# Chemical118/TREW

Hardware: NVIDIA B200
Metric: Gbases/s for trew short 5 32 at 1/2/4/8 B200; % of HBM roofline (higher is better)
Workload: dtype u64

## Files before the change

trew_b200/csrc/device_ctx.cu:

```cuda
#include <algorithm>
#include <chrono>
#include <cstdarg>
#include <cstdio>
#include <cstdlib>
#include <cstring>
#include <string>
#include <thread>
#include <vector>

#include <cuda_runtime.h>

#include "host_internal.h"
#include "scan_kernels.cuh"

using namespace trew;

namespace {

template <typename T, bool Pinned = false>
struct Buf {
    T* p = nullptr;
    size_t cap = 0;
    Buf() = default;
    Buf(Buf&& o) noexcept : p(o.p), cap(o.cap) { o.p = nullptr; o.cap = 0; }
    Buf(const Buf&) = delete;
    Buf& operator=(const Buf&) = delete;
    ~Buf() { release(); }
    cudaError_t grow(size_t n, cudaStream_t st) {
        if (n <= cap) return cudaSuccess;
        if (p) { cudaError_t e = cudaStreamSynchronize(st); if (e != cudaSuccess) return e; }
        return alloc(std::max((n + n / 4) * sizeof(T), (size_t)1 << 20) / sizeof(T));
    }
    cudaError_t alloc(size_t n) {
        cudaError_t e = release();
        if (e == cudaSuccess) e = Pinned ? cudaHostAlloc((void**)&p, n * sizeof(T), cudaHostAllocDefault) : cudaMalloc((void**)&p, n * sizeof(T));
        if (e != cudaSuccess) p = nullptr;
        else cap = n;
        return e;
    }
    cudaError_t release() {
        cudaError_t e = cudaSuccess;
        if (p) e = Pinned ? cudaFreeHost(p) : cudaFree(p);
        p = nullptr; cap = 0;
        return e;
    }
};

constexpr int kScanCounters = 8;
struct ScanBufs {
    Buf<unsigned int> survivors, counters;
    Buf<unsigned char> scratch;
    cudaError_t alloc(uint32_t n_units) {
        cudaError_t e = survivors.alloc(2 * (size_t)std::max<uint32_t>(n_units, 1));
        return e == cudaSuccess ? counters.alloc(kScanCounters) : e;
    }
};

struct SlotRes {
    Buf<unsigned char, true> h_buf;
    Buf<unsigned char> d_buf;
    Buf<unsigned char, true> h_inv;
    Buf<unsigned char> d_inv;
    size_t inv_cap = 0;
    Buf<unsigned int, true> h_keys;
    ScanBufs scan;
    size_t survivors_cap = 0;
    cudaStream_t stream = nullptr;
    cudaEvent_t ev_start = nullptr, ev_done = nullptr;
    bool in_flight = false;
};

struct RangeInfo { uint32_t r0, r1; uint64_t bases; uint32_t max_len; };

}

struct trew_resident {
    Buf<unsigned char> d_buf;
    DevBatch batch{};
    uint32_t n_reads = 0, n_units = 0, max_read_len = 0;
    uint64_t bases = 0;
    ScanBufs scan;
    cudaEvent_t ev[4] = {nullptr, nullptr, nullptr, nullptr};
    bool ev_pending = false;
};

struct trew_ctx {
    trew_config cfg{};
    int sm_count = 0;
    LaunchPlan plan{};
    cudaStream_t aux_stream = nullptr;
    cudaEvent_t ev_join = nullptr;
    int resident_streams = 1;
    uint64_t resident_seq = 0;
    DevCfg dcfg{};
    size_t n_slots = 0;
    Buf<Slot> table;
    Buf<unsigned int> d_error;
    Buf<unsigned short> d_thr;
    Buf<unsigned long long> d_total_surv;
    std::vector<SlotRes> slots;
    size_t next_slot = 0;
    size_t staging_bytes = 0;
    cudaStream_t main_stream = nullptr;
    cudaEvent_t ev_a = nullptr, ev_b = nullptr;
    Buf<trew_entry> d_entries;
    Buf<trew_entry> d_sorted;
    Buf<trew_entry> d_concat;
    bool sorted_valid = false;
    Buf<unsigned char> d_sort_tmp;
    Buf<unsigned int> d_n;
    uint64_t n_export = 0;
    bool export_valid = false;
    trew_stats stats{};
    Pool* pool = nullptr;
    bool own_pool = true;
    std::string err;
    std::vector<RangeInfo> ranges_tmp;
    unsigned int keys_seen = 0;
    bool sparse_val = true;
    unsigned int exact_flags = 0;
    std::vector<InvList> inv_tmp;
    IngestScratch ingest;
    cudaEvent_t ev_t0 = nullptr, ev_t1 = nullptr;
    double screen_ms = 0, decide_ms = 0, exact_ms = 0; uint64_t n_prof_scans = 0;
    std::vector<trew_resident*> pending_prof;
    Buf<trew_entry, true> h_export;
    unsigned int report_min = 0;
    Buf<trew_entry> d_filtered;
    Buf<UnitRecs> d_recs; Buf<trew_unit_record> d_rec_buf;
    uint64_t unit_next = 0;
    bool table_used = false;
    Buf<trew_unit_record> d_rec_out;
    Buf<trew_unit_record> d_rec_cat;
    Buf<trew_unit_record, true> h_rec;
};

namespace {

int fail(trew_ctx* c, int status, const char* fmt, ...) {
    char buf[512];
    va_list ap; va_start(ap, fmt); vsnprintf(buf, sizeof(buf), fmt, ap); va_end(ap);
    if (c) c->err = buf;
    return status;
}

#define CK(call)                                                                                         \
    do {                                                                                                 \
        cudaError_t e_ = (call);                                                                         \
        if (e_ != cudaSuccess) return fail(ctx, TREW_ERR_CUDA, "%s: %s", #call, cudaGetErrorString(e_)); \
    } while (0)

void build_thr(double B, std::vector<unsigned short>& thr) {
    thr.assign(kThrTableSize, 0xFFFF);
    for (int T = 1; T < kThrTableSize; T++) {
        int lo = 0, hi = T;
        while (lo < hi) {
            int mid = (lo + hi) / 2;
            if ((double)mid / (double)T >= B) hi = mid; else lo = mid + 1;
        }
        thr[T] = (unsigned short)lo;
    }
}

int run_cap_for(const trew_config& cfg, uint32_t max_read_len) {
    uint32_t w = max_read_len;
    if (cfg.mode == TREW_MODE_LONG) w = std::min<uint32_t>(max_read_len, 2u * (uint32_t)cfg.slice_length);
    w = std::min<uint32_t>(w, (uint32_t)kMaxWindow);
    return (int)std::max<uint32_t>((w + 2 + 7) & ~7u, 32u);
}

constexpr unsigned int kLongThreadCap = 32768;

size_t scratch_need(const trew_ctx* ctx, uint32_t max_read_len, uint32_t n_units, unsigned int* stride, size_t* long_off,
                    unsigned int* s_cap, unsigned int* max_slices) {
    unsigned int st = 16;
    if (ctx->cfg.mode == TREW_MODE_LONG) st = 2u * (max_read_len / (uint32_t)ctx->cfg.slice_length + 2u);
    st = (st + 15u) & ~15u;
    *stride = st;
    size_t bytes = ((size_t)st * (size_t)exact_warps_total(ctx->sm_count) + 255) & ~(size_t)255;
    *long_off = bytes;
    *s_cap = 0; *max_slices = 0;
    if (long_thread_path_applies(ctx->dcfg) && (ctx->exact_flags & 16u)) {
        *s_cap = std::min<unsigned int>(std::max<unsigned int>(n_units, 1u), kLongThreadCap);
        *max_slices = max_read_len / (uint32_t)ctx->cfg.slice_length + 1u;
        bytes += long_thread_scratch_bytes(*s_cap, *max_slices);
    }
    return bytes;
}

static int env_blocks_thread() {
    static const int v = [] { const char* e = getenv("TREW_GRID_THREAD"); int x = e && *e ? atoi(e) : 0; return x > 0 ? x : 0; }();
    return v;
}

int launch_scan(trew_ctx* ctx, const DevBatch& b, uint32_t n_units, uint32_t max_read_len, ScanBufs& sb, cudaStream_t st,
                cudaEvent_t* ev = nullptr) {
    unsigned int stride, s_cap, max_slices;
    size_t long_off;
    CK(sb.scratch.grow(scratch_need(ctx, max_read_len, n_units, &stride, &long_off, &s_cap, &max_slices), st));
    unsigned int* d_survivors = sb.survivors.p;
    unsigned int* d_counters = sb.counters.p;
    ctx->export_valid = false;
    ctx->table_used = true;
    DevCfg cfg = ctx->dcfg;
    cfg.unit_base = ctx->unit_next;
    ctx->unit_next += n_units;
    CK(cudaMemsetAsync(d_counters, 0, kScanCounters * sizeof(unsigned int), st));
    if (ev) CK(cudaEventRecord(ev[0], st));
    const bool thread_path = thread_path_applies(cfg, max_read_len) && !(ctx->exact_flags & 4u) && n_units < (1u << 28);
    launch_filter(cfg, b, n_units, max_read_len, d_survivors + n_units, d_counters + 2, d_survivors, d_counters, ctx->plan, st,
                  ev ? ev[1] : nullptr, thread_path ? d_survivors + n_units - 1 : nullptr, thread_path ? d_counters + 4 : nullptr,
                  d_counters + 7);
    if (ev) CK(cudaEventRecord(ev[2], st));
    ExactArgs a{};
    a.survivors = d_survivors; a.n_survivors = d_counters; a.work_counter = d_counters + 1;
    a.slice_scratch = sb.scratch.p; a.slice_scratch_stride = stride; a.run_cap = run_cap_for(ctx->cfg, max_read_len);
    a.total_survivors = ctx->d_total_surv.p;
    a.packed_probes = n_units < (1u << 28) ? 1 : 0;
    a.exp_flags = ctx->exact_flags;
    if (thread_path) {
        unsigned int* hard = d_survivors + n_units;
        launch_exact_thread(cfg, b, d_survivors, d_counters, a.packed_probes, hard, d_counters + 3, ctx->d_total_surv.p,
                            ctx->sm_count, env_blocks_thread(), d_counters + 6, st);
        ExactArgs ab = a;
        ab.survivors = d_survivors + n_units - 1; ab.reverse = 1; ab.n_survivors = d_counters + 4;
        launch_exact(cfg, b, ab, ctx->plan, st);
        a.survivors = hard; a.n_survivors = d_counters + 3; a.work_counter = d_counters + 5; a.total_survivors = nullptr;
        ctx->stats.kernel_launches += 2;
    } else if (s_cap > 0 && n_units < (1u << 28)) {
        unsigned int* hard = d_survivors + n_units;
        launch_long_thread(cfg, b, d_survivors, d_counters, a.packed_probes, s_cap, max_slices, sb.scratch.p + long_off, hard,
                           d_counters + 3, ctx->d_total_surv.p, ctx->sm_count, st);
        a.survivors = hard; a.n_survivors = d_counters + 3; a.total_survivors = nullptr;
        ctx->stats.kernel_launches += 3;
    }
    launch_exact(cfg, b, a, ctx->plan, st);
    if (ev) CK(cudaEventRecord(ev[3], st));
    CK(cudaGetLastError());
    ctx->stats.kernel_launches += 3;
    return TREW_OK;
}

int retire_slot(trew_ctx* ctx, SlotRes& s) {
    if (!s.in_flight) return TREW_OK;
    CK(cudaEventSynchronize(s.ev_done));
    float ms = 0.f;
    CK(cudaEventElapsedTime(&ms, s.ev_start, s.ev_done));
    ctx->stats.device_ms += ms;
    s.in_flight = false;
    ctx->keys_seen = std::max(ctx->keys_seen, *s.h_keys.p);
    return TREW_OK;
}

int export_entries(trew_ctx* ctx, bool need_sorted, const trew_entry** out, uint64_t* n_out);
int check_device_error(trew_ctx* ctx);

int grow_table_to(trew_ctx* ctx, size_t min_slots) {
    size_t new_slots = ctx->n_slots;
    while (new_slots < ((size_t)1 << 28) && new_slots < min_slots) new_slots <<= 1;
    if (new_slots == ctx->n_slots) return TREW_OK;
    uint64_t n = 0;
    int rc = export_entries(ctx, false, nullptr, &n);
    if (rc) return rc;
    Buf<Slot> other;
    CK(other.alloc(new_slots));
    CK(cudaMemsetAsync(other.p, 0, new_slots * sizeof(Slot), ctx->main_stream));
    CK(cudaMemsetAsync(ctx->d_error.p + 1, 0, sizeof(unsigned int), ctx->main_stream));
    std::swap(ctx->table.p, other.p); std::swap(ctx->table.cap, other.cap);
    ctx->dcfg.slots = ctx->table.p; ctx->dcfg.slot_mask = (unsigned int)(new_slots - 1); ctx->n_slots = new_slots;
    launch_merge_entries(ctx->dcfg, ctx->d_entries.p, (unsigned int)n, ctx->main_stream);
    CK(cudaGetLastError());
    CK(cudaStreamSynchronize(ctx->main_stream));
    CK(other.release());
    ctx->stats.kernel_launches += 1;
    ctx->keys_seen = (unsigned int)n;
    for (auto& sl : ctx->slots) *sl.h_keys.p = (unsigned int)n;
    return check_device_error(ctx);
}

int maybe_grow_table(trew_ctx* ctx) {
    if ((size_t)ctx->keys_seen * 16 <= ctx->n_slots) return TREW_OK;
    unsigned int keys = 0;
    CK(cudaMemcpy(&keys, ctx->d_error.p + 1, sizeof(keys), cudaMemcpyDeviceToHost));
    ctx->keys_seen = std::max(ctx->keys_seen, keys);
    if ((size_t)keys * 4 <= ctx->n_slots) return TREW_OK;
    return grow_table_to(ctx, (size_t)keys * 8);
}

DevBatch device_batch(const BatchView& v, uint32_t n, const void* host_base, const void* device_base) {
    auto at = [&](const uint32_t* p) { return (const unsigned int*)((const char*)device_base + ((const char*)p - (const char*)host_base)); };
    DevBatch b{};
    b.n_reads = n; b.bit_off = at(v.bit_off); b.hi = at(v.hi); b.lo = at(v.lo); b.val = at(v.val);
    return b;
}

void copy_batch(const trew_batch* batch, const BatchView& v, Pool* pool) {
    const uint32_t n = batch->n_reads;
    const size_t words = (size_t)((batch->bit_off[n] + 31ULL) / 32);
    memcpy(v.bit_off, batch->bit_off, (size_t)(n + 1) * 4);
    const uint32_t* src[3] = {batch->hi, batch->lo, batch->val};
    uint32_t* dst[3] = {v.hi, v.lo, v.val};
    pool->run(3, [&](int i) {
        memcpy(dst[i], src[i], words * 4);
        memset(dst[i] + words, 0, (v.plane_words - words) * 4);
    });
}

int scan_on_slot(trew_ctx* ctx, SlotRes& s, const DevBatch& b, uint32_t max_len, uint64_t bases, size_t h2d_bytes) {
    const uint32_t n = b.n_reads;
    const uint32_t n_units = ctx->cfg.mode == TREW_MODE_PAIR ? n / 2 : n;
    int rc = launch_scan(ctx, b, n_units, max_len, s.scan, s.stream);
    if (rc) return rc;
    CK(cudaMemcpyAsync(s.h_keys.p, ctx->d_error.p + 1, sizeof(unsigned int), cudaMemcpyDeviceToHost, s.stream));
    CK(cudaEventRecord(s.ev_done, s.stream));
    s.in_flight = true;
    ctx->stats.reads += n; ctx->stats.bases += bases; ctx->stats.units += n_units; ctx->stats.h2d_bytes += h2d_bytes;
    return TREW_OK;
}

int submit_ranges(trew_ctx* ctx, const ChunkView& cv, const RangeInfo* rg, int n_ranges) {
    uint64_t total_bases = 0; uint32_t max_len = 0;
    for (int i = 0; i < n_ranges; i++) { total_bases += rg[i].bases; max_len = std::max(max_len, rg[i].max_len); }
    const uint32_t n = n_ranges ? rg[n_ranges - 1].r1 - rg[0].r0 : 0u;
    if (n == 0) return TREW_OK;
    SlotRes& s = ctx->slots[ctx->next_slot];
    ctx->next_slot = (ctx->next_slot + 1) % ctx->slots.size();
    static const bool trace = getenv("TREW_SUBMIT_TRACE") != nullptr;
    auto now = [] { return std::chrono::duration<double, std::milli>(std::chrono::steady_clock::now().time_since_epoch()).count(); };
    const double t0 = trace ? now() : 0;
    int rc = retire_slot(ctx, s);
    if (rc) return rc;
    const double t1 = trace ? now() : 0;
    if ((rc = maybe_grow_table(ctx)) != TREW_OK) return rc;
    const double t2 = now();
    BatchView v;
    batch_layout(s.h_buf.p, n, total_bases, &v);
    std::vector<uint64_t> bit0((size_t)n_ranges);
    uint64_t acc = 0;
    for (int i = 0; i < n_ranges; i++) { bit0[i] = acc; acc += rg[i].bases; }
    v.bit_off[n] = (uint32_t)total_bases;
    const uint32_t first = rg[0].r0;
    std::vector<uint64_t> side_flat((size_t)3 * n_ranges);
    uint64_t (*side)[3] = (uint64_t (*)[3])side_flat.data();
    if (ctx->inv_tmp.size() < (size_t)n_ranges) ctx->inv_tmp.resize((size_t)n_ranges);
    auto pack = [&](bool list) {
        pack_prepare(bit0.data(), n_ranges, total_bases, v);
        ctx->pool->run(n_ranges, [&](int i) {
            pack_chunk_range(cv, rg[i].r0, rg[i].r1, rg[i].r0 - first, bit0[i], v, side[i], list ? &ctx->inv_tmp[(size_t)i] : nullptr, list,
                             rg[i].bases);
        });
        pack_fixup(bit0.data(), side, n_ranges, v);
    };
    size_t n_inv = 0;
    bool sparse = ctx->sparse_val;
    pack(sparse);
    const bool tail_pad = (total_bases & 31) != 0;
    if (sparse) {
        n_inv = tail_pad ? 1 : 0;
        for (int i = 0; i < n_ranges; i++) n_inv += ctx->inv_tmp[(size_t)i].size();
        if (n_inv > s.inv_cap) { sparse = false; pack(false); }
    }

    const double t3 = now();
    ctx->stats.host_pack_bytes += total_bases; ctx->stats.host_pack_ms += t3 - t2;
    CK(cudaEventRecord(s.ev_start, s.stream));
    const size_t head_bytes = (size_t)((char*)v.val - (char*)s.h_buf.p);
    unsigned int* d_val = (unsigned int*)(s.d_buf.p + head_bytes);
    size_t sent = v.bytes;
    if (sparse) {
        std::vector<size_t> at((size_t)n_ranges + 1, 0);
        for (int i = 0; i < n_ranges; i++) at[(size_t)i + 1] = at[(size_t)i] + ctx->inv_tmp[(size_t)i].bytes();
        ctx->pool->run(n_ranges, [&](int i) {
            const InvList& l = ctx->inv_tmp[(size_t)i];
            if (l.bytes()) memcpy(s.h_inv.p + at[(size_t)i], l.buf.get(), l.bytes());
        });
        if (tail_pad) inv_record(s.h_inv.p + at[(size_t)n_ranges], (uint32_t)total_bases, (1ULL << (32 - (total_bases & 31))) - 1ULL);
        const size_t ones_words = (size_t)((total_bases + 31) / 32);
        CK(cudaMemsetAsync(d_val, 0xFF, ones_words * 4, s.stream));
        CK(cudaMemsetAsync(d_val + ones_words, 0, (v.plane_words - ones_words) * 4, s.stream));
        CK(cudaMemcpyAsync(s.d_buf.p, s.h_buf.p, head_bytes, cudaMemcpyHostToDevice, s.stream));
        if (n_inv) {
            CK(cudaMemcpyAsync(s.d_inv.p, s.h_inv.p, n_inv * kInvRecBytes, cudaMemcpyHostToDevice, s.stream));
            launch_clear_invalid(d_val, (const unsigned int*)s.d_inv.p, (unsigned int)n_inv, s.stream);
            ctx->stats.kernel_launches += 1;
        }
        sent = head_bytes + n_inv * kInvRecBytes;
    } else {
        CK(cudaMemcpyAsync(s.d_buf.p, s.h_buf.p, v.bytes, cudaMemcpyHostToDevice, s.stream));
    }
    rc = scan_on_slot(ctx, s, device_batch(v, n, s.h_buf.p, s.d_buf.p), max_len, total_bases, sent);
    if (rc) return rc;
    if (trace)
        fprintf(stderr, "[submit] %u reads: wait slot %.3f ms, table check %.3f ms, pack %.3f ms, enqueue %.3f ms\n", n, t1 - t0, t2 - t1,
                t3 - t2, now() - t3);
    return TREW_OK;
}

int check_lengths(trew_ctx* ctx, int mode, uint32_t longest) {
    if (mode == TREW_MODE_SHORT && longest > 1000) return fail(ctx, TREW_ERR_TOO_LONG, "%s", trew_status_string(TREW_ERR_TOO_LONG));
    if (mode == TREW_MODE_PAIR && longest > (uint32_t)kMaxWindow) return fail(ctx, TREW_ERR_TOO_LONG, "paired read longer than %d", kMaxWindow);
    return TREW_OK;
}

size_t take_fitting(const trew_ctx* ctx, const RangeInfo* rg, size_t g, size_t n_ranges) {
    size_t h = g; uint64_t bases = 0, reads = 0;
    while (h < n_ranges) {
        const uint64_t nb = bases + rg[h].bases, nr = reads + (rg[h].r1 - rg[h].r0);
        if (batch_bytes((uint32_t)nr, nb) > ctx->staging_bytes || nr > ctx->slots[0].survivors_cap || nb >= 0xfffff000ULL) break;
        bases = nb; reads = nr; h++;
    }
    return h;
}

int submit_chunk_view(trew_ctx* ctx, const ChunkView& cv, uint32_t n) {
    if (n == 0) return TREW_OK;
    const uint32_t unit = cv.unit;
    const uint32_t n_units = n / unit;
    uint64_t span = 0;
    for (int sd = 0; sd < (int)unit; sd++) {
        const int32_t* l = cv.locs[sd];
        span += (uint64_t)std::max<int64_t>(0, (int64_t)l[2 * (size_t)(n_units - 1) + 1] - l[0] + 1);
    }
    uint64_t by_size = span / std::max<uint64_t>(1, ctx->staging_bytes / 16) + 1;
    uint32_t n_ranges = (uint32_t)std::min<uint64_t>(n_units, std::max<uint64_t>(by_size, (uint64_t)ctx->pool->size() * 4));
    auto& rg = ctx->ranges_tmp;
    rg.resize(n_ranges);
    for (uint32_t i = 0; i < n_ranges; i++) {
        rg[i].r0 = (uint32_t)((uint64_t)n_units * i / n_ranges) * unit;
        rg[i].r1 = (uint32_t)((uint64_t)n_units * (i + 1) / n_ranges) * unit;
    }
    ctx->pool->run((int)n_ranges, [&](int i) { chunk_stats(cv, rg[i].r0, rg[i].r1, &rg[i].bases, &rg[i].max_len); });
    uint32_t mx = 0;
    for (auto& r : rg) mx = std::max(mx, r.max_len);
    int rc = check_lengths(ctx, ctx->cfg.mode, mx);
    if (rc) return rc;
    auto too_big = [&](const RangeInfo& r) {
        return fail(ctx, TREW_ERR_ARG, "a single read/pair (%llu bases) does not fit a staging buffer of %zu bytes",
                    (unsigned long long)r.bases, ctx->staging_bytes);
    };
    size_t g = 0;
    while (g < n_ranges) {
        const size_t h = take_fitting(ctx, rg.data(), g, n_ranges);
        if (h > g) {
            if ((rc = submit_ranges(ctx, cv, rg.data() + g, (int)(h - g))) != TREW_OK) return rc;
            g = h;
            continue;
        }
        if (rg[g].r1 - rg[g].r0 <= unit) return too_big(rg[g]);
        std::vector<RangeInfo> fine;
        for (uint32_t r = rg[g].r0; r < rg[g].r1; r += unit) {
            RangeInfo f{r, r + unit, 0, 0};
            chunk_stats(cv, f.r0, f.r1, &f.bases, &f.max_len);
            fine.push_back(f);
        }
        for (size_t a = 0; a < fine.size();) {
            const size_t e = take_fitting(ctx, fine.data(), a, fine.size());
            if (e == a) return too_big(fine[a]);
            std::vector<RangeInfo> merged;
            size_t per = std::max<size_t>(1, (e - a) / (size_t)ctx->pool->size());
            for (size_t i = a; i < e; i += per) {
                RangeInfo m{fine[i].r0, 0, 0, 0};
                for (size_t j = i; j < std::min(e, i + per); j++) { m.r1 = fine[j].r1; m.bases += fine[j].bases; m.max_len = std::max(m.max_len, fine[j].max_len); }
                merged.push_back(m);
            }
            if ((rc = submit_ranges(ctx, cv, merged.data(), (int)merged.size())) != TREW_OK) return rc;
            a = e;
        }
        g++;
    }
    return TREW_OK;
}

int collect_prof(trew_ctx* ctx) {
    for (trew_resident* r : ctx->pending_prof) {
        if (!r->ev_pending) continue;
        CK(cudaEventSynchronize(r->ev[3]));
        float a = 0, b = 0, c = 0;
        CK(cudaEventElapsedTime(&a, r->ev[0], r->ev[1]));
        CK(cudaEventElapsedTime(&b, r->ev[1], r->ev[2]));
        CK(cudaEventElapsedTime(&c, r->ev[2], r->ev[3]));
        ctx->screen_ms += a; ctx->decide_ms += b; ctx->exact_ms += c; ctx->n_prof_scans++;
        ctx->stats.device_ms += a + b + c;
        r->ev_pending = false;
    }
    ctx->pending_prof.clear();
    return TREW_OK;
}

int join_aux(trew_ctx* ctx) {
    if (ctx->resident_streams != 2) return TREW_OK;
    CK(cudaEventRecord(ctx->ev_join, ctx->aux_stream));
    CK(cudaStreamWaitEvent(ctx->main_stream, ctx->ev_join, 0));
    return TREW_OK;
}

int fork_aux(trew_ctx* ctx) {
    if (ctx->resident_streams != 2) return TREW_OK;
    CK(cudaEventRecord(ctx->ev_join, ctx->main_stream));
    CK(cudaStreamWaitEvent(ctx->aux_stream, ctx->ev_join, 0));
    return TREW_OK;
}

int reader_slice_length(const trew_ctx* ctx) { return ctx->d_recs.p ? 0 : ctx->cfg.slice_length; }

int check_batch(trew_ctx* ctx, int mode, const trew_batch* batch) {
    if (!batch) return fail(ctx, TREW_ERR_ARG, "null batch");
    const uint32_t n = batch->n_reads;
    if (n == 0) return TREW_OK;
    if (!batch->bit_off) return fail(ctx, TREW_ERR_ARG, "null bit_off");
    if (batch->bit_off[0] != 0) return fail(ctx, TREW_ERR_ARG, "bit_off[0] must be 0");
    if (mode == TREW_MODE_PAIR && (n & 1u)) return fail(ctx, TREW_ERR_ARG, "paired batch with an odd n_reads (%u): mates come in twos", n);
    uint32_t longest = 0;
    for (uint32_t i = 0; i < n; i++) {
        const uint32_t a = batch->bit_off[i], b = batch->bit_off[i + 1];
        if (b < a) return fail(ctx, TREW_ERR_ARG, "bit_off decreases at read %u (%u after %u)", i, b, a);
        longest = std::max(longest, b - a);
    }
    if (int rc = check_lengths(ctx, mode, longest)) return rc;
    if (batch->max_read_len < longest)
        return fail(ctx, TREW_ERR_ARG, "max_read_len (%u) is smaller than the longest read (%u)", batch->max_read_len, longest);
    return TREW_OK;
}

int check_device_error(trew_ctx* ctx) {
    unsigned int e = 0;
    CK(cudaMemcpy(&e, ctx->d_error.p, sizeof(e), cudaMemcpyDeviceToHost));
    if (e == 3u) return fail(ctx, TREW_ERR_TABLE_FULL, "device count table full (%zu slots): raise table_log2_slots", ctx->n_slots);
    if (e) return fail(ctx, TREW_ERR_CUDA, "device error flag %u", e);
    return TREW_OK;
}

}

extern "C" {

int trew_abi_version(void) { return TREW_ABI_VERSION; }

const char* trew_status_string(int status) {
    switch (status) {
        case TREW_OK: return "ok";
        case TREW_ERR_ARG: return "bad argument";
        case TREW_ERR_CUDA: return "CUDA failure";
        case TREW_ERR_TABLE_FULL: return "device count table full";
        case TREW_ERR_TOO_LONG: return "This mode is designed for short-read sequencing. Please use 'trew long'.";
        case TREW_ERR_IO: return "file I/O error";
        case TREW_ERR_PAIRING: return "paired-end record mismatch";
        case TREW_ERR_NOMEM: return "memory allocation failure";
        default: return "unknown status";
    }
}

int trew_check_batch(int mode, const trew_batch* batch) {
    if (mode < TREW_MODE_SHORT || mode > TREW_MODE_LONG) return TREW_ERR_ARG;
    return check_batch(nullptr, mode, batch);
}

static thread_local std::string g_create_error;

static int default_host_threads(int asked) {
    return asked > 0 ? asked : (int)std::min(64u, std::max(1u, std::thread::hardware_concurrency()));
}

const char* trew_dev_last_error(const trew_ctx* ctx) { return ctx ? ctx->err.c_str() : g_create_error.c_str(); }

static int create_ctx(const trew_config* cfg, trew_ctx** out, std::string& g_create_error, Pool* shared_pool) {
    if (!cfg || !out) return TREW_ERR_ARG;
    *out = nullptr;
    g_create_error.clear();
    auto bad_arg = [&](const char* msg) { g_create_error = msg; return TREW_ERR_ARG; };
    if (cfg->mode < 0 || cfg->mode > 2) return bad_arg("mode must be TREW_MODE_SHORT, _PAIR or _LONG");
    if (cfg->min_mer < 3 || cfg->max_mer > 64 || cfg->min_mer > cfg->max_mer) return bad_arg("need 3 <= MIN_MER <= MAX_MER <= 64");
    if (!(0 < cfg->low_baseline && cfg->low_baseline <= 1) || !(0 < cfg->high_baseline && cfg->high_baseline <= 1) ||
        cfg->low_baseline > cfg->high_baseline) return bad_arg("need 0 < LOW_BASELINE <= HIGH_BASELINE <= 1");
    if (cfg->mode == TREW_MODE_LONG && cfg->slice_length > 0 && cfg->slice_length < 2 * cfg->max_mer)
        return bad_arg("SLICE_LENGTH must be greater than or equal to twice of MAX_MER.");
    if (cfg->mode == TREW_MODE_LONG && cfg->slice_length > 512)
        return bad_arg("SLICE_LENGTH above 512 is not supported by the GPU path (a slice of up to 2*SLICE_LENGTH-1 bases must fit "
                       "a 1023-base window); use -s 512 or less.");
    trew_ctx* ctx = new trew_ctx();
    ctx->cfg = *cfg;
    if (ctx->cfg.slice_length <= 0) ctx->cfg.slice_length = 150;
    auto bail = [&](int rc) { g_create_error = ctx->err; trew_dev_destroy(ctx); return rc; };
#define CKC(call)                                                                                   \
    do {                                                                                            \
        cudaError_t e_ = (call);                                                                    \
        if (e_ != cudaSuccess) { fail(ctx, TREW_ERR_CUDA, "%s: %s", #call, cudaGetErrorString(e_)); return bail(TREW_ERR_CUDA); } \
    } while (0)
    const bool timing = getenv("TREW_CLI_TIMING") != nullptr;
    auto now = [] { return std::chrono::duration<double, std::milli>(std::chrono::steady_clock::now().time_since_epoch()).count(); };
    double t_prev = now();
    auto lap = [&](const char* what) {
        if (!timing) return;
        const double t = now();
        fprintf(stderr, "[trew] create, device %d: %s %.1f ms\n", cfg->device, what, t - t_prev);
        t_prev = t;
    };
    int ndev = 0;
    CKC(cudaGetDeviceCount(&ndev));
    lap("driver init");
    if (cfg->device < 0 || cfg->device >= ndev) { fail(ctx, TREW_ERR_CUDA, "no CUDA device %d (found %d)", cfg->device, ndev); return bail(TREW_ERR_CUDA); }
    CKC(cudaSetDevice(cfg->device));
    cudaDeviceProp prop;
    CKC(cudaGetDeviceProperties(&prop, cfg->device));
    ctx->sm_count = prop.multiProcessorCount;
    ctx->plan = default_launch_plan(ctx->sm_count);
    {
        auto env_int = [](const char* name, int dflt) { const char* e = getenv(name); return e && *e ? atoi(e) : dflt; };
        int v;
        if ((v = env_int("TREW_GRID_SCREEN", 0)) > 0) ctx->plan.screen_blocks = ctx->sm_count * v;
        if ((v = env_int("TREW_GRID_DECIDE", 0)) > 0) ctx->plan.decide_blocks = ctx->sm_count * v;
        if ((v = env_int("TREW_GRID_EXACT", 0)) > 0) ctx->plan.exact_blocks = std::min(ctx->plan.exact_blocks, ctx->sm_count * v);
        ctx->resident_streams = env_int("TREW_RESIDENT_STREAMS", 1) >= 2 ? 2 : 1;
        ctx->sparse_val = env_int("TREW_DENSE_VAL", 0) == 0;
        ctx->exact_flags = (unsigned int)env_int("TREW_EXACT_FLAGS", 0);
    }
    int lg = cfg->table_log2_slots > 0 ? cfg->table_log2_slots : 22;
    if (lg < 10 || lg > 28) { fail(ctx, TREW_ERR_ARG, "table_log2_slots out of range"); return bail(TREW_ERR_ARG); }
    ctx->n_slots = (size_t)1 << lg;
    CKC(ctx->table.alloc(ctx->n_slots));
    CKC(cudaMemset(ctx->table.p, 0, ctx->n_slots * sizeof(Slot)));
    lap("primary context + count table");
    CKC(ctx->d_error.alloc(2));
    CKC(cudaMemset(ctx->d_error.p, 0, 2 * sizeof(unsigned int)));
    CKC(ctx->d_total_surv.alloc(1));
    CKC(cudaMemset(ctx->d_total_surv.p, 0, sizeof(unsigned long long)));
    std::vector<unsigned short> thr;
    build_thr(cfg->low_baseline, thr);
    std::vector<unsigned short> thr_hi;
    build_thr(cfg->high_baseline, thr_hi);
    CKC(ctx->d_thr.alloc(2 * thr.size()));
    CKC(cudaMemcpy(ctx->d_thr.p, thr.data(), thr.size() * sizeof(unsigned short), cudaMemcpyHostToDevice));
    CKC(cudaMemcpy(ctx->d_thr.p + thr.size(), thr_hi.data(), thr_hi.size() * sizeof(unsigned short), cudaMemcpyHostToDevice));
    ctx->dcfg.mode = cfg->mode; ctx->dcfg.min_mer = cfg->min_mer; ctx->dcfg.max_mer = cfg->max_mer;
    ctx->dcfg.slice_len = ctx->cfg.slice_length; ctx->dcfg.low = cfg->low_baseline; ctx->dcfg.high = cfg->high_baseline;
    ctx->dcfg.slots = ctx->table.p; ctx->dcfg.slot_mask = (unsigned int)(ctx->n_slots - 1);
    ctx->dcfg.error_flag = ctx->d_error.p; ctx->dcfg.thr_low = ctx->d_thr.p; ctx->dcfg.thr_high = ctx->d_thr.p + kThrTableSize;
    CKC(prepare_exact(kMaxWindow + 9));
    lap("kernel attributes (module load)");
    CKC(cudaStreamCreateWithFlags(&ctx->main_stream, cudaStreamNonBlocking));
    CKC(cudaStreamCreateWithFlags(&ctx->aux_stream, cudaStreamNonBlocking));
    CKC(cudaEventCreateWithFlags(&ctx->ev_join, cudaEventDisableTiming));
    CKC(cudaEventCreate(&ctx->ev_a));
    CKC(cudaEventCreate(&ctx->ev_b));
    CKC(cudaEventCreate(&ctx->ev_t0));
    CKC(cudaEventCreate(&ctx->ev_t1));
    ctx->staging_bytes = cfg->staging_bytes ? (size_t)cfg->staging_bytes : ((size_t)64 << 20);
    int ns = cfg->n_staging > 0 ? cfg->n_staging : 3;
    ctx->slots.resize((size_t)ns);
    for (auto& s : ctx->slots) {
        CKC(s.h_buf.alloc(ctx->staging_bytes));
        CKC(s.d_buf.alloc(ctx->staging_bytes));
        s.inv_cap = ctx->staging_bytes / 8 / kInvRecBytes;
        CKC(s.h_inv.alloc((s.inv_cap + 1) * kInvRecBytes));
        CKC(s.d_inv.alloc((s.inv_cap + 1) * kInvRecBytes));
        CKC(s.h_keys.alloc(1));
        *s.h_keys.p = 0;
        s.survivors_cap = ctx->staging_bytes / 8;
        CKC(s.scan.alloc((uint32_t)s.survivors_cap));
        CKC(cudaStreamCreateWithFlags(&s.stream, cudaStreamNonBlocking));
        CKC(cudaEventCreate(&s.ev_start));
        CKC(cudaEventCreate(&s.ev_done));
    }
    CKC(ctx->d_n.alloc(1));
    lap("staging ring (pinned + device buffers)");
    if (shared_pool) { ctx->pool = shared_pool; ctx->own_pool = false; }
    else ctx->pool = new Pool(default_host_threads(cfg->host_threads));
#undef CKC
    *out = ctx;
    return TREW_OK;
}

int trew_dev_create(const trew_config* cfg, trew_ctx** out) { return create_ctx(cfg, out, g_create_error, nullptr); }

void trew_dev_destroy(trew_ctx* ctx) {
    if (!ctx) return;
    cudaSetDevice(ctx->cfg.device);
    cudaDeviceSynchronize();
    for (auto& s : ctx->slots) {
        if (s.stream) cudaStreamDestroy(s.stream);
        if (s.ev_start) cudaEventDestroy(s.ev_start);
        if (s.ev_done) cudaEventDestroy(s.ev_done);
    }
    if (ctx->main_stream) cudaStreamDestroy(ctx->main_stream);
    if (ctx->aux_stream) cudaStreamDestroy(ctx->aux_stream);
    if (ctx->ev_join) cudaEventDestroy(ctx->ev_join);
    if (ctx->ev_a) cudaEventDestroy(ctx->ev_a);
    if (ctx->ev_b) cudaEventDestroy(ctx->ev_b);
    if (ctx->ev_t0) cudaEventDestroy(ctx->ev_t0);
    if (ctx->ev_t1) cudaEventDestroy(ctx->ev_t1);
    if (ctx->own_pool) delete ctx->pool;
    delete ctx;
}

int trew_dev_submit_chunk(trew_ctx* ctx, const char* buffer1, const int32_t* locs1, uint32_t n1,
                          const char* buffer2, const int32_t* locs2, uint32_t n2) {
    if (!ctx) return TREW_ERR_ARG;
    CK(cudaSetDevice(ctx->cfg.device));
    const bool pair = ctx->cfg.mode == TREW_MODE_PAIR;
    if (pair ? (!buffer2 && n2) : (buffer2 != nullptr || n2 != 0)) return fail(ctx, TREW_ERR_ARG, "second chunk only in pair mode");
    if ((n1 && (!buffer1 || !locs1)) || (n2 && !locs2)) return fail(ctx, TREW_ERR_ARG, "null chunk");
    ChunkView cv{{buffer1, buffer2}, {locs1, locs2}, {nullptr, nullptr}, pair ? 2u : 1u};
    const uint32_t n = pair ? 2u * std::min(n1, n2) : n1;
    if (n == 0) return TREW_OK;
    for (int sd = 0; sd < (pair ? 2 : 1); sd++) {
        const int32_t* l = cv.locs[sd];
        uint32_t cnt = pair ? n / 2 : n;
        int32_t last = l[2 * (size_t)(cnt - 1) + 1];
        if (last >= l[2 * (size_t)(cnt - 1)]) cv.end[sd] = cv.buf[sd] + last + 1;
    }
    return submit_chunk_view(ctx, cv, n);
}

int trew_dev_submit_packed(trew_ctx* ctx, const trew_batch* batch) {
    if (!ctx || !batch) return TREW_ERR_ARG;
    int rc = check_batch(ctx, ctx->cfg.mode, batch);
    if (rc) return rc;
    CK(cudaSetDevice(ctx->cfg.device));
    uint32_t n = batch->n_reads;
    if (n == 0) return TREW_OK;
    uint64_t bases = batch->bit_off[n];
    size_t bytes = batch_bytes(n, bases);
    if (bytes > ctx->staging_bytes || n > ctx->slots[0].survivors_cap)
        return fail(ctx, TREW_ERR_ARG, "packed batch (%zu bytes) larger than a staging buffer (%zu)", bytes, ctx->staging_bytes);
    SlotRes& s = ctx->slots[ctx->next_slot];
    ctx->next_slot = (ctx->next_slot + 1) % ctx->slots.size();
    rc = retire_slot(ctx, s);
    if (rc) return rc;
    BatchView v;
    batch_layout(s.h_buf.p, n, bases, &v);
    copy_batch(batch, v, ctx->pool);
    CK(cudaEventRecord(s.ev_start, s.stream));
    CK(cudaMemcpyAsync(s.d_buf.p, s.h_buf.p, v.bytes, cudaMemcpyHostToDevice, s.stream));
    return scan_on_slot(ctx, s, device_batch(v, n, s.h_buf.p, s.d_buf.p), batch->max_read_len, bases, v.bytes);
}

int trew_dev_upload(trew_ctx* ctx, const trew_batch* batch, trew_resident** out) {
    if (!ctx || !batch || !out) return TREW_ERR_ARG;
    int rc = check_batch(ctx, ctx->cfg.mode, batch);
    if (rc) return rc;
    CK(cudaSetDevice(ctx->cfg.device));
    uint32_t n = batch->n_reads;
    uint64_t bases = n ? batch->bit_off[n] : 0;
    auto r = std::make_unique<trew_resident>();
    size_t bytes = batch_bytes(n, bases);
    std::vector<char> tmp(bytes, 0);
    BatchView v;
    batch_layout(tmp.data(), n, bases, &v);
    if (n) copy_batch(batch, v, ctx->pool);
    CK(r->d_buf.alloc(bytes));
    CK(cudaMemcpy(r->d_buf.p, tmp.data(), bytes, cudaMemcpyHostToDevice));
    r->batch = device_batch(v, n, tmp.data(), r->d_buf.p);
    r->n_reads = n; r->n_units = ctx->cfg.mode == TREW_MODE_PAIR ? n / 2 : n; r->max_read_len = batch->max_read_len; r->bases = bases;
    CK(r->scan.alloc(r->n_units));
    *out = r.release();
    return TREW_OK;
}

int trew_dev_scan_resident(trew_ctx* ctx, const trew_resident* rb) {
    if (!ctx || !rb) return TREW_ERR_ARG;
    CK(cudaSetDevice(ctx->cfg.device));
    trew_resident* r = const_cast<trew_resident*>(rb);
    ctx->keys_seen = std::max<unsigned int>(ctx->keys_seen, (unsigned int)(ctx->n_slots / 16 + 1));
    if (r->ev_pending) { int rc0 = collect_prof(ctx); if (rc0) return rc0; }
    if (!r->ev[0]) for (int i = 0; i < 4; i++) CK(cudaEventCreate(&r->ev[i]));
    cudaStream_t st = (ctx->resident_streams == 2 && (ctx->resident_seq++ & 1)) ? ctx->aux_stream : ctx->main_stream;
    CK(cudaEventRecord(ctx->ev_a, st));
    int rc = launch_scan(ctx, r->batch, r->n_units, r->max_read_len, r->scan, st, r->ev);
    r->ev_pending = true; ctx->pending_prof.push_back(r);
    if (rc) return rc;
    CK(cudaEventRecord(ctx->ev_b, st));
    ctx->stats.reads += r->n_reads; ctx->stats.bases += r->bases; ctx->stats.units += r->n_units;
    return TREW_OK;
}

void trew_dev_free_resident(trew_ctx* ctx, trew_resident* r) {
    if (!r) return;
    if (ctx) { cudaSetDevice(ctx->cfg.device); cudaStreamSynchronize(ctx->main_stream); cudaStreamSynchronize(ctx->aux_stream); collect_prof(ctx); }
    for (int i = 0; i < 4; i++) if (r->ev[i]) cudaEventDestroy(r->ev[i]);
    delete r;
}

int trew_dev_sync(trew_ctx* ctx) {
    if (!ctx) return TREW_ERR_ARG;
    CK(cudaSetDevice(ctx->cfg.device));
    for (auto& s : ctx->slots) { int rc = retire_slot(ctx, s); if (rc) return rc; }
    { int rc = join_aux(ctx); if (rc) return rc; }
    CK(cudaStreamSynchronize(ctx->main_stream));
    { int rc = collect_prof(ctx); if (rc) return rc; }
    return check_device_error(ctx);
}

}

namespace {

template <typename Call>
cudaError_t with_temp(trew_ctx* ctx, Call call) {
    size_t need = 0;
    cudaError_t e = call(nullptr, &need);
    if (e == cudaSuccess) e = ctx->d_sort_tmp.grow(need, ctx->main_stream);
    if (e != cudaSuccess) return e;
    size_t bytes = ctx->d_sort_tmp.cap;
    return call(ctx->d_sort_tmp.p, &bytes);
}

int export_entries(trew_ctx* ctx, bool need_sorted, const trew_entry** out, uint64_t* n_out) {
    int rc = trew_dev_sync(ctx);
    if (rc) return rc;
    if (!ctx->export_valid) {
        unsigned int n = 1u << 20;
        for (int pass = 0; pass < 2; pass++) {
            CK(ctx->d_entries.grow(n, ctx->main_stream));
            CK(cudaMemsetAsync(ctx->d_n.p, 0, sizeof(unsigned int), ctx->main_stream));
            launch_compact(ctx->dcfg.slots, (unsigned int)ctx->n_slots, ctx->d_entries.p, ctx->d_n.p, ctx->main_stream,
                           (unsigned int)ctx->d_entries.cap);
            CK(cudaGetLastError());
            ctx->stats.kernel_launches += 1;
            CK(cudaMemcpyAsync(&n, ctx->d_n.p, sizeof(n), cudaMemcpyDeviceToHost, ctx->main_stream));
            CK(cudaStreamSynchronize(ctx->main_stream));
            if (n <= ctx->d_entries.cap) break;
        }
        ctx->n_export = n;
        ctx->export_valid = true;
        ctx->sorted_valid = false;
    }
    const unsigned int n = (unsigned int)ctx->n_export;
    if (need_sorted && !ctx->sorted_valid) {
        CK(ctx->d_sorted.grow(n, ctx->main_stream));
        if (n == 1) CK(cudaMemcpyAsync(ctx->d_sorted.p, ctx->d_entries.p, sizeof(trew_entry), cudaMemcpyDeviceToDevice, ctx->main_stream));
        if (n > 1) {
            const bool wide = ctx->cfg.max_mer > 32;
            CK(with_temp(ctx, [&](void* t, size_t* b) { return sort_entries_radix(ctx->d_entries.p, ctx->d_sorted.p, n, wide, t, b, ctx->main_stream); }));
            ctx->stats.kernel_launches += wide ? 11 : 8;
        }
        CK(cudaStreamSynchronize(ctx->main_stream));
        ctx->sorted_valid = true;
    }
    if (out) *out = need_sorted ? ctx->d_sorted.p : ctx->d_entries.p;
    if (n_out) *n_out = n;
    return TREW_OK;
}

template <typename T>
int rows_to_host(trew_ctx* ctx, Buf<T, true>& host, const T* d_rows, uint64_t n, const T** rows, uint64_t* n_rows) {
    CK(host.grow((size_t)n + 64 / sizeof(T), ctx->main_stream));
    if (n) {
        CK(cudaMemcpyAsync(host.p, d_rows, n * sizeof(T), cudaMemcpyDeviceToHost, ctx->main_stream));
        CK(cudaStreamSynchronize(ctx->main_stream));
    }
    ctx->stats.d2h_bytes += n * sizeof(T) + 4;
    if (rows) *rows = host.p;
    if (n_rows) *n_rows = n;
    return TREW_OK;
}

int finish_rows(trew_ctx* ctx, const trew_entry* d_in, uint64_t n_in, bool combine, const trew_entry** entries, uint64_t* n_entries) {
    CK(ctx->d_sorted.grow((size_t)n_in, ctx->main_stream));
    CK(ctx->d_filtered.grow((size_t)n_in, ctx->main_stream));
    ctx->sorted_valid = false;
    const bool wide = ctx->cfg.max_mer > 32;
    const trew_entry* src = d_in;
    unsigned int n = (unsigned int)n_in;
    cudaStream_t st = ctx->main_stream;
    if (ctx->report_min > 0 && n > 0) {
        CK(with_temp(ctx, [&](void* t, size_t* b) { return filter_report_rows(src, n, ctx->report_min, ctx->d_filtered.p, ctx->d_n.p, t, b, st); }));
        CK(cudaMemcpyAsync(&n, ctx->d_n.p, sizeof(n), cudaMemcpyDeviceToHost, st));
        CK(cudaStreamSynchronize(st));
        ctx->stats.kernel_launches += 5;
        src = ctx->d_filtered.p;
    }
    if (n == 1) CK(cudaMemcpyAsync(ctx->d_sorted.p, src, sizeof(trew_entry), cudaMemcpyDeviceToDevice, st));
    if (n > 1) {
        CK(with_temp(ctx, [&](void* t, size_t* b) { return sort_entries_radix(src, ctx->d_sorted.p, n, wide, t, b, st); }));
        ctx->stats.kernel_launches += wide ? 11 : 8;
    }
    const trew_entry* rows = ctx->d_sorted.p;
    if (combine && n > 0) {
        CK(with_temp(ctx, [&](void* t, size_t* b) { return combine_sorted_rows(ctx->d_sorted.p, n, ctx->d_filtered.p, ctx->d_n.p, t, b, st); }));
        CK(cudaMemcpyAsync(&n, ctx->d_n.p, sizeof(n), cudaMemcpyDeviceToHost, st));
        CK(cudaStreamSynchronize(st));
        ctx->stats.kernel_launches += 3;
        rows = ctx->d_filtered.p;
    }
    return rows_to_host(ctx, ctx->h_export, rows, n, entries, n_entries);
}

int unit_record_count(trew_ctx* ctx, uint64_t* made) {
    unsigned long long m = 0;
    CK(cudaMemcpy(&m, &ctx->d_recs.p->n, sizeof(m), cudaMemcpyDeviceToHost));
    *made = m;
    if (m > ctx->d_rec_buf.cap)
        return fail(ctx, TREW_ERR_TABLE_FULL, "unit records overflowed: %llu records made, capacity %llu (a capacity of %llu is enough)", m,
                    (unsigned long long)ctx->d_rec_buf.cap, m);
    return TREW_OK;
}

int records_to_host(trew_ctx* ctx, const trew_unit_record* d_in, uint64_t n_in, const trew_unit_record** recs, uint64_t* n_out) {
    if (n_in > 0x7fffffffULL) return fail(ctx, TREW_ERR_ARG, "too many unit records (%llu)", (unsigned long long)n_in);
    CK(ctx->d_rec_out.grow((size_t)n_in, ctx->main_stream));
    const unsigned int n = (unsigned int)n_in;
    const bool wide = ctx->cfg.max_mer > 32;
    CK(with_temp(ctx, [&](void* t, size_t* b) { return sort_combine_records(d_in, n, wide, ctx->d_rec_out.p, ctx->d_n.p, t, b, ctx->main_stream); }));
    unsigned int m = 0;
    CK(cudaMemcpyAsync(&m, ctx->d_n.p, sizeof(m), cudaMemcpyDeviceToHost, ctx->main_stream));
    CK(cudaStreamSynchronize(ctx->main_stream));
    return rows_to_host(ctx, ctx->h_rec, ctx->d_rec_out.p, m, recs, n_out);
}

}

extern "C" {

int trew_dev_export_device(trew_ctx* ctx, const trew_entry** d_entries, uint64_t* n_entries) {
    if (!ctx) return TREW_ERR_ARG;
    return export_entries(ctx, true, d_entries, n_entries);
}

int trew_dev_finish(trew_ctx* ctx, const trew_entry** entries, uint64_t* n_entries) {
    if (!ctx) return TREW_ERR_ARG;
    uint64_t n = 0;
    const trew_entry* d_rows = nullptr;
    if (ctx->report_min > 0) {
        int rc = export_entries(ctx, false, &d_rows, &n);
        if (rc) return rc;
        return finish_rows(ctx, d_rows, n, false, entries, n_entries);
    }
    int rc = export_entries(ctx, true, &d_rows, &n);
    if (rc) return rc;
    return rows_to_host(ctx, ctx->h_export, d_rows, n, entries, n_entries);
}

int trew_dev_finish_merged(trew_ctx* ctx, const trew_entry* const* d_lists, const uint64_t* n_rows, uint32_t n_lists,
                           const trew_entry** entries, uint64_t* n_entries) {
    if (!ctx || (n_lists && (!d_lists || !n_rows))) return TREW_ERR_ARG;
    uint64_t n0 = 0;
    const trew_entry* d_own = nullptr;
    int rc = export_entries(ctx, false, &d_own, &n0);
    if (rc) return rc;
    uint64_t total = n0;
    for (uint32_t i = 0; i < n_lists; i++) total += n_rows[i];
    if (total > 0xfffffff0ULL) return fail(ctx, TREW_ERR_ARG, "too many rows to merge (%llu)", (unsigned long long)total);
    CK(ctx->d_concat.grow((size_t)total, ctx->main_stream));
    uint64_t at = 0;
    if (n0) CK(cudaMemcpyAsync(ctx->d_concat.p, d_own, n0 * sizeof(trew_entry), cudaMemcpyDeviceToDevice, ctx->main_stream));
    at += n0;
    for (uint32_t i = 0; i < n_lists; i++) {
        if (n_rows[i]) CK(cudaMemcpyAsync(ctx->d_concat.p + at, d_lists[i], n_rows[i] * sizeof(trew_entry), cudaMemcpyDeviceToDevice, ctx->main_stream));
        at += n_rows[i];
    }
    return finish_rows(ctx, ctx->d_concat.p, total, true, entries, n_entries);
}

int trew_dev_export_rows(trew_ctx* ctx, trew_entry* d_rows, uint64_t capacity_rows, uint64_t* n_rows) {
    if (!ctx || !n_rows) return TREW_ERR_ARG;
    uint64_t n = 0;
    const trew_entry* d_src = nullptr;
    int rc = export_entries(ctx, false, &d_src, &n);
    if (rc) return rc;
    *n_rows = n;
    if (!d_rows) return TREW_OK;
    if (n > capacity_rows) return fail(ctx, TREW_ERR_ARG, "row buffer too small: %llu rows, capacity %llu", (unsigned long long)n,
                                       (unsigned long long)capacity_rows);
    if (n) CK(cudaMemcpyAsync(d_rows, d_src, n * sizeof(trew_entry), cudaMemcpyDeviceToDevice, ctx->main_stream));
    CK(cudaStreamSynchronize(ctx->main_stream));
    return TREW_OK;
}

int trew_dev_merge_rows(trew_ctx* ctx, const trew_entry* d_rows, uint64_t n_rows) {
    if (!ctx || (n_rows && !d_rows) || n_rows > 0xffffffffULL) return TREW_ERR_ARG;
    CK(cudaSetDevice(ctx->cfg.device));
    ctx->export_valid = false;
    ctx->table_used = true;
    ctx->keys_seen = std::max<unsigned int>(ctx->keys_seen, (unsigned int)(ctx->n_slots / 16 + 1));
    launch_merge_entries(ctx->dcfg, d_rows, (unsigned int)n_rows, ctx->main_stream);
    CK(cudaGetLastError());
    ctx->stats.kernel_launches += n_rows ? 1 : 0;
    return TREW_OK;
}

int trew_dev_set_report_filter(trew_ctx* ctx, uint32_t min_total) {
    if (!ctx) return TREW_ERR_ARG;
    ctx->report_min = min_total;
    return TREW_OK;
}

int trew_dev_reserve(trew_ctx* ctx, uint64_t expected_new_keys) {
    if (!ctx) return TREW_ERR_ARG;
    int rc = trew_dev_sync(ctx);
    if (rc) return rc;
    unsigned int keys = 0;
    CK(cudaMemcpy(&keys, ctx->d_error.p + 1, sizeof(keys), cudaMemcpyDeviceToHost));
    const uint64_t want = ((uint64_t)keys + expected_new_keys) * 4;
    if (want <= ctx->n_slots) return TREW_OK;
    return grow_table_to(ctx, (size_t)std::min<uint64_t>(want, (uint64_t)1 << 28));
}

int trew_dev_reset(trew_ctx* ctx) {
    if (!ctx) return TREW_ERR_ARG;
    int rc = trew_dev_sync(ctx);
    if (rc && rc != TREW_ERR_TABLE_FULL) return rc;
    ctx->export_valid = false;
    CK(cudaMemsetAsync(ctx->dcfg.slots, 0, ctx->n_slots * sizeof(Slot), ctx->main_stream));
    CK(cudaMemsetAsync(ctx->d_error.p, 0, 2 * sizeof(unsigned int), ctx->main_stream));
    if (ctx->d_recs.p) CK(cudaMemsetAsync(&ctx->d_recs.p->n, 0, sizeof(unsigned long long), ctx->main_stream));
    CK(cudaStreamSynchronize(ctx->main_stream));
    ctx->unit_next = 0;
    ctx->table_used = false;
    ctx->keys_seen = 0;
    for (auto& sl : ctx->slots) *sl.h_keys.p = 0;
    return TREW_OK;
}

int trew_dev_enable_unit_records(trew_ctx* ctx, uint64_t capacity_records) {
    if (!ctx) return TREW_ERR_ARG;
    if (ctx->table_used) return fail(ctx, TREW_ERR_ARG, "unit records can only be switched on or off while the table is empty (after create or reset)");
    if (capacity_records > 0x7fffffffULL) return fail(ctx, TREW_ERR_ARG, "unit record capacity above 2^31 - 1");
    CK(cudaSetDevice(ctx->cfg.device));
    CK(cudaStreamSynchronize(ctx->main_stream));
    ctx->dcfg.recs = nullptr;
    CK(ctx->d_rec_buf.release());
    CK(ctx->d_recs.release());
    if (capacity_records == 0) return TREW_OK;
    CK(ctx->d_rec_buf.alloc(capacity_records));
    CK(ctx->d_recs.alloc(1));
    const UnitRecs r{ctx->d_rec_buf.p, (unsigned long long)capacity_records, 0ULL};
    CK(cudaMemcpy(ctx->d_recs.p, &r, sizeof(r), cudaMemcpyHostToDevice));
    ctx->dcfg.recs = ctx->d_recs.p;
    return TREW_OK;
}

int trew_dev_unit_records(trew_ctx* ctx, const trew_unit_record** recs, uint64_t* n) {
    if (!ctx || !recs || !n) return TREW_ERR_ARG;
    if (!ctx->d_recs.p) return fail(ctx, TREW_ERR_ARG, "unit records are off (trew_dev_enable_unit_records)");
    int rc = trew_dev_sync(ctx);
    if (rc) return rc;
    uint64_t made = 0;
    if ((rc = unit_record_count(ctx, &made)) != TREW_OK) return rc;
    return records_to_host(ctx, ctx->d_rec_buf.p, made, recs, n);
}

int trew_dev_get_stats(trew_ctx* ctx, trew_stats* out) {
    if (!ctx || !out) return TREW_ERR_ARG;
    CK(cudaSetDevice(ctx->cfg.device));
    unsigned long long s = 0;
    CK(cudaMemcpy(&s, ctx->d_total_surv.p, sizeof(s), cudaMemcpyDeviceToHost));
    ctx->stats.survivors = s;
    *out = ctx->stats;
    return TREW_OK;
}

int trew_dev_last_resident_ms(trew_ctx* ctx, float* ms) {
    if (!ctx || !ms) return TREW_ERR_ARG;
    CK(cudaEventSynchronize(ctx->ev_b));
    CK(cudaEventElapsedTime(ms, ctx->ev_a, ctx->ev_b));
    return TREW_OK;
}

int trew_dev_timer_start(trew_ctx* ctx) {
    if (!ctx) return TREW_ERR_ARG;
    CK(cudaSetDevice(ctx->cfg.device));
    CK(cudaEventRecord(ctx->ev_t0, ctx->main_stream));
    return fork_aux(ctx);
}

int trew_dev_timer_stop(trew_ctx* ctx, float* ms) {
    if (!ctx || !ms) return TREW_ERR_ARG;
    CK(cudaSetDevice(ctx->cfg.device));
    { int rc = join_aux(ctx); if (rc) return rc; }
    CK(cudaEventRecord(ctx->ev_t1, ctx->main_stream));
    CK(cudaEventSynchronize(ctx->ev_t1));
    CK(cudaEventElapsedTime(ms, ctx->ev_t0, ctx->ev_t1));
    return TREW_OK;
}

int trew_dev_kernel_times(trew_ctx* ctx, double* screen_ms, double* decide_ms, double* exact_ms, uint64_t* n_scans) {
    if (!ctx) return TREW_ERR_ARG;
    CK(cudaSetDevice(ctx->cfg.device));
    { int rc0 = join_aux(ctx); if (rc0) return rc0; }
    CK(cudaStreamSynchronize(ctx->main_stream));
    int rc = collect_prof(ctx);
    if (rc) return rc;
    if (screen_ms) *screen_ms = ctx->screen_ms;
    if (decide_ms) *decide_ms = ctx->decide_ms;
    if (exact_ms) *exact_ms = ctx->exact_ms;
    if (n_scans) *n_scans = ctx->n_prof_scans;
    ctx->screen_ms = ctx->decide_ms = ctx->exact_ms = 0; ctx->n_prof_scans = 0;
    return TREW_OK;
}

int trew_synth_resident(trew_ctx* ctx, uint64_t seed, uint32_t n_reads, uint32_t read_len, uint32_t tel_ppm,
                        uint32_t half_ppm, uint32_t n_ppm, uint32_t sub_ppm, trew_resident** out) {
    return trew_synth_resident_ex(ctx, seed, n_reads, read_len, tel_ppm, half_ppm, n_ppm, sub_ppm, 0, out);
}

int trew_synth_resident_ex(trew_ctx* ctx, uint64_t seed, uint32_t n_reads, uint32_t read_len, uint32_t tel_ppm,
                           uint32_t half_ppm, uint32_t n_ppm, uint32_t sub_ppm, uint32_t flavor, trew_resident** out) {
    if (!ctx || !out || read_len == 0 || flavor > 2 || (uint64_t)n_reads * read_len >= 0xfffff000ULL) return TREW_ERR_ARG;
    CK(cudaSetDevice(ctx->cfg.device));
    auto thr = [](uint32_t ppm) { return (unsigned int)(((unsigned long long)ppm << 32) / 1000000ULL); };
    uint64_t bases = (uint64_t)n_reads * read_len;
    size_t bytes = batch_bytes(n_reads, bases);
    auto r = std::make_unique<trew_resident>();
    CK(r->d_buf.alloc(bytes));
    BatchView v;
    batch_layout(r->d_buf.p, n_reads, bases, &v);
    launch_synth(seed, n_reads, read_len, thr(tel_ppm), thr(half_ppm), thr(n_ppm), thr(sub_ppm), flavor, v.bit_off, v.hi, v.lo, v.val,
                 v.plane_words, ctx->main_stream);
    CK(cudaGetLastError());
    CK(cudaStreamSynchronize(ctx->main_stream));
    r->batch = device_batch(v, n_reads, r->d_buf.p, r->d_buf.p);
    r->n_reads = n_reads; r->n_units = ctx->cfg.mode == TREW_MODE_PAIR ? n_reads / 2 : n_reads;
    r->max_read_len = read_len; r->bases = bases;
    CK(r->scan.alloc(r->n_units));
    *out = r.release();
    return TREW_OK;
}

int trew_dev_process_file(trew_ctx* ctx, const char* file1, int is_gz1, const char* file2, int is_gz2) {
    if (!ctx || !file1) return TREW_ERR_ARG;
    if ((ctx->cfg.mode == TREW_MODE_PAIR) != (file2 != nullptr)) return fail(ctx, TREW_ERR_ARG, "second file only in pair mode");
    const size_t chunk = 0;
    IngestResult r = ingest_file(ctx->cfg.mode, reader_slice_length(ctx), file1, is_gz1 != 0, file2, is_gz2 != 0, chunk,
                                 [&](const char* b1, const std::vector<int32_t>& l1, const char* b2, const std::vector<int32_t>& l2) {
                                     return trew_dev_submit_chunk(ctx, b1, l1.data(), (uint32_t)(l1.size() / 2), b2,
                                                                  b2 ? l2.data() : nullptr, b2 ? (uint32_t)(l2.size() / 2) : 0u);
                                 },
                                 ctx->pool, &ctx->ingest);
    if (r.status != TREW_OK && r.status != TREW_ERR_CUDA && !r.message.empty()) ctx->err = r.message;
    return r.status;
}

}


struct trew_multi {
    std::vector<trew_ctx*> ctx;
    Pool* pool = nullptr;
    size_t next = 0;
    uint64_t unit_next = 0;
    std::string err;
    Buf<trew_entry> d_peer;
};

namespace {
int mfail(trew_multi* m, int status, const std::string& msg) { if (m) m->err = msg; return status; }
uint64_t chunk_units(const trew_ctx* x, uint32_t n1, uint32_t n2) { return x->cfg.mode == TREW_MODE_PAIR ? std::min(n1, n2) : n1; }

template <typename T>
int gather_to_first(trew_multi* m, size_t first, const std::vector<const T*>& src, const std::vector<uint64_t>& n, Buf<T>& dst) {
    trew_ctx* ctx = m->ctx[0];
    CK(cudaSetDevice(ctx->cfg.device));
    uint64_t total = 0;
    for (size_t i = first; i < n.size(); i++) total += n[i];
    CK(dst.grow((size_t)total, ctx->main_stream));
    uint64_t at = 0;
    for (size_t i = first; i < n.size(); i++) {
        if (n[i]) CK(cudaMemcpyPeerAsync(dst.p + at, ctx->cfg.device, src[i], m->ctx[i]->cfg.device, n[i] * sizeof(T), ctx->main_stream));
        at += n[i];
    }
    return TREW_OK;
}
}

extern "C" {

int trew_multi_create(const trew_config* cfg, const int32_t* devices, int32_t n_devices, trew_multi** out) {
    if (!cfg || !out || n_devices < 0 || (n_devices > 0 && !devices)) return TREW_ERR_ARG;
    *out = nullptr;
    std::vector<int32_t> dev;
    if (n_devices == 0) {
        int nd = 0;
        if (cudaGetDeviceCount(&nd) != cudaSuccess || nd <= 0) { g_create_error = "no CUDA device"; return TREW_ERR_CUDA; }
        for (int i = 0; i < nd; i++) dev.push_back(i);
    } else {
        dev.assign(devices, devices + n_devices);
    }
    trew_multi* m = new trew_multi();
    m->pool = new Pool(default_host_threads(cfg->host_threads));
    int rc = TREW_OK;
    {
        std::vector<trew_ctx*> made(dev.size(), nullptr);
        std::vector<int> rcs(dev.size(), TREW_OK);
        std::vector<std::string> errs(dev.size());
        std::vector<std::thread> th;
        auto make = [&](size_t i) {
            trew_config c = *cfg;
            c.device = dev[i];
            rcs[i] = create_ctx(&c, &made[i], errs[i], m->pool);
        };
        for (size_t i = 1; i < dev.size(); i++) th.emplace_back(make, i);
        make(0);
        for (auto& t : th) t.join();
        for (size_t i = 0; i < dev.size(); i++) {
            if (rcs[i] != TREW_OK && rc == TREW_OK) { rc = rcs[i]; g_create_error = errs[i]; }
            if (made[i]) m->ctx.push_back(made[i]);
        }
    }
    if (rc != TREW_OK) { trew_multi_destroy(m); return rc; }
    for (size_t i = 1; i < m->ctx.size(); i++) {
        int can = 0;
        if (dev[i] != dev[0] && cudaDeviceCanAccessPeer(&can, dev[0], dev[i]) == cudaSuccess && can) {
            cudaSetDevice(dev[0]);
            cudaError_t e = cudaDeviceEnablePeerAccess(dev[i], 0);
            if (e != cudaSuccess) cudaGetLastError();
        }
    }
    *out = m;
    return TREW_OK;
}

void trew_multi_destroy(trew_multi* m) {
    if (!m) return;
    if (!m->ctx.empty()) {
        cudaSetDevice(m->ctx[0]->cfg.device);
        m->d_peer.release();
    }
    for (trew_ctx* x : m->ctx) trew_dev_destroy(x);
    delete m->pool;
    delete m;
}

int trew_multi_device_count(const trew_multi* m) { return m ? (int)m->ctx.size() : 0; }

const char* trew_multi_last_error(const trew_multi* m) { return m ? m->err.c_str() : g_create_error.c_str(); }

trew_ctx* trew_multi_ctx(trew_multi* m, int32_t i) { return m && i >= 0 && (size_t)i < m->ctx.size() ? m->ctx[(size_t)i] : nullptr; }

int trew_multi_submit_chunk(trew_multi* m, const char* buffer1, const int32_t* locs1, uint32_t n1, const char* buffer2,
                            const int32_t* locs2, uint32_t n2) {
    if (!m) return TREW_ERR_ARG;
    trew_ctx* x = m->ctx[m->next];
    m->next = (m->next + 1) % m->ctx.size();
    x->unit_next = m->unit_next;
    int rc = trew_dev_submit_chunk(x, buffer1, locs1, n1, buffer2, locs2, n2);
    if (rc != TREW_OK) return mfail(m, rc, x->err);
    m->unit_next += chunk_units(x, n1, n2);
    return TREW_OK;
}

int trew_multi_process_file(trew_multi* m, const char* file1, int is_gz1, const char* file2, int is_gz2) {
    if (!m || !file1) return TREW_ERR_ARG;
    trew_ctx* x0 = m->ctx[0];
    if ((x0->cfg.mode == TREW_MODE_PAIR) != (file2 != nullptr)) return mfail(m, TREW_ERR_ARG, "second file only in pair mode");
    IngestResult r = ingest_file(x0->cfg.mode, reader_slice_length(x0), file1, is_gz1 != 0, file2, is_gz2 != 0, 0,
                                 [&](const char* b1, const std::vector<int32_t>& l1, const char* b2, const std::vector<int32_t>& l2) {
                                     return trew_multi_submit_chunk(m, b1, l1.data(), (uint32_t)(l1.size() / 2), b2, b2 ? l2.data() : nullptr,
                                                                    b2 ? (uint32_t)(l2.size() / 2) : 0u);
                                 },
                                 m->pool, &x0->ingest);
    if (r.status != TREW_OK && !r.message.empty()) m->err = r.message;
    return r.status;
}

int trew_multi_reset(trew_multi* m) {
    if (!m) return TREW_ERR_ARG;
    for (trew_ctx* x : m->ctx) { int rc = trew_dev_reset(x); if (rc != TREW_OK) return mfail(m, rc, x->err); }
    m->next = 0;
    m->unit_next = 0;
    return TREW_OK;
}

int trew_multi_finish(trew_multi* m, const trew_entry** entries, uint64_t* n_entries) {
    if (!m) return TREW_ERR_ARG;
    trew_ctx* x0 = m->ctx[0];
    const size_t nd = m->ctx.size();
    if (nd == 1) {
        int rc = trew_dev_finish(x0, entries, n_entries);
        return rc == TREW_OK ? rc : mfail(m, rc, x0->err);
    }
    std::vector<const trew_entry*> d_src(nd, nullptr);
    std::vector<uint64_t> n_rows(nd, 0);
    for (size_t i = 1; i < nd; i++) {
        int rc = export_entries(m->ctx[i], false, &d_src[i], &n_rows[i]);
        if (rc != TREW_OK) return mfail(m, rc, m->ctx[i]->err);
    }
    int rc = gather_to_first(m, 1, d_src, n_rows, m->d_peer);
    if (rc) return rc;
    const trew_entry* peers = m->d_peer.p;
    uint64_t n_peers = 0;
    for (size_t i = 1; i < nd; i++) n_peers += n_rows[i];
    rc = trew_dev_finish_merged(x0, &peers, &n_peers, 1, entries, n_entries);
    return rc == TREW_OK ? rc : mfail(m, rc, x0->err);
}

int trew_multi_enable_unit_records(trew_multi* m, uint64_t capacity_records) {
    if (!m) return TREW_ERR_ARG;
    for (trew_ctx* x : m->ctx) {
        int rc = trew_dev_enable_unit_records(x, capacity_records);
        if (rc != TREW_OK) return mfail(m, rc, x->err);
    }
    return TREW_OK;
}

int trew_multi_unit_records(trew_multi* m, const trew_unit_record** recs, uint64_t* n) {
    if (!m || !recs || !n) return TREW_ERR_ARG;
    trew_ctx* x0 = m->ctx[0];
    if (!x0->d_recs.p) return mfail(m, TREW_ERR_ARG, "unit records are off (trew_multi_enable_unit_records)");
    const size_t nd = m->ctx.size();
    std::vector<uint64_t> made(nd, 0);
    uint64_t total = 0, most = 0;
    int full = TREW_OK;
    for (size_t i = 0; i < nd; i++) {
        int rc = trew_dev_sync(m->ctx[i]);
        if (rc != TREW_OK) return mfail(m, rc, m->ctx[i]->err);
        rc = unit_record_count(m->ctx[i], &made[i]);
        if (rc == TREW_ERR_TABLE_FULL) full = rc;
        else if (rc != TREW_OK) return mfail(m, rc, m->ctx[i]->err);
        total += made[i]; most = std::max(most, made[i]);
    }
    if (full != TREW_OK)
        return mfail(m, full, "unit records overflowed on a device: " + std::to_string(most) + " records made, capacity " +
                                  std::to_string(x0->d_rec_buf.cap) + " (a capacity of " + std::to_string(most) + " is enough)");
    if (nd == 1) {
        int rc = records_to_host(x0, x0->d_rec_buf.p, made[0], recs, n);
        return rc == TREW_OK ? rc : mfail(m, rc, x0->err);
    }
    std::vector<const trew_unit_record*> src;
    for (trew_ctx* x : m->ctx) src.push_back(x->d_rec_buf.p);
    int rc = gather_to_first(m, 0, src, made, x0->d_rec_cat);
    if (rc) return rc;
    rc = records_to_host(x0, x0->d_rec_cat.p, total, recs, n);
    return rc == TREW_OK ? rc : mfail(m, rc, x0->err);
}

int trew_multi_set_report_filter(trew_multi* m, uint32_t min_total) {
    if (!m) return TREW_ERR_ARG;
    return trew_dev_set_report_filter(m->ctx[0], min_total);
}

int trew_multi_get_stats(trew_multi* m, trew_stats* out) {
    if (!m || !out) return TREW_ERR_ARG;
    trew_stats t;
    memset(&t, 0, sizeof(t));
    for (trew_ctx* x : m->ctx) {
        trew_stats s;
        int rc = trew_dev_get_stats(x, &s);
        if (rc != TREW_OK) return mfail(m, rc, x->err);
        t.reads += s.reads; t.bases += s.bases; t.units += s.units; t.survivors += s.survivors;
        t.kernel_launches += s.kernel_launches; t.h2d_bytes += s.h2d_bytes; t.d2h_bytes += s.d2h_bytes;
        t.host_pack_bytes += s.host_pack_bytes; t.host_pack_ms += s.host_pack_ms;
        t.device_ms = std::max(t.device_ms, s.device_ms);
    }
    *out = t;
    return TREW_OK;
}

}
```

trew_b200/csrc/scan_kernels.cu:

```cuda
#include "scan_kernels.cuh"
#include "exact_thread.cuh"

#include <cstdio>

namespace trew {

typedef unsigned int u32;
typedef unsigned long long u64;
typedef unsigned __int128 u128;


__device__ __forceinline__ u32 lane_id() { return threadIdx.x & 31; }

__device__ __forceinline__ u32 low_mask(int bits) {
    return bits >= 32 ? 0xffffffffu : ((1u << bits) - 1u);
}

__device__ __forceinline__ u32 prefix_xor32(u32 x) {
    x ^= x << 1; x ^= x << 2; x ^= x << 4; x ^= x << 8; x ^= x << 16;
    return x;
}

__device__ __forceinline__ u64 mix64(u64 x) {
    x ^= x >> 33; x *= 0xff51afd7ed558ccdULL; x ^= x >> 33; x *= 0xc4ceb9fe1a85ec53ULL; x ^= x >> 33;
// ... 196 lines not shown

template <int NW>
__device__ __forceinline__ void prefix_xor_excl(const u32 (&in)[NW], u32 (&out)[NW]) {
    u32 carry = 0, prev_top = 0;
#pragma unroll
    for (int j = 0; j < NW; j++) {
        u32 inc = prefix_xor32(in[j]) ^ carry;
        out[j] = (inc << 1) | prev_top;
        prev_top = inc >> 31;
        carry = 0u - prev_top;
    }
}

template <int NW>
__device__ __forceinline__ void shr1(u32 (&x)[NW]) {
#pragma unroll
    for (int j = 0; j < NW; j++) x[j] = __funnelshift_r(x[j], j + 1 < NW ? x[j + 1] : 0u, 1);
}

template <int NW>
__device__ __forceinline__ void shr_var(const u32 (&in)[NW], int k, u32 (&out)[NW]) {
#pragma unroll
    for (int j = 0; j < NW; j++) out[j] = in[j];
    for (int s = k >> 5; s > 0; s--) {
#pragma unroll
        for (int j = 0; j < NW; j++) out[j] = j + 1 < NW ? out[j + 1] : 0u;
    }
    u32 r = k & 31;
#pragma unroll
    for (int j = 0; j < NW; j++) out[j] = __funnelshift_r(out[j], j + 1 < NW ? out[j + 1] : 0u, r);
}

template <int NW>
__device__ __forceinline__ void sliding_and(u32 (&a)[NW], int k) {
    u32 t[NW];
    int w = 1;
    while (2 * w <= k) {
        shr_var<NW>(a, w, t);
#pragma unroll
        for (int j = 0; j < NW; j++) a[j] &= t[j];
        w *= 2;
    }
    if (k > w) {
        shr_var<NW>(a, k - w, t);
#pragma unroll
        for (int j = 0; j < NW; j++) a[j] &= t[j];
    }
}

__device__ __forceinline__ void csa(u32 a, u32 b, u32 c, u32& s, u32& cy) {
    s = a ^ b ^ c;
    cy = (a & b) | (c & (a ^ b));
}

template <int NW>
__device__ __forceinline__ int popc_multi(const u32 (&x)[NW]) {
    if constexpr (NW == 1) return __popc(x[0]);
    else if constexpr (NW == 2) return __popc(x[0]) + __popc(x[1]);
    else if constexpr (NW == 3) {
        u32 s, c; csa(x[0], x[1], x[2], s, c);
        return __popc(s) + 2 * __popc(c);
    } else if constexpr (NW == 5) {
        u32 s1, c1, s2, c2; csa(x[0], x[1], x[2], s1, c1); csa(s1, x[3], x[4], s2, c2);
        return __popc(s2) + 2 * (__popc(c1) + __popc(c2));
    } else if constexpr (NW == 8) {
        u32 s1, c1, s2, c2, s3, c3, s4, c4;
        csa(x[0], x[1], x[2], s1, c1); csa(x[3], x[4], x[5], s2, c2); csa(s1, s2, x[6], s3, c3);
        csa(c1, c2, c3, s4, c4);
        return __popc(s3) + __popc(x[7]) + 2 * __popc(s4) + 4 * __popc(c4);
    } else {
        int t = 0;
#pragma unroll
        for (int j = 0; j < NW; j++) t += __popc(x[j]);
        return t;
    }
}

template <int NW>
__device__ __noinline__ bool probe_filter(const DevBatch& b, u32 pos, int wl, int k0, int k1,
                                          const unsigned short* __restrict__ thr) {
    u32 PH[NW], PL[NW], QH[NW], QL[NW], WV[NW];
    {
        u32 t[NW];
        load_bits<NW>(b.hi, pos, t); prefix_xor_excl<NW>(t, PH);
        load_bits<NW>(b.lo, pos, t); prefix_xor_excl<NW>(t, PL);
        load_bits<NW>(b.val, pos, WV); mask_bits<NW>(WV, wl);
    }
    shr_var<NW>(PH, k0, QH);
    shr_var<NW>(PL, k0, QL);
    sliding_and<NW>(WV, k0);
    u32 PA[NW];
    bool have_pa = false;
    for (int k = k0; k <= k1; k++) {
        u32 a[NW], bb[NW], c[NW];
#pragma unroll
        for (int j = 0; j < NW; j++) {
            u32 dh = QH[j] ^ PH[j], dl = QL[j] ^ PL[j];
            a[j] = dh & WV[j]; bb[j] = dl & WV[j]; c[j] = a[j] & dl;
        }
        int T = popc_multi<NW>(WV);
        if (T == 0) break;
        int cH = popc_multi<NW>(a), cL = popc_multi<NW>(bb), c11 = popc_multi<NW>(c);
        int c10 = cH - c11, c01 = cL - c11, c00 = T - cH - cL + c11;
        int U = max(max(c00, c01), max(c10, c11));
        int need = thr[T];
        if (U >= need) {
            u32 QA[NW];
            if (!have_pa) {
                u32 A[NW], t[NW];
                load_bits<NW>(b.hi, pos, A); load_bits<NW>(b.lo, pos, t);
#pragma unroll
                for (int j = 0; j < NW; j++) A[j] &= t[j];
                prefix_xor_excl<NW>(A, PA);
                have_pa = true;
            }
            shr_var<NW>(PA, k, QA);
            u32 x11[NW], x10[NW], x01[NW], x00[NW];
#pragma unroll
            for (int j = 0; j < NW; j++) {
                u32 da = QA[j] ^ PA[j];
                u32 dh = QH[j] ^ PH[j], dl = QL[j] ^ PL[j];
                x11[j] = c[j] & da; x10[j] = a[j] & ~dl & da; x01[j] = bb[j] & ~dh & da; x00[j] = WV[j] & ~dh & ~dl & da;
            }
            int n11 = popc_multi<NW>(x11), n10 = popc_multi<NW>(x10), n01 = popc_multi<NW>(x01), n00 = popc_multi<NW>(x00);
            int U2 = max(max(max(n11, c11 - n11), max(n10, c10 - n10)), max(max(n01, c01 - n01), max(n00, c00 - n00)));
            if (U2 >= need) return true;
        }
        shr1<NW>(QH); shr1<NW>(QL);
        u32 t[NW];
#pragma unroll
        for (int j = 0; j < NW; j++) t[j] = WV[j];
        shr1<NW>(t);
#pragma unroll
        for (int j = 0; j < NW; j++) WV[j] &= t[j];
    }
    return false;
}

template <int MAXNW>
__device__ __forceinline__ bool probe_dispatch(const DevBatch& b, const Probe& p, const unsigned short* thr) {
    if (p.k1 < p.k0) return false;
    int need_bits = p.wl + 1;
    if (need_bits <= 96) return probe_filter<3>(b, p.pos, p.wl, p.k0, p.k1, thr);
    if constexpr (MAXNW >= 5) { if (need_bits <= 160) return probe_filter<5>(b, p.pos, p.wl, p.k0, p.k1, thr); }
    if constexpr (MAXNW >= 8) { if (need_bits <= 256) return probe_filter<8>(b, p.pos, p.wl, p.k0, p.k1, thr); }
    return true;
}


constexpr u32 kPackC11 = 1u - (1u << 8) - (1u << 16) + (1u << 24);
constexpr u32 kPackH = (1u << 8) - (1u << 24);
constexpr u32 kPackL = (1u << 16) - (1u << 24);
#ifndef TREW_SCREEN_UNROLL
#define TREW_SCREEN_UNROLL 2
#endif
constexpr int kScreenUnroll = TREW_SCREEN_UNROLL;
constexpr int kFastMaxWl = 95;
constexpr int kFastTabSize = kFastMaxWl + 2;
constexpr int kProbeShift = 28;
constexpr int kMod4BelowWindows = 48;
constexpr int kThreadMinWindows = 36;

__device__ __forceinline__ uint4 fast_entry(int T, int need) {
    uint4 e = make_uint4(0u, 0u, 0u, 0u);
    if (T <= 0) return e;
    int T01 = min(T, 64);
    e.y = T >= 32 ? 0xffffffffu : ((1u << T) - 1u);
    e.z = T <= 32 ? 0u : (T >= 64 ? 0xffffffffu : ((1u << (T - 32)) - 1u));
    int np = need - (T - T01);
    if (np <= 0) e.x = 0x80808080u;
    else if (np > 64) e.x = (u32)T01 << 24;
    else e.x = ((u32)T01 << 24) + (u32)(128 - np) * 0x01010101u;
    return e;
}

template <int S>
__device__ __forceinline__ bool fast_span(const u32 (&ph)[5], const u32 (&pl)[5], int wl, int ka, int kb,
                                          const uint4* __restrict__ tab) {
    const uint4* tp = tab + (wl - ka + 1);
#pragma unroll (kScreenUnroll)
    for (int k = ka; k <= kb; k++, tp--) {
        const uint4 e = *tp;
        u32 qh0 = __funnelshift_r(ph[S], ph[S + 1], k), qh1 = __funnelshift_r(ph[S + 1], ph[S + 2], k);
        u32 ql0 = __funnelshift_r(pl[S], pl[S + 1], k), ql1 = __funnelshift_r(pl[S + 1], pl[S + 2], k);
        u32 a0 = (qh0 ^ ph[0]) & e.y, a1 = (qh1 ^ ph[1]) & e.z;
        u32 b0 = (ql0 ^ pl[0]) & e.y, b1 = (ql1 ^ pl[1]) & e.z;
        u32 x = e.x + (u32)(__popc(a0) + __popc(a1)) * kPackH + (u32)(__popc(b0) + __popc(b1)) * kPackL +
                (u32)(__popc(a0 & b0) + __popc(a1 & b1)) * kPackC11;
        if (x & 0x80808080u) return true;
    }
    return false;
}

__device__ __forceinline__ bool probe_is_fast(const Probe& p) { return p.wl <= kFastMaxWl && p.k1 <= 63 && p.k1 <= p.wl; }

__device__ __forceinline__ bool screen_probe(const DevBatch& b, const Probe& p, const uint4* __restrict__ tab) {
    if (p.k1 < p.k0) return false;
    if (!probe_is_fast(p)) return true;
    u32 t[3], full[3] = {0xffffffffu, 0xffffffffu, 0xffffffffu};
    mask_bits<3>(full, p.wl);
    load_bits<3>(b.val, p.pos, t);
    if ((((t[0] & full[0]) ^ full[0]) | ((t[1] & full[1]) ^ full[1]) | ((t[2] & full[2]) ^ full[2])) != 0u) return true;
    u32 ph[5], pl[5], q[3];
    load_bits<3>(b.hi, p.pos, t); mask_bits<3>(t, p.wl); prefix_xor_excl<3>(t, q);
    ph[0] = q[0]; ph[1] = q[1]; ph[2] = q[2]; ph[3] = 0u; ph[4] = 0u;
    load_bits<3>(b.lo, p.pos, t); mask_bits<3>(t, p.wl); prefix_xor_excl<3>(t, q);
    pl[0] = q[0]; pl[1] = q[1]; pl[2] = q[2]; pl[3] = 0u; pl[4] = 0u;
    int k0 = p.k0;
    if (k0 < 32) {
        if (fast_span<0>(ph, pl, p.wl, k0, min(p.k1, 31), tab)) return true;
        k0 = 32;
    }
    return p.k1 >= 32 && fast_span<1>(ph, pl, p.wl, k0, p.k1, tab);
}

constexpr int kFastMaxWlLong = 159;
constexpr int kFastTabSizeLong = kFastMaxWlLong + 2;
struct __align__(16) FastEntryLong { u32 base, m0, m1, m2, m3, pad0, pad1, pad2; };

__device__ __forceinline__ FastEntryLong fast_entry_long(int T, int need) {
    FastEntryLong e = {0u, 0u, 0u, 0u, 0u, 0u, 0u, 0u};
    if (T <= 0) return e;
    const int T01 = min(T, 128);
    u32 m[4];
#pragma unroll
    for (int j = 0; j < 4; j++) { int vb = T - 32 * j; m[j] = vb <= 0 ? 0u : low_mask(min(32, vb)); }
    e.m0 = m[0]; e.m1 = m[1]; e.m2 = m[2]; e.m3 = m[3];
    const int np = need - (T - T01);
    if (np <= 0) e.base = 0x80808080u;
    else if (np > 128) e.base = 0u;
    else e.base = ((u32)T01 << 24) + (u32)(128 - np) * 0x01010101u;
    return e;
}

template <int S>
__device__ __forceinline__ bool fast_span_long(const u32 (&ph)[8], const u32 (&pl)[8], int wl, int ka, int kb,
                                               const FastEntryLong* __restrict__ tab) {
    const FastEntryLong* tp = tab + (wl - ka + 1);
    for (int k = ka; k <= kb; k++, tp--) {
        const uint4 e0 = *reinterpret_cast<const uint4*>(tp);
        const u32 m3 = tp->m3;
        if (e0.x == 0u) continue;
        const u32 mk[4] = {e0.y, e0.z, e0.w, m3};
        int cH = 0, cL = 0, c11 = 0;
#pragma unroll
        for (int j = 0; j < 4; j++) {
            u32 a = (__funnelshift_r(ph[S + j], ph[S + j + 1], k) ^ ph[j]) & mk[j];
            u32 bb = (__funnelshift_r(pl[S + j], pl[S + j + 1], k) ^ pl[j]) & mk[j];
            cH += __popc(a); cL += __popc(bb); c11 += __popc(a & bb);
        }
        u32 x = e0.x + (u32)cH * kPackH + (u32)cL * kPackL + (u32)c11 * kPackC11;
        if (x & 0x80808080u) return true;
    }
    return false;
}

__device__ __forceinline__ bool probe_is_fast_long(const Probe& p) { return p.wl <= kFastMaxWlLong && p.k1 <= 64 && p.k1 <= p.wl; }

__device__ __noinline__ bool screen_probe_long(const DevBatch& b, const Probe& p, const FastEntryLong* __restrict__ tab) {
    u32 t[5], full[5] = {0xffffffffu, 0xffffffffu, 0xffffffffu, 0xffffffffu, 0xffffffffu};
    mask_bits<5>(full, p.wl);
    load_bits<5>(b.val, p.pos, t);
    u32 bad = 0;
#pragma unroll
    for (int j = 0; j < 5; j++) bad |= (t[j] & full[j]) ^ full[j];
    if (bad) return true;
    u32 ph[8], pl[8], q[5];
    load_bits<5>(b.hi, p.pos, t); mask_bits<5>(t, p.wl); prefix_xor_excl<5>(t, q);
#pragma unroll
    for (int j = 0; j < 8; j++) ph[j] = j < 5 ? q[j] : 0u;
    load_bits<5>(b.lo, p.pos, t); mask_bits<5>(t, p.wl); prefix_xor_excl<5>(t, q);
#pragma unroll
    for (int j = 0; j < 8; j++) pl[j] = j < 5 ? q[j] : 0u;
    int k0 = p.k0;
    if (k0 < 32) {
        if (fast_span_long<0>(ph, pl, p.wl, k0, min(p.k1, 31), tab)) return true;
        k0 = 32;
    }
    if (k0 < 64 && p.k1 >= 32) {
        if (fast_span_long<1>(ph, pl, p.wl, k0, min(p.k1, 63), tab)) return true;
        k0 = 64;
    }
    return p.k1 >= 64 && fast_span_long<2>(ph, pl, p.wl, k0, p.k1, tab);
}

__device__ __forceinline__ void list_append(bool flag, u32 value, u32* __restrict__ list, u32* __restrict__ count) {
    u32 m = __ballot_sync(0xffffffffu, flag);
    if (m) {
        u32 base = 0;
        if (lane_id() == 0) base = atomicAdd(count, (u32)__popc(m));
        base = __shfl_sync(0xffffffffu, base, 0);
        if (flag) list[base + __popc(m & ((1u << lane_id()) - 1u))] = value;
    }
}

__device__ __forceinline__ void list_append_rev(bool flag, u32 value, u32* __restrict__ top, u32* __restrict__ count) {
    u32 m = __ballot_sync(0xffffffffu, flag);
    if (m) {
        u32 base = 0;
        if (lane_id() == 0) base = atomicAdd(count, (u32)__popc(m));
        base = __shfl_sync(0xffffffffu, base, 0);
        if (flag) *(top - (base + __popc(m & ((1u << lane_id()) - 1u)))) = value;
    }
}

#ifndef TREW_SCREEN_BPS
#define TREW_SCREEN_BPS 8
#endif
template <bool LONG>
__global__ void __launch_bounds__(256, LONG ? 4 : TREW_SCREEN_BPS) trew_screen_kernel(DevCfg cfg, DevBatch b, u32 n_units,
                                                                                     u32* __restrict__ deferred, u32* __restrict__ n_deferred) {
    __shared__ uint4 tab[kFastTabSize];
    __shared__ FastEntryLong tab_long[LONG ? kFastTabSizeLong : 1];
    for (int T = threadIdx.x; T < kFastTabSize; T += blockDim.x) tab[T] = fast_entry(T, (int)cfg.thr_low[T]);
    if (LONG) for (int T = threadIdx.x; T < kFastTabSizeLong; T += blockDim.x) tab_long[T] = fast_entry_long(T, (int)cfg.thr_low[T]);
    __syncthreads();
    u32 stride = gridDim.x * blockDim.x;
    u32 n_round = (n_units + 31u) & ~31u;
    for (u32 u = blockIdx.x * blockDim.x + threadIdx.x; u < n_round; u += stride) {
        u32 pm = 0;
        if (u < n_units) {
            Probe p[4];
            int np = unit_probes(cfg, b, u, p);
            for (int i = 0; i < np; i++) {
                bool d;
                if (LONG && p[i].k1 >= p[i].k0 && !probe_is_fast(p[i]) && probe_is_fast_long(p[i])) d = screen_probe_long(b, p[i], tab_long);
                else d = screen_probe(b, p[i], tab);
                pm |= d ? 1u << i : 0u;
            }
        }
        list_append(pm != 0, u | (pm << kProbeShift), deferred, n_deferred);
    }
}

__device__ __forceinline__ int max4(int a, int b, int c, int d) { return max(max(a, b), max(c, d)); }

__device__ __forceinline__ u32 shr3(const u32 (&p)[3], int j, int k) {
    const int s = k >> 5;
    const u32 lo = j + s < 3 ? (s ? (j == 0 ? p[1] : p[2]) : p[j]) : 0u;
    const u32 hi = j + s + 1 < 3 ? (s ? p[2] : (j == 0 ? p[1] : p[2])) : 0u;
    return __funnelshift_r(lo, hi, k);
}
constexpr int kDecideThreads = 256;
__device__ __noinline__ bool mod4_level(const DevBatch& b, u32 pos, int wl, int k, int need, u32 pass8, u32 wv0, u32 wv1, u32 wv2, u32* cache,
                                        bool& cached) {
    const u32 wv[3] = {wv0, wv1, wv2};
    u32 p0[3][3], p1[3][3];
    if (!cached) {
        u32 x[3][3];
        load_bits<3>(b.hi, pos, x[0]); mask_bits<3>(x[0], wl);
        load_bits<3>(b.lo, pos, x[1]); mask_bits<3>(x[1], wl);
#pragma unroll
        for (int j = 0; j < 3; j++) x[2][j] = x[0][j] & x[1][j];
#pragma unroll
        for (int p = 0; p < 3; p++) {
            prefix_xor_excl<3>(x[p], p0[p]);
            u32 c[3];
#pragma unroll
            for (int j = 0; j < 3; j++) c[j] = x[p][j] & p0[p][j];
            prefix_xor_excl<3>(c, p1[p]);
#pragma unroll
            for (int j = 0; j < 3; j++) { cache[(6 * p + j) * kDecideThreads] = p0[p][j]; cache[(6 * p + 3 + j) * kDecideThreads] = p1[p][j]; }
        }
        cached = true;
    } else {
#pragma unroll
        for (int p = 0; p < 3; p++)
#pragma unroll
            for (int j = 0; j < 3; j++) { p0[p][j] = cache[(6 * p + j) * kDecideThreads]; p1[p][j] = cache[(6 * p + 3 + j) * kDecideThreads]; }
    }
    u32 d0[3][3], d1[3][3];
#pragma unroll
    for (int p = 0; p < 3; p++) {
#pragma unroll
        for (int j = 0; j < 3; j++) {
            const u32 q0 = shr3(p0[p], j, k);
            d0[p][j] = q0 ^ p0[p][j];
            d1[p][j] = shr3(p1[p], j, k) ^ p1[p][j] ^ (~q0 & p0[p][j]);
        }
    }
#pragma unroll 1
    for (int c2 = 0; c2 < 8; c2++) {
        if (!((pass8 >> c2) & 1u)) continue;
        u32 mw[3];
        int cnt = 0;
#pragma unroll
        for (int j = 0; j < 3; j++) {
            mw[j] = wv[j] & (d0[0][j] ^ ((c2 & 1) ? 0u : ~0u)) & (d0[1][j] ^ ((c2 & 2) ? 0u : ~0u)) & (d0[2][j] ^ ((c2 & 4) ? 0u : ~0u));
            cnt += __popc(mw[j]);
        }
        if (cnt < need) continue;
        bool may = true;
#pragma unroll
        for (int p = 0; p < 3 && may; p++) {
            const int one = __popc(mw[0] & d1[p][0]) + __popc(mw[1] & d1[p][1]) + __popc(mw[2] & d1[p][2]);
            const int zero = cnt - one;
            if (min(one, zero) >= need) return true;
            const u32 flip = one >= zero ? 0u : ~0u;
#pragma unroll
            for (int j = 0; j < 3; j++) mw[j] &= d1[p][j] ^ flip;
            cnt = max(one, zero);
            may = cnt >= need;
        }
        if (may) return true;
    }
    return false;
}

template <int S>
__device__ __forceinline__ bool decide_span(const u32 (&ph)[5], const u32 (&pl)[5], const u32 (&pa)[5], u32 (&wv)[3], int ka, int kb,
                                            const unsigned short* __restrict__ thr, bool& done, int& t_hit, const DevBatch& bt, u32 pos, int wl,
                                            u32* cache, bool& cached, int m4_below) {
    for (int k = ka; k <= kb; k++) {
        const int T01 = __popc(wv[0]) + __popc(wv[1]), E = __popc(wv[2]), T = T01 + E;
        if (T == 0) { done = true; return false; }
        const int need = thr[T];
        u32 a0 = (__funnelshift_r(ph[S], ph[S + 1], k) ^ ph[0]) & wv[0], a1 = (__funnelshift_r(ph[S + 1], ph[S + 2], k) ^ ph[1]) & wv[1];
        u32 b0 = (__funnelshift_r(pl[S], pl[S + 1], k) ^ pl[0]) & wv[0], b1 = (__funnelshift_r(pl[S + 1], pl[S + 2], k) ^ pl[1]) & wv[1];
        int cH = __popc(a0) + __popc(a1), cL = __popc(b0) + __popc(b1), c11 = __popc(a0 & b0) + __popc(a1 & b1);
        if (max4(c11, cH - c11, cL - c11, T01 - cH - cL + c11) + E >= need) {
            u32 a2 = (__funnelshift_r(ph[S + 2], ph[S + 3], k) ^ ph[2]) & wv[2], b2 = (__funnelshift_r(pl[S + 2], pl[S + 3], k) ^ pl[2]) & wv[2];
            cH += __popc(a2); cL += __popc(b2); c11 += __popc(a2 & b2);
            const int c10 = cH - c11, c01 = cL - c11, c00 = T - cH - cL + c11;
            if (max4(c11, c10, c01, c00) >= need) {
                u32 x0 = __funnelshift_r(pa[S], pa[S + 1], k) ^ pa[0], x1 = __funnelshift_r(pa[S + 1], pa[S + 2], k) ^ pa[1];
                u32 x2 = __funnelshift_r(pa[S + 2], pa[S + 3], k) ^ pa[2];
                int n11 = __popc(a0 & b0 & x0) + __popc(a1 & b1 & x1) + __popc(a2 & b2 & x2);
                int n10 = __popc(a0 & ~b0 & x0) + __popc(a1 & ~b1 & x1) + __popc(a2 & ~b2 & x2);
                int n01 = __popc(b0 & ~a0 & x0) + __popc(b1 & ~a1 & x1) + __popc(b2 & ~a2 & x2);
                int n00 = __popc(wv[0] & ~a0 & ~b0 & x0) + __popc(wv[1] & ~a1 & ~b1 & x1) + __popc(wv[2] & ~a2 & ~b2 & x2);
                int U2 = max(max4(n11, c11 - n11, n10, c10 - n10), max4(n01, c01 - n01, n00, c00 - n00));
                if (U2 >= need) {
                    const u32 pass8 = (u32)(c00 - n00 >= need) | (u32)(c10 - n10 >= need) << 1 | (u32)(c01 - n01 >= need) << 2 |
                                      (u32)(c11 - n11 >= need) << 3 | (u32)(n00 >= need) << 4 | (u32)(n10 >= need) << 5 |
                                      (u32)(n01 >= need) << 6 | (u32)(n11 >= need) << 7;
                    if (T >= m4_below || mod4_level(bt, pos, wl, k, need, pass8, wv[0], wv[1], wv[2], cache, cached)) { t_hit = T; return true; }
                }
            }
        }
        u32 t0 = __funnelshift_r(wv[0], wv[1], 1), t1 = __funnelshift_r(wv[1], wv[2], 1), t2 = wv[2] >> 1;
        wv[0] &= t0; wv[1] &= t1; wv[2] &= t2;
    }
    return false;
}

__device__ __noinline__ bool decide_short(const DevBatch& b, u32 pos, int wl, int k0, int k1, const unsigned short* __restrict__ thr, int& t_hit,
                                          u32* cache, int m4_below) {
    bool cached = false;
    u32 wv[3], ph[5], pl[5], pa[5];
    load_bits<3>(b.val, pos, wv); mask_bits<3>(wv, wl);
    {
        u32 h[3], l[3], q[3];
        load_bits<3>(b.hi, pos, h); mask_bits<3>(h, wl); prefix_xor_excl<3>(h, q);
        ph[0] = q[0]; ph[1] = q[1]; ph[2] = q[2]; ph[3] = 0u; ph[4] = 0u;
        load_bits<3>(b.lo, pos, l); mask_bits<3>(l, wl); prefix_xor_excl<3>(l, q);
        pl[0] = q[0]; pl[1] = q[1]; pl[2] = q[2]; pl[3] = 0u; pl[4] = 0u;
#pragma unroll
        for (int j = 0; j < 3; j++) h[j] &= l[j];
        prefix_xor_excl<3>(h, q);
        pa[0] = q[0]; pa[1] = q[1]; pa[2] = q[2]; pa[3] = 0u; pa[4] = 0u;
    }
    sliding_and<3>(wv, k0);
    bool done = false;
    if (k0 < 32) {
        if (decide_span<0>(ph, pl, pa, wv, k0, min(k1, 31), thr, done, t_hit, b, pos, wl, cache, cached, m4_below)) return true;
        if (done) return false;
        k0 = 32;
    }
    return k1 >= 32 && decide_span<1>(ph, pl, pa, wv, k0, k1, thr, done, t_hit, b, pos, wl, cache, cached, m4_below);
}

template <int MAXNW>
__global__ void __launch_bounds__(kDecideThreads, (MAXNW <= 5 ? 4 : 2)) trew_filter_kernel(DevCfg cfg, DevBatch b, const u32* __restrict__ units,
                                                          const u32* __restrict__ n_units_ptr, u32 n_units_all,
                                                          u32* __restrict__ survivors, u32* __restrict__ n_survivors,
                                                          u32* __restrict__ surv_b_top, u32* __restrict__ n_surv_b, int thread_min_windows, int third_level,
                                                          u32* __restrict__ work_counter) {
    __shared__ unsigned short thr[kThrTableSize];
    __shared__ u32 s_m4[18 * kDecideThreads];
    for (int i = threadIdx.x; i < kThrTableSize; i += blockDim.x) thr[i] = cfg.thr_low[i];
    __syncthreads();
    const u32 n_units = units ? *n_units_ptr : n_units_all;
    const bool pack_probes = n_units_all < (1u << kProbeShift);
    const u32 lane = lane_id();
    bool have = false, maybe = false, exhausted = false;
    u32 u = 0, live = 0, todo = 0;
    int t_hit = 1 << 20;
    Probe p[4];
    for (;;) {
        const u32 idle = __ballot_sync(0xffffffffu, !have);
        if (idle != 0u && !exhausted) {
            u32 base = 0;
            if (lane == 0) base = atomicAdd(work_counter, (u32)__popc(idle));
            base = __shfl_sync(0xffffffffu, base, 0);
            exhausted = base + (u32)__popc(idle) >= n_units;
            const u32 i = base + (u32)__popc(idle & ((1u << lane) - 1u));
            if (!have && i < n_units) {
                u32 pm = 0xfu;
                u = i;
                if (units) { const u32 e = units[i]; u = e & ((1u << kProbeShift) - 1u); pm = e >> kProbeShift; }
                const int np = unit_probes(cfg, b, u, p);
                live = todo = pm & ((1u << np) - 1u);
                maybe = false; t_hit = 1 << 20; have = true;
            }
        }
        if (__ballot_sync(0xffffffffu, have) == 0u) break;
        if (have && todo != 0u) {
            const int j = __ffs(todo) - 1;
            todo &= todo - 1u;
            if (p[j].k1 >= p[j].k0)
                maybe = probe_is_fast(p[j]) ? decide_short(b, p[j].pos, p[j].wl, p[j].k0, p[j].k1, thr, t_hit, s_m4 + threadIdx.x, third_level)
                                            : probe_dispatch<MAXNW>(b, p[j], thr);
            if (!maybe) live &= ~(1u << j);
        }
        const bool fin = have && (todo == 0u || maybe);
        const bool keep = fin && maybe;
        const u32 entry = pack_probes ? u | (live << kProbeShift) : u;
        if (surv_b_top == nullptr) {
            list_append(keep, entry, survivors, n_survivors);
        } else {
            bool to_b = false;
            if (keep) {
                int len;
                if (cfg.mode == 1) {
                    const u32 a0 = __ldg(b.bit_off + 2 * u), a1 = __ldg(b.bit_off + 2 * u + 1), a2 = __ldg(b.bit_off + 2 * u + 2);
                    len = (int)max(a1 - a0, a2 - a1);
                } else {
                    len = (int)(__ldg(b.bit_off + u + 1) - __ldg(b.bit_off + u));
                }
                to_b = len > et::kMaxRead || t_hit < thread_min_windows;
            }
            list_append(keep && !to_b, entry, survivors, n_survivors);
            list_append_rev(keep && to_b, entry, surv_b_top, n_surv_b);
        }
        if (fin) have = false;
    }
}

void launch_filter(const DevCfg& cfg, const DevBatch& b, unsigned int n_units, unsigned int max_read_len,
                   unsigned int* deferred, unsigned int* n_deferred, unsigned int* survivors, unsigned int* n_survivors,
                   const LaunchPlan& plan, cudaStream_t stream, cudaEvent_t after_screen, unsigned int* surv_b_top,
                   unsigned int* n_surv_b, unsigned int* work_counter) {
    if (n_units == 0) return;
    unsigned int longest;
    if (cfg.mode == 2) longest = 2u * (unsigned)cfg.slice_len;
    else longest = (max_read_len < 4u * (unsigned)cfg.max_mer) ? max_read_len : (max_read_len + 1) / 2;
    unsigned int need = (n_units + 255) / 256;
    const bool screen = deferred != nullptr && !(cfg.mode == 2 && cfg.slice_len > kFastMaxWlLong) && n_units < (1u << kProbeShift);
    if (screen) {
        int blocks = plan.screen_blocks;
        if ((unsigned)blocks > need) blocks = (int)need;
        if (longest <= (unsigned)kFastMaxWl) trew_screen_kernel<false><<<blocks, 256, 0, stream>>>(cfg, b, n_units, deferred, n_deferred);
        else trew_screen_kernel<true><<<blocks, 256, 0, stream>>>(cfg, b, n_units, deferred, n_deferred);
    }
    if (after_screen) cudaEventRecord(after_screen, stream);
    static const int tmw = [] { const char* e = getenv("TREW_THREAD_MIN_WINDOWS"); return e && *e ? atoi(e) : kThreadMinWindows; }();
    static const int m4_on = [] { const char* e = getenv("TREW_MOD4_BELOW"); return e && *e ? atoi(e) : kMod4BelowWindows; }();
    const unsigned int* list = screen ? deferred : nullptr;
    int blocks = plan.decide_blocks;
    if ((unsigned)blocks > need) blocks = (int)need;
    if (longest + 1 <= 96) trew_filter_kernel<3><<<blocks, 256, 0, stream>>>(cfg, b, list, n_deferred, n_units, survivors, n_survivors, surv_b_top, n_surv_b, tmw, m4_on, work_counter);
    else if (longest + 1 <= 160) trew_filter_kernel<5><<<blocks, 256, 0, stream>>>(cfg, b, list, n_deferred, n_units, survivors, n_survivors, surv_b_top, n_surv_b, tmw, m4_on, work_counter);
    else trew_filter_kernel<8><<<blocks, 256, 0, stream>>>(cfg, b, list, n_deferred, n_units, survivors, n_survivors, surv_b_top, n_surv_b, tmw, m4_on, work_counter);
}


extern __shared__ __align__(16) unsigned char g_smem[];

constexpr int kPlaneWords = 36;
#ifndef TREW_EXACT_BPS
#define TREW_EXACT_BPS 8
#endif
#ifndef TREW_EXACT_WARPS
#define TREW_EXACT_WARPS 4
#endif
constexpr int kExactWarps = TREW_EXACT_WARPS;
constexpr u32 kEmptySlot = 0xffffffffu;
constexpr int kSerialMaxRuns = 12;

enum { HD_CUR_POS = 0, HD_CUR_LEN, HD_ALLVALID, HD_EV_POS, HD_EV_LEN, HD_EV_K, HD_EV_PACK, HD_UNIT = 7 ,
       HD_S = 8 ,
       HD_BLK_L = 12 , HD_BLK_H = 14 , HD_NEED_L = 16, HD_NEED_H = 17, HD_BLK64 = 18, HD_RES = 19,
       HD_SH = 20 , HD_SL = 24 , HD_UNIT_BASE = 28 ,
       HD_RECS = 30  };
constexpr int kHeaderBytes = 128;

__host__ __device__ inline int exact_hash_slots(int cap) {
    int hs = 64;
    while (hs < cap + cap / 4) hs <<= 1;
    return hs;
}

__host__ __device__ inline size_t exact_warp_bytes(int cap) {
    size_t b = kHeaderBytes + 5 * kPlaneWords * sizeof(u32) + kPlaneWords * sizeof(u64);
    b += (size_t)2 * cap * sizeof(u64) + (size_t)exact_hash_slots(cap) * sizeof(u32) + (size_t)2 * cap * sizeof(u32);
    b += (size_t)(3 * cap + 4) * sizeof(unsigned short);
    return (b + 15) & ~(size_t)15;
}

size_t exact_smem_bytes(int run_cap, bool) { return exact_warp_bytes(run_cap) * kExactWarps; }

struct WS {
    u32 off; int cap; int hs; u32 lane; u32 flags;
    __device__ __forceinline__ u32* hdr() const { return (u32*)(g_smem + off); }
    __device__ __forceinline__ u32* H() const { return (u32*)(g_smem + off + kHeaderBytes); }
    __device__ __forceinline__ u32* L() const { return H() + kPlaneWords; }
    __device__ __forceinline__ u32* V() const { return H() + 2 * kPlaneWords; }
    __device__ __forceinline__ u32* PH() const { return H() + 3 * kPlaneWords; }
    __device__ __forceinline__ u32* PL() const { return H() + 4 * kPlaneWords; }
    __device__ __forceinline__ u64* rev2() const { return (u64*)(H() + 5 * kPlaneWords); }
    __device__ __forceinline__ u64* run_lo() const { return rev2() + kPlaneWords; }
    __device__ __forceinline__ u64* run_hi() const { return run_lo() + cap; }
    __device__ __forceinline__ u32* htab() const { return (u32*)(run_hi() + cap); }
    __device__ __forceinline__ u32* grp_tot() const { return htab() + hs; }
    __device__ __forceinline__ u32* grp_last() const { return grp_tot() + cap; }
    __device__ __forceinline__ unsigned short* run_start() const { return (unsigned short*)(grp_last() + cap); }
    __device__ __forceinline__ unsigned short* run_cw() const { return run_start() + cap; }
    __device__ __forceinline__ unsigned short* run_total() const { return run_cw() + cap + 4; }
};

struct TableRef { Slot* slots; u32 mask; u32* err; };

struct ScanRes { int th, tl; u64 sh_lo, sh_hi, sl_lo, sl_hi; };

__device__ __forceinline__ int pk_T(u32 p) { return (int)(p & 1023u); }
__device__ __forceinline__ int pk_M(u32 p) { return (int)((p >> 10) & 1023u); }
__device__ __forceinline__ int pk_runs(u32 p) { return (int)((p >> 20) & 1023u); }
__device__ __forceinline__ bool pk_homo(u32 p) { return ((p >> 30) & 1u) != 0; }


__device__ __noinline__ u64 canon64(u64 w, int k) {
    int sh = 2 * (k - 1);
    if (k <= 16) {
        u32 b32 = (u32)w, c32 = (u32)w;
        for (int r = 1; r < k; r++) {
            c32 = ((c32 & 3u) << sh) | (c32 >> 2);
            b32 = min(b32, c32);
        }
        return b32;
    }
    u64 best = w, cur = w;
    for (int r = 1; r < k; r++) {
        cur = ((cur & 3ULL) << sh) | (cur >> 2);
        best = cur < best ? cur : best;
    }
    return best;
}

__device__ __noinline__ u128 canon128(u128 w, int k) {
    u128 best = w, cur = w;
    int sh = 2 * (k - 1);
    for (int r = 1; r < k; r++) {
        cur = ((cur & 3) << sh) | (cur >> 2);
        best = cur < best ? cur : best;
    }
    return best;
}

__device__ __forceinline__ u64 rev_pairs64(u64 x) {
    x = __brevll(x);
    return ((x >> 1) & 0x5555555555555555ULL) | ((x & 0x5555555555555555ULL) << 1);
}

__device__ __forceinline__ void canon_pair(u64& lo, u64& hi, int k) {
    if (k <= 32) { lo = canon64(lo, k); hi = 0; }
    else { u128 c = canon128(((u128)hi << 64) | lo, k); lo = (u64)c; hi = (u64)(c >> 64); }
}

__device__ __forceinline__ void crc_pair(u64& lo, u64& hi, int k) {
    if (k <= 32) {
        u64 r = ~rev_pairs64(lo) >> (64 - 2 * k);
        lo = canon64(r, k); hi = 0;
    } else {
        u128 r = ((u128)(~rev_pairs64(lo)) << 64) | (u128)(~rev_pairs64(hi));
        r >>= (128 - 2 * k);
        u128 c = canon128(r, k); lo = (u64)c; hi = (u64)(c >> 64);
    }
}

__device__ __forceinline__ bool homo_pair(u64 lo, u64 hi, int k) {
    if (k <= 1) return true;
    if (k <= 32) return ((lo ^ (lo >> 2)) & ((1ULL << (2 * (k - 1))) - 1ULL)) == 0;
    u128 w = ((u128)hi << 64) | lo;
    u128 m = (((u128)1 << (2 * (k - 1))) - 1);
    return ((w ^ (w >> 2)) & m) == 0;
}

__device__ __forceinline__ bool less_pair(u64 alo, u64 ahi, u64 blo, u64 bhi) {
    return ahi < bhi || (ahi == bhi && alo < blo);
}

__device__ __forceinline__ u32 shfl_next_bit0(u32 x, u32 lane) {
    u32 nx = __shfl_down_sync(0xffffffffu, x, 1);
    return lane == 31 ? 0u : (nx & 1u);
}


__device__ __noinline__ void load_window(WS ws, const u32* __restrict__ bhi, const u32* __restrict__ blo,
                                         const u32* __restrict__ bval, u32 pos, int len) {
    u32* hd = ws.hdr();
    if ((int)hd[HD_CUR_LEN] == len && hd[HD_CUR_POS] == pos) return;
    __syncwarp();
    const u32 lane = ws.lane;
    int vbits = len - 32 * (int)lane;
    u32 msk = vbits <= 0 ? 0u : low_mask(vbits);
    u32 h = 0, l = 0, v = 0;
    if (vbits > 0) {
        u32 wi = (pos >> 5) + lane, sh = pos & 31;
        h = __funnelshift_r(__ldg(bhi + wi), __ldg(bhi + wi + 1), sh) & msk;
        l = __funnelshift_r(__ldg(blo + wi), __ldg(blo + wi + 1), sh) & msk;
        v = __funnelshift_r(__ldg(bval + wi), __ldg(bval + wi + 1), sh) & msk;
    }
    const bool all_valid = __all_sync(0xffffffffu, v == msk);
    u32 ih = prefix_xor32(h), il = prefix_xor32(l);
    u32 bh = __ballot_sync(0xffffffffu, ih >> 31), bl = __ballot_sync(0xffffffffu, il >> 31);
    u32 lt = (1u << lane) - 1u;
    if (__popc(bh & lt) & 1) ih = ~ih;
    if (__popc(bl & lt) & 1) il = ~il;
    u32 ph_prev = __shfl_up_sync(0xffffffffu, ih, 1), pl_prev = __shfl_up_sync(0xffffffffu, il, 1);
    u32 ph = (ih << 1) | (lane ? ph_prev >> 31 : 0u);
    u32 pl = (il << 1) | (lane ? pl_prev >> 31 : 0u);
    u32 *H = ws.H(), *L = ws.L(), *V = ws.V(), *PH = ws.PH(), *PL = ws.PL();
    u64* rev2 = ws.rev2();
    H[lane] = h; L[lane] = l; V[lane] = v; PH[lane] = ph; PL[lane] = pl;
    if (lane < kPlaneWords - 32) {
        H[32 + lane] = 0; L[32 + lane] = 0; V[32 + lane] = 0; PH[32 + lane] = 0; PL[32 + lane] = 0;
        rev2[32 + lane] = 0;
    }
    __syncwarp();
    {
        int cs = len - 32 * (int)lane - 32;
        u32 hb = 0, lb = 0;
        if (cs > -32) {
            if (cs >= 0) {
                int wi = cs >> 5, sh = cs & 31;
                hb = __funnelshift_r(H[wi], H[wi + 1], sh);
                lb = __funnelshift_r(L[wi], L[wi + 1], sh);
            } else {
                hb = H[0] << (-cs);
                lb = L[0] << (-cs);
            }
        }
        hb = __brev(hb); lb = __brev(lb);
        u64 x = hb, y = lb;
        x = (x | (x << 16)) & 0x0000FFFF0000FFFFULL; y = (y | (y << 16)) & 0x0000FFFF0000FFFFULL;
        x = (x | (x << 8)) & 0x00FF00FF00FF00FFULL;  y = (y | (y << 8)) & 0x00FF00FF00FF00FFULL;
        x = (x | (x << 4)) & 0x0F0F0F0F0F0F0F0FULL;  y = (y | (y << 4)) & 0x0F0F0F0F0F0F0F0FULL;
        x = (x | (x << 2)) & 0x3333333333333333ULL;  y = (y | (y << 2)) & 0x3333333333333333ULL;
        x = (x | (x << 1)) & 0x5555555555555555ULL;  y = (y | (y << 1)) & 0x5555555555555555ULL;
        rev2[lane] = (x << 1) | y;
    }
    if (lane == 0) { hd[HD_CUR_POS] = pos; hd[HD_CUR_LEN] = (u32)len; hd[HD_ALLVALID] = all_valid ? 1u : 0u; }
    __syncwarp();
}

__device__ __forceinline__ void kmer_at(const u64* __restrict__ rev2, int len, int i, int k, u64& lo, u64& hi) {
    int o = 2 * (len - i - k);
    int wi = o >> 6, sh = o & 63;
    u64 a = rev2[wi], b = rev2[wi + 1];
    lo = sh ? (a >> sh) | (b << (64 - sh)) : a;
    if (k <= 32) {
        if (k < 32) lo &= (1ULL << (2 * k)) - 1ULL;
        hi = 0;
    } else {
        u64 c = rev2[wi + 2];
        hi = sh ? (b >> sh) | (c << (64 - sh)) : b;
        if (k < 64) hi &= (1ULL << (2 * k - 64)) - 1ULL;
    }
}

__device__ __forceinline__ u32 wv_for_k(WS ws, int len, int k) {
    const u32 lane = ws.lane;
    if (ws.hdr()[HD_ALLVALID]) {
        int vb = len - k + 1 - 32 * (int)lane;
        return vb <= 0 ? 0u : low_mask(min(32, vb));
    }
    u32 wv = ws.V()[lane];
    for (int t = 1; t < k; t++) {
        u32 nb = shfl_next_bit0(wv, lane);
        wv &= (wv >> 1) | (nb << 31);
    }
    return wv;
}

__device__ __forceinline__ u32 wv_step(u32 wv, u32 lane) {
    u32 nb = shfl_next_bit0(wv, lane);
    return wv & ((wv >> 1) | (nb << 31));
}

__device__ __forceinline__ int bound_k(WS ws, int k, u32 wv, int T) {
    const u32 lane = ws.lane;
    const u32 *PH = ws.PH(), *PL = ws.PL();
    int s = k >> 5, r = k & 31;
    u32 qh = __funnelshift_r(PH[lane + s], PH[lane + s + 1], r);
    u32 ql = __funnelshift_r(PL[lane + s], PL[lane + s + 1], r);
    u32 dh = (qh ^ PH[lane]) & wv, dl = (ql ^ PL[lane]) & wv;
    u32 packed = (u32)__popc(dh) | ((u32)__popc(dl) << 10) | ((u32)__popc(dh & dl) << 20);
    packed = __reduce_add_sync(0xffffffffu, packed);
    int cH = packed & 1023, cL = (packed >> 10) & 1023, c11 = packed >> 20;
    int c10 = cH - c11, c01 = cL - c11, c00 = T - cH - cL + c11;
    return max(max(c00, c01), max(c10, c11));
}

__device__ __noinline__ int comp_bound(WS ws, int k, u32 wv, int T) {
    const u32 lane = ws.lane;
    const u32 cnt = (u32)__popc(wv);
    u32 inc = cnt;
#pragma unroll
    for (int d = 1; d < 32; d <<= 1) {
        u32 t = __shfl_up_sync(0xffffffffu, inc, d);
        if ((int)lane >= d) inc += t;
    }
    unsigned short* pos = ws.run_start();
    {
        u32 rb = inc - cnt, x = wv;
        while (x) {
            int bit = __ffs(x) - 1;
            x &= x - 1;
            pos[rb++] = (unsigned short)(32 * lane + bit);
        }
    }
    __syncwarp();
    const bool act = (int)lane < T;
    u32 key = 0;
    if (act) {
        const u32 *H = ws.H(), *L = ws.L();
        const int p = pos[lane], w0 = p >> 5, o = p & 31;
        const u32 m0 = low_mask(min(k, 32)), m1 = k <= 32 ? 0u : low_mask(k - 32);
        const u32 h0 = __funnelshift_r(H[w0], H[w0 + 1], o) & m0, h1 = __funnelshift_r(H[w0 + 1], H[w0 + 2], o) & m1;
        const u32 l0 = __funnelshift_r(L[w0], L[w0 + 1], o) & m0, l1 = __funnelshift_r(L[w0 + 1], L[w0 + 2], o) & m1;
        key = (u32)(__popc(h0) + __popc(h1)) | ((u32)(__popc(l0) + __popc(l1)) << 8) | ((u32)(__popc(h0 & l0) + __popc(h1 & l1)) << 16);
    }
    const u32 actm = __ballot_sync(0xffffffffu, act);
    const u32 same = __match_any_sync(0xffffffffu, key) & actm;
    const u32 best = __reduce_max_sync(0xffffffffu, act ? (u32)__popc(same) : 0u);
    __syncwarp();
    return (int)best;
}

__device__ __noinline__ u32 eval_k(WS ws, int len, int k, u32 wv) {
    const u32 lane = ws.lane;
    u32* hd = ws.hdr();
    const u32 *H = ws.H(), *L = ws.L();
    int s = k >> 5, r = k & 31;
    u32 hs = __funnelshift_r(H[lane + s], H[lane + s + 1], r);
    u32 ls = __funnelshift_r(L[lane + s], L[lane + s + 1], r);
    u32 eq = ~((hs ^ H[lane]) | (ls ^ L[lane]));
    u32 nb = shfl_next_bit0(wv, lane);
    u32 link = eq & wv & ((wv >> 1) | (nb << 31));
    u32 link_prev = __shfl_up_sync(0xffffffffu, link, 1);
    u32 rs = wv & ~((link << 1) | (lane ? link_prev >> 31 : 0u));
    u32 pk = (u32)__popc(wv) | ((u32)__popc(rs) << 16);
    const u32 tot_pk = __reduce_add_sync(0xffffffffu, pk);
    const int T = (int)(tot_pk & 0xffffu), R = (int)(tot_pk >> 16);
    if (T == 0) return 0u;
    unsigned short *run_start = ws.run_start(), *run_cw = ws.run_cw(), *run_total = ws.run_total();
    u64 *run_lo = ws.run_lo(), *run_hi = ws.run_hi();
    u32 *htab = ws.htab(), *grp_tot = ws.grp_tot(), *grp_last = ws.grp_last();
    const u64* rev2 = ws.rev2();
    const bool wide = k > 32;
    if (!wide && R <= kSerialMaxRuns && (ws.flags & 1u)) {
        u32* scr = htab;
        scr[lane] = wv; scr[32 + lane] = link; scr[64 + lane] = rs;
        __syncwarp();
        unsigned short* cls_last = run_cw;
        int ncls = 0, ord = 0;
// ... 285 lines not shown
        int T = (int)__reduce_add_sync(0xffffffffu, (u32)__popc(wv));
        if (T == 0) break;
        int U = bound_k(ws, k, wv, T);
        try_k(ws, thr_low, low, high, pos, len, k, U, T, wv);
    }
    return hd[HD_RES];
}

__device__ __forceinline__ ScanRes scan_stats(WS ws, const DevBatch& b, u32 pos, int len, int kmin, int kmax, const DevCfg& cfg) {
    const u32 r = scan_core(ws, b, pos, len, kmin, kmax, cfg.thr_low, cfg.low, cfg.high);
    const u32* hd = ws.hdr();
    ScanRes res;
    res.th = (int)(r & 0xffu); res.tl = (int)(r >> 8);
    res.sh_lo = (u64)hd[HD_SH] | ((u64)hd[HD_SH + 1] << 32); res.sh_hi = (u64)hd[HD_SH + 2] | ((u64)hd[HD_SH + 3] << 32);
    res.sl_lo = (u64)hd[HD_SL] | ((u64)hd[HD_SL + 1] << 32); res.sl_hi = (u64)hd[HD_SL + 2] | ((u64)hd[HD_SL + 3] << 32);
    return res;
}

__device__ __noinline__ u32 eval_cached(WS ws, DevBatch b, u32 pos, int len, int k) {
    u32* hd = ws.hdr();
    if ((int)hd[HD_EV_K] == k && hd[HD_EV_POS] == pos && (int)hd[HD_EV_LEN] == len) return hd[HD_EV_PACK];
    load_window(ws, b.hi, b.lo, b.val, pos, len);
    u32 wv = wv_for_k(ws, len, k);
    u32 ev = eval_k(ws, len, k, wv);
    if (ws.lane == 0) { hd[HD_EV_POS] = pos; hd[HD_EV_LEN] = (u32)len; hd[HD_EV_K] = (u32)k; hd[HD_EV_PACK] = ev; }
    __syncwarp();
    return ev;
}

template <bool REC>
__device__ void emit_window(TableRef tr, WS ws, const DevBatch& b, u32 pos, int len, int k, int table, bool folded) {
    u32 ev = eval_cached(ws, b, pos, len, k);
    emit_classes<REC>(tr, ws, k, pk_runs(ev), table, folded);
}

template <bool REC>
__device__ void target_window(TableRef tr, WS ws, const DevBatch& b, u32 pos, int len, int k, const unsigned short* thr_low, bool high, int table) {
    u32 ev = eval_cached(ws, b, pos, len, k);
    if (pk_T(ev) > 0 && !pk_homo(ev) && pk_M(ev) >= thr_at(ws, thr_low, high, pk_T(ev))) emit_classes<REC>(tr, ws, k, pk_runs(ev), table, true);
}


enum { T_F = 0, T_B = 2, T_O = 4 };

template <bool REC>
__device__ void route_short(const DevCfg& cfg, TableRef tr, WS ws, const DevBatch& b, u32 u, u32 pm) {
    const int MINM = cfg.min_mer, MAXM = cfg.max_mer;
    u32 b0 = __ldg(b.bit_off + u);
    int n = (int)(__ldg(b.bit_off + u + 1) - b0);
    if (n < 2 * MINM || n > kMaxWindow) return;
    int L[2] = {0, 0}, R[2] = {0, 0};
    if (n >= 4 * MINM) {
        int kmax = min(n / 4, MAXM);
        u32 lpos = b0, rpos = b0 + (u32)(n - (n + 1) / 2);
        int llen = n / 2, rlen = (n + 1) / 2;
        if (pm & 1u) { ScanRes l = scan_stats(ws, b, lpos, llen, MINM, kmax, cfg); L[0] = l.th; L[1] = l.tl; }
        if (pm & 2u) { ScanRes r = scan_stats(ws, b, rpos, rlen, MINM, kmax, cfg); R[0] = r.th; R[1] = r.tl; }
        pm >>= 2;
#pragma unroll
        for (int c = 0; c < 2; c++) {
            if (L[c] > 0 && L[c] == R[c]) target_window<REC>(tr, ws, b, b0, n, L[c], cfg.thr_low, c == 0, T_O + c);
            else if (L[c] > 0) emit_window<REC>(tr, ws, b, lpos, llen, L[c], T_F + c, false);
            else if (R[c] > 0) emit_window<REC>(tr, ws, b, rpos, rlen, R[c], T_B + c, false);
        }
    }
    bool hc[2] = {L[0] == 0 && R[0] == 0, L[1] == 0 && R[1] == 0};
    if (4 * MAXM > n && (hc[0] || hc[1]) && (pm & 1u)) {
        ScanRes s = scan_stats(ws, b, b0, n, max(n / 4 + 1, MINM), min(n / 2, MAXM), cfg);
        if (hc[0] && s.th) emit_window<REC>(tr, ws, b, b0, n, s.th, T_O + 0, false);
        if (hc[1] && s.tl) emit_window<REC>(tr, ws, b, b0, n, s.tl, T_O + 1, false);
    }
}

template <bool REC>
__device__ void route_pair(const DevCfg& cfg, TableRef tr, WS ws, const DevBatch& b, u32 u) {
    const int MINM = cfg.min_mer, MAXM = cfg.max_mer;
    u32 a0 = __ldg(b.bit_off + 2 * u), a1 = __ldg(b.bit_off + 2 * u + 1), a2 = __ldg(b.bit_off + 2 * u + 2);
    int n1 = (int)(a1 - a0), n2 = (int)(a2 - a1);
    int n = min(n1, n2);
    if (n < 2 * MINM || n1 > kMaxWindow || n2 > kMaxWindow) return;
    int lef[2] = {0, 0}, km[2] = {0, 0};
    if (n >= 4 * MINM) {
        u32 spos[5] = {0, a0, a0 + (u32)(n1 - (n1 + 1) / 2), a1 + (u32)(n2 - (n2 + 1) / 2), a1};
        int slen[5] = {0, n1 / 2, (n1 + 1) / 2, (n2 + 1) / 2, n2 / 2};
        int kmax = min(n / 4, MAXM);
        ScanRes sr[5]; bool have[5] = {false, false, false, false, false};
        int pseg[2][8], ptmp[2][8], np[2] = {0, 0};
        int si[2] = {1, 1}; bool ended[2] = {false, false};
        u64 ks_lo[2] = {0, 0}, ks_hi[2] = {0, 0};
        for (int ti = 1; ti <= 4 && !(ended[0] && ended[1]); ti++) {
            if (!have[ti]) { sr[ti] = scan_stats(ws, b, spos[ti], slen[ti], MINM, kmax, cfg); have[ti] = true; }
            int k[2] = {sr[ti].th, sr[ti].tl};
            u64 slo[2] = {sr[ti].sh_lo, sr[ti].sl_lo}, shi[2] = {sr[ti].sh_hi, sr[ti].sl_hi};
#pragma unroll
            for (int c = 0; c < 2; c++) {
                if (!ended[c] && k[c]) { pseg[c][np[c]] = ti; ptmp[c][np[c]] = ti <= 2 ? 0 : 1; np[c]++; }
                bool ok = !ended[c] && k[c] > 0;
                if (ok && ti != 1) {
                    u64 dlo = slo[c], dhi = shi[c];
                    if (ti > 2) crc_pair(dlo, dhi, k[c]);
                    ok = km[c] == k[c] && ks_lo[c] == dlo && ks_hi[c] == dhi;
                }
                if (ok) { si[c]++; km[c] = k[c]; if (ti == 1) { ks_lo[c] = slo[c]; ks_hi[c] = shi[c]; } }
                else ended[c] = true;
            }
        }
        lef[0] = km[0]; lef[1] = km[1];
#pragma unroll
        for (int c = 0; c < 2; c++) {
            if (si[c] == 5) {
                for (int e = 0; e < np[c]; e++) {
                    int sg = pseg[c][e];
                    emit_window<REC>(tr, ws, b, spos[sg], slen[sg], c == 0 ? sr[sg].th : sr[sg].tl, T_O + c, true);
                }
            }
        }
        if (si[0] <= 4 || si[1] <= 4) {
            int sj[2] = {4, 4}; km[0] = km[1] = 0; ended[0] = ended[1] = false;
            for (int tj = 4; tj >= 1 && !(ended[0] && ended[1]); tj--) {
                if (!have[tj]) { sr[tj] = scan_stats(ws, b, spos[tj], slen[tj], MINM, kmax, cfg); have[tj] = true; }
                int k[2] = {sr[tj].th, sr[tj].tl};
                u64 slo[2] = {sr[tj].sh_lo, sr[tj].sl_lo}, shi[2] = {sr[tj].sh_hi, sr[tj].sl_hi};
#pragma unroll
                for (int c = 0; c < 2; c++) {
                    if (!ended[c] && k[c]) { pseg[c][np[c]] = tj; ptmp[c][np[c]] = tj <= 2 ? 1 : 0; np[c]++; }
                    bool ok = sj[c] >= si[c] && !ended[c] && k[c] > 0;
                    if (ok && tj != 4) {
                        u64 dlo = slo[c], dhi = shi[c];
                        if (tj <= 2) crc_pair(dlo, dhi, k[c]);
                        ok = km[c] == k[c] && ks_lo[c] == dlo && ks_hi[c] == dhi;
                    }
                    if (ok) { sj[c]--; km[c] = k[c]; if (tj == 4) { ks_lo[c] = slo[c]; ks_hi[c] = shi[c]; } }
                    else ended[c] = true;
                }
            }
        }
#pragma unroll
        for (int c = 0; c < 2; c++) {
            if (si[c] <= 4) {
                for (int e = 0; e < np[c]; e++) {
                    int sg = pseg[c][e];
                    emit_window<REC>(tr, ws, b, spos[sg], slen[sg], c == 0 ? sr[sg].th : sr[sg].tl,
                                (ptmp[c][e] == 0 ? T_F : T_B) + c, false);
                }
            }
        }
    }
    if (4 * MAXM > n && (lef[0] == 0 || lef[1] == 0 || km[0] == 0 || km[1] == 0)) {
        int lo = max(n / 4 + 1, MINM), hi = min(n / 2, MAXM);
        ScanRes l, r; l.th = l.tl = r.th = r.tl = 0; l.sh_lo = l.sh_hi = l.sl_lo = l.sl_hi = 0; r = l;
        if (lef[0] == 0 || lef[1] == 0) l = scan_stats(ws, b, a0, n1, lo, hi, cfg);
        if (km[0] == 0 || km[1] == 0) r = scan_stats(ws, b, a1, n2, lo, hi, cfg);
        int ltk[2] = {l.th, l.tl}, rtk[2] = {r.th, r.tl};
        u64 llo[2] = {l.sh_lo, l.sl_lo}, lhi[2] = {l.sh_hi, l.sl_hi}, rlo[2] = {r.sh_lo, r.sl_lo}, rhi[2] = {r.sh_hi, r.sl_hi};
#pragma unroll
        for (int c = 0; c < 2; c++) {
            bool el = lef[c] == 0 && ltk[c] > 0, er = km[c] == 0 && rtk[c] > 0;
            bool both = lef[c] == 0 && km[c] == 0 && ltk[c] == rtk[c] && ltk[c] > 0;
            if (both) {
                u64 dlo = rlo[c], dhi = rhi[c];
                crc_pair(dlo, dhi, rtk[c]);
                both = llo[c] == dlo && lhi[c] == dhi;
            }
            if (both) {
                if (el) emit_window<REC>(tr, ws, b, a0, n1, ltk[c], T_O + c, true);
                if (er) emit_window<REC>(tr, ws, b, a1, n2, rtk[c], T_O + c, true);
            }
            if (el) emit_window<REC>(tr, ws, b, a0, n1, ltk[c], T_F + c, false);
            if (er) emit_window<REC>(tr, ws, b, a1, n2, rtk[c], T_F + c, false);
        }
    }
}

template <bool REC>
__device__ void route_long(const DevCfg& cfg, TableRef tr, WS ws, const DevBatch& b, u32 u, unsigned char* scratch) {
    const int MINM = cfg.min_mer, MAXM = cfg.max_mer, SL = cfg.slice_len;
    u32 b0 = __ldg(b.bit_off + u);
    int n = (int)(__ldg(b.bit_off + u + 1) - b0);
    if (n < SL) return;
    int snum = n / SL, mid = (snum + 1) / 2, bonus = n % SL;
    auto s_start = [&](int t) { return (u32)((t - 1) * SL + (t > mid ? bonus : 0)); };
    auto s_len = [&](int t) { return SL + (t == mid ? bonus : 0); };
    int si[2] = {1, 1}, km[2] = {0, 0}; bool ended[2] = {false, false};
    int nf = 0;
    for (int ti = 1; ti <= snum && !(ended[0] && ended[1]); ti++) {
        ScanRes sr = scan_stats(ws, b, b0 + s_start(ti), s_len(ti), MINM, MAXM, cfg);
        if (ws.lane == 0) { scratch[2 * (ti - 1)] = (unsigned char)sr.th; scratch[2 * (ti - 1) + 1] = (unsigned char)sr.tl; }
        int k[2] = {sr.th, sr.tl};
#pragma unroll
        for (int c = 0; c < 2; c++) {
            if (!ended[c] && k[c] > 0 && (ti == 1 || km[c] == k[c])) { si[c]++; km[c] = k[c]; }
            else ended[c] = true;
        }
        nf = ti;
    }
    __syncwarp();
    {
        bool en[2] = {false, false}; int kk[2] = {0, 0};
        bool full[2] = {si[0] == snum + 1, si[1] == snum + 1};
        for (int ti = 1; ti <= nf; ti++) {
            int k[2] = {scratch[2 * (ti - 1)], scratch[2 * (ti - 1) + 1]};
#pragma unroll
            for (int c = 0; c < 2; c++) {
                if (!en[c] && k[c]) emit_window<REC>(tr, ws, b, b0 + s_start(ti), s_len(ti), k[c], (full[c] ? T_O : T_F) + c, full[c]);
                if (!en[c] && k[c] > 0 && (ti == 1 || kk[c] == k[c])) kk[c] = k[c];
                else en[c] = true;
            }
        }
    }
    if (si[0] <= snum || si[1] <= snum) {
        int sj[2] = {snum, snum}; km[0] = km[1] = 0; ended[0] = ended[1] = false;
        for (int tj = snum; tj >= 1 && !(ended[0] && ended[1]); tj--) {
            ScanRes sr = scan_stats(ws, b, b0 + s_start(tj), s_len(tj), MINM, MAXM, cfg);
            int k[2] = {sr.th, sr.tl};
#pragma unroll
            for (int c = 0; c < 2; c++) {
                if (!ended[c] && k[c]) emit_window<REC>(tr, ws, b, b0 + s_start(tj), s_len(tj), k[c], T_B + c, false);
                if (sj[c] >= si[c] && !ended[c] && k[c] > 0 && (tj == snum || km[c] == k[c])) { sj[c]--; km[c] = k[c]; }
                else ended[c] = true;
            }
        }
    }
}


constexpr int kStageSlots = 256;
constexpr int kStageProbes = 6;
constexpr u32 kStageLock = 0xffffffffu;

struct StageEmit {
    u32* s_meta; u32* s_cnt; u64* s_key;
    Slot* slots; u32 mask; u32* err;
    __device__ __forceinline__ void operator()(int table, int k, et::u128 key, u64 count) const {
        const u64 hi = (u64)(key >> 64);
        if (hi) table_add_impl(slots, mask, err, ((u32)table << 8) | (u32)k, (u64)key, hi, count);
        else (*this)(table, k, (et::u64)key, count);
    }
    __device__ __forceinline__ void operator()(int table, int k, et::u64 key_, u64 count) const {
        const u64 key = (u64)key_;
        const u32 meta = ((u32)table << 8) | (u32)k, tag = meta | 0x80000000u;
        u32 i = (u32)(mix64(key ^ ((u64)meta << 53)) >> 40) & (kStageSlots - 1);
        bool done = false;
        for (int p = 0; p < kStageProbes && !done; p++, i = (i + 1) & (kStageSlots - 1)) {
            int outcome = 0;
            do {
                const u32 st = atomicCAS(&s_meta[i], 0u, kStageLock);
                if (st == 0u) {
                    s_key[i] = key;
                    __threadfence_block();
                    atomicExch(&s_meta[i], tag);
                    atomicAdd(&s_cnt[i], (u32)count);
                    outcome = 1;
                } else if (st != kStageLock) {
                    __threadfence_block();
                    if (st == tag && *(volatile u64*)&s_key[i] == key) { atomicAdd(&s_cnt[i], (u32)count); outcome = 1; }
                    else outcome = 2;
                }
            } while (outcome == 0);
            done = outcome == 1;
        }
        if (!done) table_add_impl(slots, mask, err, meta, key, 0ULL, count);
    }
};

struct RecStageEmit {
    StageEmit add; UnitRecs* recs; u64 unit;
    __device__ __forceinline__ void operator()(int table, int k, et::u128 key, u64 count) const {
        add(table, k, key, count);
        rec_append(recs, unit, table, k, (u64)key, (u64)(key >> 64), count);
    }
    __device__ __forceinline__ void operator()(int table, int k, et::u64 key, u64 count) const {
        add(table, k, key, count);
        rec_append(recs, unit, table, k, (u64)key, 0ULL, count);
    }
};

#ifndef TREW_THREAD_BLOCK
#define TREW_THREAD_BLOCK 128
#endif
template <class K>
constexpr size_t thread_kernel_smem() { return (size_t)et::Lay<K>::WORDS * TREW_THREAD_BLOCK * sizeof(u32) + (size_t)kStageSlots * 16; }
constexpr size_t kThreadKernelSmem = thread_kernel_smem<et::u64>();
template <int MODE, class K>
constexpr int thread_kernel_bps() { return (sizeof(K) == 8 ? 6 : 5) - (MODE == 1 ? 1 : 0); }

struct PlaneLoad {
    et::Mem m; const u32 *hi, *lo, *val; u32 b0[2];
    __device__ __forceinline__ void operator()(int mate, int off, int len) const {
        const u32 pos = b0[mate] + (u32)off, w0 = pos >> 5, sh = pos & 31u;
        for (int j = 0; j < et::kReadWords + 2; j++) {
            const u32 msk = low_mask(min(32, max(0, len - 32 * j)));
            u32 h = 0u, l = 0u;
            if (msk) {
                h = __funnelshift_r(__ldg(hi + w0 + j), __ldg(hi + w0 + j + 1), sh) & msk;
                l = __funnelshift_r(__ldg(lo + w0 + j), __ldg(lo + w0 + j + 1), sh) & msk;
            }
            m[et::W_H + j] = h; m[et::W_L + j] = l;
            if (j < et::kReadWords) m[et::W_V + j] = msk ? __funnelshift_r(__ldg(val + w0 + j), __ldg(val + w0 + j + 1), sh) & msk : 0u;
        }
    }
};

template <int MODE, class K, bool REC>
__global__ void __launch_bounds__(TREW_THREAD_BLOCK, (thread_kernel_bps<MODE, K>())) trew_exact_thread_kernel(DevCfg cfg, DevBatch b, const u32* __restrict__ survivors,
                                                                              const u32* __restrict__ n_survivors, int packed_probes,
                                                                              u32* __restrict__ hard, u32* __restrict__ n_hard,
                                                                              unsigned long long* total_survivors, u32* work_counter) {
    u32* work = reinterpret_cast<u32*>(g_smem);
    u64* s_key = reinterpret_cast<u64*>(work + et::Lay<K>::WORDS * TREW_THREAD_BLOCK);
    u32* s_meta = reinterpret_cast<u32*>(s_key + kStageSlots);
    u32* s_cnt = s_meta + kStageSlots;
    for (int i = threadIdx.x; i < kStageSlots; i += blockDim.x) { s_meta[i] = 0u; s_cnt[i] = 0u; }
    __syncthreads();
    const et::Mem m{work + threadIdx.x, TREW_THREAD_BLOCK};
    const u32 n = *n_survivors;
    if (blockIdx.x == 0 && threadIdx.x == 0 && total_survivors) atomicAdd(total_survivors, (unsigned long long)n);
    StageEmit emit{s_meta, s_cnt, s_key, cfg.slots, cfg.slot_mask, cfg.error_flag};
    for (;;) {
        u32 base = 0;
        if (lane_id() == 0) base = atomicAdd(work_counter, 32u);
        base = __shfl_sync(0xffffffffu, base, 0);
        if (base >= n) break;
        const u32 i = base + lane_id();
        bool bail = false;
        u32 entry = 0;
        if (i < n) {
            entry = survivors[i];
            u32 u = entry, pm = 3u;
            if (packed_probes) { pm = entry >> kProbeShift; u &= (1u << kProbeShift) - 1u; }
            auto route = [&](auto& em) {
                if (MODE == 0) {
                    const u32 b0 = __ldg(b.bit_off + u);
                    const int len = (int)(__ldg(b.bit_off + u + 1) - b0);
                    if (len > et::kMaxRead) return false;
                    PlaneLoad load{m, b.hi, b.lo, b.val, {b0, 0u}};
                    return et::route_short_thread<K>(m, len, pm & 7u, cfg.min_mer, cfg.max_mer, cfg.thr_low, cfg.thr_high, load, em);
                }
                const u32 a0 = __ldg(b.bit_off + 2 * u), a1 = __ldg(b.bit_off + 2 * u + 1), a2 = __ldg(b.bit_off + 2 * u + 2);
                const int n1 = (int)(a1 - a0), n2 = (int)(a2 - a1);
                PlaneLoad load{m, b.hi, b.lo, b.val, {a0, a1}};
                return et::route_pair_thread<K>(m, n1, n2, cfg.min_mer, cfg.max_mer, cfg.thr_low, cfg.thr_high, load, em);
            };
            if constexpr (REC) {
                RecStageEmit rem{emit, cfg.recs, cfg.unit_base + u};
                bail = !route(rem);
            } else {
                bail = !route(emit);
            }
        }
        list_append(bail, entry, hard, n_hard);
    }
    __syncthreads();
    for (int i = threadIdx.x; i < kStageSlots; i += blockDim.x) {
        const u32 st = s_meta[i], c = s_cnt[i];
        if (st != 0u && st != kStageLock && c != 0u) table_add_impl(cfg.slots, cfg.slot_mask, cfg.error_flag, st & 0x7fffffffu, s_key[i], 0ULL, (u64)c);
    }
}


struct LongArgs {
    const u32* survivors; const u32* n_survivors; int packed_probes;
    u32 s_cap, max_slices;
    unsigned short* stats; u32* emis;
    u32* hard; u32* n_hard;
    unsigned long long* total_survivors;
};

__global__ void __launch_bounds__(TREW_THREAD_BLOCK, 4) trew_long_stats_kernel(DevCfg cfg, DevBatch b, LongArgs a) {
    u32* work = reinterpret_cast<u32*>(g_smem);
    const et::Mem m{work + threadIdx.x, TREW_THREAD_BLOCK};
    const u32 n = min(*a.n_survivors, a.s_cap);
    const u32 warps = gridDim.x * (blockDim.x >> 5), lane = lane_id();
    et::ClsSpill<et::u64> x;
    for (u32 idx = blockIdx.x * (blockDim.x >> 5) + (threadIdx.x >> 5); idx < n; idx += warps) {
        u32 u = a.survivors[idx];
        if (a.packed_probes) u &= (1u << kProbeShift) - 1u;
        const u32 b0 = __ldg(b.bit_off + u);
        const int len = (int)(__ldg(b.bit_off + u + 1) - b0);
        if (len < cfg.slice_len) continue;
        const et::LongGeom g(len, cfg.slice_len);
        PlaneLoad load{m, b.hi, b.lo, b.val, {b0, 0u}};
        unsigned short* row = a.stats + (size_t)idx * (a.max_slices + 1);
        for (int t = 1 + (int)lane; t <= g.snum; t += 32) {
            u32 r = 0;
            if (g.len(t) <= et::kMaxRead) r = et::long_slice_stats(m, g, t, cfg.min_mer, cfg.max_mer, cfg.thr_low, cfg.thr_high, load, x);
            row[t] = (unsigned short)r;
        }
    }
}

__global__ void __launch_bounds__(256) trew_long_walk_kernel(DevCfg cfg, DevBatch b, LongArgs a) {
    const u32 n_all = *a.n_survivors;
    if (blockIdx.x == 0 && threadIdx.x == 0 && a.total_survivors) atomicAdd(a.total_survivors, (unsigned long long)n_all);
    const u32 stride = gridDim.x * blockDim.x, n_round = (n_all + 31u) & ~31u;
    for (u32 idx = blockIdx.x * blockDim.x + threadIdx.x; idx < n_round; idx += stride) {
        bool bail = false;
        u32 entry = 0;
        if (idx < n_all) {
            entry = a.survivors[idx];
            u32 u = entry;
            if (a.packed_probes) u &= (1u << kProbeShift) - 1u;
            const int len = (int)(__ldg(b.bit_off + u + 1) - __ldg(b.bit_off + u));
            if (idx >= a.s_cap) bail = len >= cfg.slice_len;
            else if (len >= cfg.slice_len) {
                const et::LongGeom g(len, cfg.slice_len);
                const unsigned short* row = a.stats + (size_t)idx * (a.max_slices + 1);
                u32* em = a.emis + (size_t)idx * (a.max_slices + 1);
                for (int t = 1; t <= g.snum; t++) em[t] = 0u;
                auto stat = [&](int t) { return (u32)row[t]; };
                auto task = [&](const et::LongTask& tk) {
                    const int tb = tk.table_folded & 7, c = tb & 1;
                    const bool backward = (tb & 6) == et::T_B;
                    const u32 byte = (u32)tk.k | ((tk.table_folded & 8) ? 0x80u : 0u);
                    em[tk.slice] |= byte << (8 * ((backward ? 2 : 0) + c));
                };
                bail = !et::long_walk(g, stat, task);
                if (bail) for (int t = 1; t <= g.snum; t++) em[t] = 0u;
            }
        }
        list_append(bail, entry, a.hard, a.n_hard);
    }
}

template <bool REC>
__global__ void __launch_bounds__(TREW_THREAD_BLOCK, 4) trew_long_emit_kernel(DevCfg cfg, DevBatch b, LongArgs a) {
    u32* work = reinterpret_cast<u32*>(g_smem);
    u64* s_key = reinterpret_cast<u64*>(work + et::Lay<et::u64>::WORDS * TREW_THREAD_BLOCK);
    u32* s_meta = reinterpret_cast<u32*>(s_key + kStageSlots);
    u32* s_cnt = s_meta + kStageSlots;
    for (int i = threadIdx.x; i < kStageSlots; i += blockDim.x) { s_meta[i] = 0u; s_cnt[i] = 0u; }
    __syncthreads();
    const et::Mem m{work + threadIdx.x, TREW_THREAD_BLOCK};
    StageEmit emit{s_meta, s_cnt, s_key, cfg.slots, cfg.slot_mask, cfg.error_flag};
    const u32 n = min(*a.n_survivors, a.s_cap);
    const u32 warps = gridDim.x * (blockDim.x >> 5), lane = lane_id();
    et::ClsSpill<et::u64> x;
    for (u32 idx = blockIdx.x * (blockDim.x >> 5) + (threadIdx.x >> 5); idx < n; idx += warps) {
        u32 u = a.survivors[idx];
        if (a.packed_probes) u &= (1u << kProbeShift) - 1u;
        const u32 b0 = __ldg(b.bit_off + u);
        const int len = (int)(__ldg(b.bit_off + u + 1) - b0);
        if (len < cfg.slice_len) continue;
        const et::LongGeom g(len, cfg.slice_len);
        PlaneLoad load{m, b.hi, b.lo, b.val, {b0, 0u}};
        const u32* em = a.emis + (size_t)idx * (a.max_slices + 1);
        for (int t = 1 + (int)lane; t <= g.snum; t += 32) {
            const u32 e = em[t];
            if (e == 0u) continue;
            for (int f = 0; f < 4; f++) {
                const u32 byte = (e >> (8 * f)) & 0xffu;
                if (byte == 0u) continue;
                const int c = f & 1;
                const bool folded = (byte & 0x80u) != 0u;
                const int table = (f >= 2 ? et::T_B : (folded ? et::T_O : et::T_F)) + c;
                et::LongTask tk{(unsigned short)t, (unsigned char)(byte & 0x7fu), (unsigned char)(table | (folded ? 8 : 0))};
                if constexpr (REC) {
                    RecStageEmit rem{emit, cfg.recs, cfg.unit_base + u};
                    et::long_emit(m, g, tk, load, x, rem);
                } else {
                    et::long_emit(m, g, tk, load, x, emit);
                }
            }
        }
    }
    __syncthreads();
    for (int i = threadIdx.x; i < kStageSlots; i += blockDim.x) {
        const u32 st = s_meta[i], c = s_cnt[i];
        if (st != 0u && st != kStageLock && c != 0u) table_add_impl(cfg.slots, cfg.slot_mask, cfg.error_flag, st & 0x7fffffffu, s_key[i], 0ULL, (u64)c);
    }
}

bool long_thread_path_applies(const DevCfg& cfg) { return cfg.mode == 2 && cfg.max_mer <= 32 && cfg.slice_len <= et::kMaxRead; }

size_t long_thread_scratch_bytes(unsigned int s_cap, unsigned int max_slices) {
    return (size_t)s_cap * (max_slices + 1) * (sizeof(unsigned short) + sizeof(u32)) + 64;
}

void launch_long_thread(const DevCfg& cfg, const DevBatch& b, const unsigned int* survivors, const unsigned int* n_survivors,
                        int packed_probes, unsigned int s_cap, unsigned int max_slices, unsigned char* scratch, unsigned int* hard,
                        unsigned int* n_hard, unsigned long long* total_survivors, int sm_count, cudaStream_t stream) {
    LongArgs a{};
    a.survivors = survivors; a.n_survivors = n_survivors; a.packed_probes = packed_probes;
    a.s_cap = s_cap; a.max_slices = max_slices;
    a.emis = reinterpret_cast<u32*>(scratch);
    a.stats = reinterpret_cast<unsigned short*>(scratch + (size_t)s_cap * (max_slices + 1) * sizeof(u32));
    a.hard = hard; a.n_hard = n_hard; a.total_survivors = total_survivors;
    const size_t smem_stats = (size_t)et::Lay<et::u64>::WORDS * TREW_THREAD_BLOCK * sizeof(u32);
    trew_long_stats_kernel<<<sm_count * 4, TREW_THREAD_BLOCK, smem_stats, stream>>>(cfg, b, a);
    trew_long_walk_kernel<<<sm_count * 2, 256, 0, stream>>>(cfg, b, a);
    if (cfg.recs) trew_long_emit_kernel<true><<<sm_count * 4, TREW_THREAD_BLOCK, kThreadKernelSmem, stream>>>(cfg, b, a);
    else trew_long_emit_kernel<false><<<sm_count * 4, TREW_THREAD_BLOCK, kThreadKernelSmem, stream>>>(cfg, b, a);
}

bool thread_path_applies(const DevCfg& cfg, unsigned int max_read_len) {
    if (cfg.max_mer > 64) return false;
    if (cfg.mode == 0) return true;
    return cfg.mode == 1 && max_read_len >= 4u * (unsigned)cfg.max_mer;
}

void launch_exact_thread(const DevCfg& cfg, const DevBatch& b, const unsigned int* survivors, const unsigned int* n_survivors,
                         int packed_probes, unsigned int* hard, unsigned int* n_hard, unsigned long long* total_survivors, int sm_count,
                         int blocks_per_sm, unsigned int* work_counter, cudaStream_t stream) {
    const bool wide = cfg.max_mer > 32;
#define TREW_LAUNCH_THREAD(MODE, K, REC)                                                                                          \
    trew_exact_thread_kernel<MODE, K, REC><<<sm_count * (blocks_per_sm > 0 ? blocks_per_sm : thread_kernel_bps<MODE, K>()),       \
                                             TREW_THREAD_BLOCK, thread_kernel_smem<K>(), stream>>>(                               \
        cfg, b, survivors, n_survivors, packed_probes, hard, n_hard, total_survivors, work_counter)
#define TREW_LAUNCH_THREAD_MODE(MODE)                                                                                             \
    if (cfg.recs) { if (wide) TREW_LAUNCH_THREAD(MODE, et::u128, true); else TREW_LAUNCH_THREAD(MODE, et::u64, true); }            \
    else          { if (wide) TREW_LAUNCH_THREAD(MODE, et::u128, false); else TREW_LAUNCH_THREAD(MODE, et::u64, false); }
    if (cfg.mode == 0) { TREW_LAUNCH_THREAD_MODE(0) }
    else               { TREW_LAUNCH_THREAD_MODE(1) }
#undef TREW_LAUNCH_THREAD_MODE
#undef TREW_LAUNCH_THREAD
}

template <int MODE, bool REC>
__global__ void __launch_bounds__(kExactWarps * 32, TREW_EXACT_BPS) trew_exact_kernel(DevCfg cfg, DevBatch b, ExactArgs a) {
    const int wid = threadIdx.x >> 5;
    const u32 lane = lane_id();
    WS ws;
    ws.cap = a.run_cap; ws.hs = exact_hash_slots(a.run_cap);
    ws.off = (u32)((size_t)wid * exact_warp_bytes(a.run_cap)); ws.lane = lane; ws.flags = a.exp_flags;
    TableRef tr{cfg.slots, cfg.slot_mask, cfg.error_flag};
    ws.hdr()[lane] = lane == HD_CUR_LEN || lane == HD_EV_LEN || lane == HD_EV_K ? 0xffffffffu : 0u;
    if constexpr (REC) {
        if (lane == HD_UNIT_BASE) { ws.hdr()[lane] = (u32)cfg.unit_base; ws.hdr()[lane + 1] = (u32)(cfg.unit_base >> 32); }
        if (lane == HD_RECS) { ws.hdr()[lane] = (u32)(u64)cfg.recs; ws.hdr()[lane + 1] = (u32)((u64)cfg.recs >> 32); }
    }
    __syncwarp();
    const u32 n = *a.n_survivors;
    if (blockIdx.x == 0 && threadIdx.x == 0 && a.total_survivors) atomicAdd(a.total_survivors, (u64)n);
    unsigned char* scratch = a.slice_scratch + (size_t)(blockIdx.x * kExactWarps + wid) * a.slice_scratch_stride;
    for (;;) {
        u32 idx = 0;
        if (lane == 0) idx = atomicAdd(a.work_counter, 1u);
        idx = __shfl_sync(0xffffffffu, idx, 0);
        if (idx >= n) break;
        u32 u = a.reverse ? *(a.survivors - idx) : a.survivors[idx], pm = 0xfu;
        if (a.packed_probes) { pm = u >> kProbeShift; u &= (1u << kProbeShift) - 1u; }
        if constexpr (REC) ws.hdr()[HD_UNIT] = u;
        if constexpr (MODE == 0) route_short<REC>(cfg, tr, ws, b, u, pm);
        else if constexpr (MODE == 1) route_pair<REC>(cfg, tr, ws, b, u);
        else route_long<REC>(cfg, tr, ws, b, u, scratch);
    }
}

constexpr int kExactBlocksPerSM = TREW_EXACT_BPS;
int exact_warps_total(int sm_count) { return sm_count * kExactBlocksPerSM * kExactWarps; }

cudaError_t prepare_exact(int run_cap_max) {
    int bytes = (int)exact_smem_bytes(run_cap_max, true);
    cudaError_t e = cudaSuccess;
#define TREW_SMEM_ATTR(F, BYTES) if (e == cudaSuccess) e = cudaFuncSetAttribute(F, cudaFuncAttributeMaxDynamicSharedMemorySize, (int)(BYTES))
    TREW_SMEM_ATTR((trew_exact_kernel<0, false>), bytes);
    TREW_SMEM_ATTR((trew_exact_kernel<1, false>), bytes);
    TREW_SMEM_ATTR((trew_exact_kernel<2, false>), bytes);
    TREW_SMEM_ATTR((trew_exact_kernel<0, true>), bytes);
    TREW_SMEM_ATTR((trew_exact_kernel<1, true>), bytes);
    TREW_SMEM_ATTR((trew_exact_kernel<2, true>), bytes);
    TREW_SMEM_ATTR((trew_exact_thread_kernel<0, et::u64, false>), thread_kernel_smem<et::u64>());
    TREW_SMEM_ATTR((trew_exact_thread_kernel<1, et::u64, false>), thread_kernel_smem<et::u64>());
    TREW_SMEM_ATTR((trew_exact_thread_kernel<0, et::u128, false>), thread_kernel_smem<et::u128>());
    TREW_SMEM_ATTR((trew_exact_thread_kernel<1, et::u128, false>), thread_kernel_smem<et::u128>());
    TREW_SMEM_ATTR((trew_exact_thread_kernel<0, et::u64, true>), thread_kernel_smem<et::u64>());
    TREW_SMEM_ATTR((trew_exact_thread_kernel<1, et::u64, true>), thread_kernel_smem<et::u64>());
    TREW_SMEM_ATTR((trew_exact_thread_kernel<0, et::u128, true>), thread_kernel_smem<et::u128>());
    TREW_SMEM_ATTR((trew_exact_thread_kernel<1, et::u128, true>), thread_kernel_smem<et::u128>());
    TREW_SMEM_ATTR(trew_long_stats_kernel, kThreadKernelSmem);
    TREW_SMEM_ATTR(trew_long_emit_kernel<false>, kThreadKernelSmem);
    TREW_SMEM_ATTR(trew_long_emit_kernel<true>, kThreadKernelSmem);
#undef TREW_SMEM_ATTR
    return e;
}

LaunchPlan default_launch_plan(int sm_count) { return LaunchPlan{sm_count * 128, sm_count * 4, sm_count * kExactBlocksPerSM}; }

void launch_exact(const DevCfg& cfg, const DevBatch& b, const ExactArgs& a, const LaunchPlan& plan, cudaStream_t stream) {
    size_t smem = exact_smem_bytes(a.run_cap, true);
    dim3 grid(plan.exact_blocks), block(kExactWarps * 32);
    if (cfg.recs) {
        if (cfg.mode == 0) trew_exact_kernel<0, true><<<grid, block, smem, stream>>>(cfg, b, a);
        else if (cfg.mode == 1) trew_exact_kernel<1, true><<<grid, block, smem, stream>>>(cfg, b, a);
        else trew_exact_kernel<2, true><<<grid, block, smem, stream>>>(cfg, b, a);
    } else {
        if (cfg.mode == 0) trew_exact_kernel<0, false><<<grid, block, smem, stream>>>(cfg, b, a);
        else if (cfg.mode == 1) trew_exact_kernel<1, false><<<grid, block, smem, stream>>>(cfg, b, a);
        else trew_exact_kernel<2, false><<<grid, block, smem, stream>>>(cfg, b, a);
    }
}

}
```

trew_b200/csrc/scan_kernels.cuh:

```cuda
#pragma once
#include <cstdint>
#include <cuda_runtime.h>

#include "../../include/trew_b200.h"

namespace trew {

constexpr int kThrTableSize = 1025;
constexpr int kMaxWindow = 1023;

struct __align__(32) Slot {
    unsigned long long seq_lo;
    unsigned long long seq_hi;
    unsigned long long count;
    unsigned int meta;
    unsigned int state;
};

struct UnitRecs {
    trew_unit_record* buf;
    unsigned long long cap;
    unsigned long long n;
};

struct DevCfg {
    int mode, min_mer, max_mer, slice_len;
    double low, high;
    Slot* slots;
    unsigned int slot_mask;
    unsigned int* error_flag;
    const unsigned short* thr_low;
    const unsigned short* thr_high;
    UnitRecs* recs;
    unsigned long long unit_base;
};

struct DevBatch {
    unsigned int n_reads;
    const unsigned int* bit_off;
    const unsigned int* hi;
    const unsigned int* lo;
    const unsigned int* val;
};

struct ExactArgs {
    const unsigned int* survivors;
    const unsigned int* n_survivors;
    unsigned int* work_counter;
    unsigned char* slice_scratch;
    unsigned int slice_scratch_stride;
    int run_cap;
    unsigned long long* total_survivors;
    int packed_probes;
    int reverse;
    unsigned int exp_flags;
};

struct LaunchPlan { int screen_blocks, decide_blocks, exact_blocks; };
LaunchPlan default_launch_plan(int sm_count);

void launch_filter(const DevCfg& cfg, const DevBatch& b, unsigned int n_units, unsigned int max_read_len,
                   unsigned int* deferred, unsigned int* n_deferred, unsigned int* survivors, unsigned int* n_survivors,
                   const LaunchPlan& plan, cudaStream_t stream, cudaEvent_t after_screen,
                   unsigned int* surv_b_top, unsigned int* n_surv_b, unsigned int* work_counter);
size_t exact_smem_bytes(int run_cap, bool wide);
cudaError_t prepare_exact(int run_cap_max);
void launch_exact(const DevCfg& cfg, const DevBatch& b, const ExactArgs& a, const LaunchPlan& plan, cudaStream_t stream);
int exact_warps_total(int sm_count);
bool long_thread_path_applies(const DevCfg& cfg);
size_t long_thread_scratch_bytes(unsigned int s_cap, unsigned int max_slices);
void launch_long_thread(const DevCfg& cfg, const DevBatch& b, const unsigned int* survivors, const unsigned int* n_survivors,
                        int packed_probes, unsigned int s_cap, unsigned int max_slices, unsigned char* scratch, unsigned int* hard,
                        unsigned int* n_hard, unsigned long long* total_survivors, int sm_count, cudaStream_t stream);
bool thread_path_applies(const DevCfg& cfg, unsigned int max_read_len);
void launch_exact_thread(const DevCfg& cfg, const DevBatch& b, const unsigned int* survivors, const unsigned int* n_survivors,
                         int packed_probes, unsigned int* hard, unsigned int* n_hard, unsigned long long* total_survivors, int sm_count,
                         int blocks_per_sm, unsigned int* work_counter, cudaStream_t stream);
void launch_compact(const Slot* slots, unsigned int n_slots, trew_entry* out, unsigned int* d_n, cudaStream_t stream, unsigned int cap);
cudaError_t sort_entries_radix(const trew_entry* d_entries, trew_entry* d_out, unsigned int n, bool wide, void* d_temp,
                               size_t* temp_bytes, cudaStream_t stream);
cudaError_t combine_sorted_rows(const trew_entry* d_sorted, unsigned int n, trew_entry* d_out, unsigned int* d_n_out, void* d_temp,
                                size_t* temp_bytes, cudaStream_t stream);
cudaError_t filter_report_rows(const trew_entry* d_rows, unsigned int n, unsigned int min_total, trew_entry* d_out, unsigned int* d_n_out,
                               void* d_temp, size_t* temp_bytes, cudaStream_t stream);
void launch_clear_invalid(unsigned int* val, const unsigned int* rec, unsigned int n, cudaStream_t stream);
void launch_merge_entries(const DevCfg& cfg, const trew_entry* entries, unsigned int n, cudaStream_t stream);

cudaError_t sort_combine_records(const trew_unit_record* d_in, unsigned int n, bool wide, trew_unit_record* d_out, unsigned int* d_n_out,
                                 void* d_temp, size_t* temp_bytes, cudaStream_t stream);

void launch_synth(unsigned long long seed, unsigned int n_reads, unsigned int read_len, unsigned int tel_thr,
                  unsigned int half_thr, unsigned int n_thr, unsigned int sub_thr, unsigned int flavor, unsigned int* bit_off,
                  unsigned int* hi, unsigned int* lo, unsigned int* val, size_t plane_words, cudaStream_t stream);

}
```

Measured before the change: 1036.

## Batch decide and exact stages across up to sixteen screened resident batches

```diff
diff --git a/trew_b200/csrc/device_ctx.cu b/trew_b200/csrc/device_ctx.cu
--- a/trew_b200/csrc/device_ctx.cu
+++ b/trew_b200/csrc/device_ctx.cu
@@ -80,8 +80,10 @@
     uint32_t n_reads = 0, n_units = 0, max_read_len = 0;
     uint64_t bases = 0;
     ScanBufs scan;
-    cudaEvent_t ev[4] = {nullptr, nullptr, nullptr, nullptr};
+    cudaEvent_t ev[5] = {};
     bool ev_pending = false;
+    bool stage_events = false;
+    StageBatch entry{};
 };
 
 struct trew_ctx {
@@ -124,6 +126,9 @@
     cudaEvent_t ev_t0 = nullptr, ev_t1 = nullptr;
     double screen_ms = 0, decide_ms = 0, exact_ms = 0; uint64_t n_prof_scans = 0;
     std::vector<trew_resident*> pending_prof;
+    std::vector<trew_resident*> pending;
+    int stage_key = 0;
+    uint32_t stage_len = 0;
     Buf<trew_entry, true> h_export;
     unsigned int report_min = 0;
     Buf<trew_entry> d_filtered;
@@ -193,52 +198,76 @@
     return v;
 }
 
-int launch_scan(trew_ctx* ctx, const DevBatch& b, uint32_t n_units, uint32_t max_read_len, ScanBufs& sb, cudaStream_t st,
-                cudaEvent_t* ev = nullptr) {
+bool thread_path_for(const trew_ctx* ctx, uint32_t max_read_len, uint32_t n_units) {
+    return thread_path_applies(ctx->dcfg, max_read_len) && !(ctx->exact_flags & 4u) && n_units < (1u << 28);
+}
+
+int stage_key_for(const trew_ctx* ctx, uint32_t max_read_len, uint32_t n_units) {
+    return decide_variant(ctx->dcfg, max_read_len) * 2 + (thread_path_for(ctx, max_read_len, n_units) ? 1 : 0);
+}
+
+int screen_batch(trew_ctx* ctx, const DevBatch& b, uint32_t n_units, uint32_t max_read_len, ScanBufs& sb, cudaStream_t st,
+                 cudaEvent_t* ev, StageBatch* out) {
+    ctx->export_valid = false;
+    ctx->table_used = true;
+    StageBatch& e = *out;
+    e = StageBatch{};
+    e.b = b; e.survivors = sb.survivors.p; e.counters = sb.counters.p; e.n_units = n_units;
+    e.unit_base = ctx->unit_next;
+    ctx->unit_next += n_units;
+    CK(cudaMemsetAsync(sb.counters.p, 0, kScanCounters * sizeof(unsigned int), st));
+    if (ev) CK(cudaEventRecord(ev[0], st));
+    e.screened = launch_screen(ctx->dcfg, b, n_units, max_read_len, sb.survivors.p + n_units, sb.counters.p + 2, ctx->plan, st) ? 1 : 0;
+    if (ev) CK(cudaEventRecord(ev[1], st));
+    CK(cudaGetLastError());
+    ctx->stats.kernel_launches += 1;
+    return TREW_OK;
+}
+
+int run_stage(trew_ctx* ctx, const StageTable& t, uint32_t max_read_len, ScanBufs& sb, cudaStream_t st, cudaEvent_t* ev) {
+    unsigned long long units = 0;
+    for (int i = 0; i < t.n; i++) units += t.e[i].n_units;
     unsigned int stride, s_cap, max_slices;
     size_t long_off;
-    CK(sb.scratch.grow(scratch_need(ctx, max_read_len, n_units, &stride, &long_off, &s_cap, &max_slices), st));
-    unsigned int* d_survivors = sb.survivors.p;
-    unsigned int* d_counters = sb.counters.p;
-    ctx->export_valid = false;
-    ctx->table_used = true;
-    DevCfg cfg = ctx->dcfg;
-    cfg.unit_base = ctx->unit_next;
-    ctx->unit_next += n_units;
-    CK(cudaMemsetAsync(d_counters, 0, kScanCounters * sizeof(unsigned int), st));
+    CK(sb.scratch.grow(scratch_need(ctx, max_read_len, (uint32_t)std::min<unsigned long long>(units, 0xffffffffULL), &stride, &long_off,
+                                    &s_cap, &max_slices), st));
+    const StageBatch& e0 = t.e[0];
+    const bool thread_path = thread_path_for(ctx, max_read_len, e0.n_units);
     if (ev) CK(cudaEventRecord(ev[0], st));
-    const bool thread_path = thread_path_applies(cfg, max_read_len) && !(ctx->exact_flags & 4u) && n_units < (1u << 28);
-    launch_filter(cfg, b, n_units, max_read_len, d_survivors + n_units, d_counters + 2, d_survivors, d_counters, ctx->plan, st,
-                  ev ? ev[1] : nullptr, thread_path ? d_survivors + n_units - 1 : nullptr, thread_path ? d_counters + 4 : nullptr,
-                  d_counters + 7);
-    if (ev) CK(cudaEventRecord(ev[2], st));
+    launch_decide(ctx->dcfg, t, max_read_len, units, thread_path, ctx->plan, st);
+    if (ev) CK(cudaEventRecord(ev[1], st));
     ExactArgs a{};
-    a.survivors = d_survivors; a.n_survivors = d_counters; a.work_counter = d_counters + 1;
+    a.list = LIST_A; a.work_counter = e0.counters + 1;
     a.slice_scratch = sb.scratch.p; a.slice_scratch_stride = stride; a.run_cap = run_cap_for(ctx->cfg, max_read_len);
     a.total_survivors = ctx->d_total_surv.p;
-    a.packed_probes = n_units < (1u << 28) ? 1 : 0;
     a.exp_flags = ctx->exact_flags;
     if (thread_path) {
-        unsigned int* hard = d_survivors + n_units;
-        launch_exact_thread(cfg, b, d_survivors, d_counters, a.packed_probes, hard, d_counters + 3, ctx->d_total_surv.p,
-                            ctx->sm_count, env_blocks_thread(), d_counters + 6, st);
+        launch_exact_thread(ctx->dcfg, t, ctx->d_total_surv.p, ctx->sm_count, env_blocks_thread(), st);
         ExactArgs ab = a;
-        ab.survivors = d_survivors + n_units - 1; ab.reverse = 1; ab.n_survivors = d_counters + 4;
-        launch_exact(cfg, b, ab, ctx->plan, st);
-        a.survivors = hard; a.n_survivors = d_counters + 3; a.work_counter = d_counters + 5; a.total_survivors = nullptr;
+        ab.list = LIST_B;
+        launch_exact(ctx->dcfg, t, ab, ctx->plan, st);
+        a.list = LIST_BAILS; a.work_counter = e0.counters + 5; a.total_survivors = nullptr;
         ctx->stats.kernel_launches += 2;
-    } else if (s_cap > 0 && n_units < (1u << 28)) {
-        unsigned int* hard = d_survivors + n_units;
-        launch_long_thread(cfg, b, d_survivors, d_counters, a.packed_probes, s_cap, max_slices, sb.scratch.p + long_off, hard,
-                           d_counters + 3, ctx->d_total_surv.p, ctx->sm_count, st);
-        a.survivors = hard; a.n_survivors = d_counters + 3; a.total_survivors = nullptr;
+    } else if (s_cap > 0 && e0.n_units < (1u << 28)) {
+        DevCfg cfg = ctx->dcfg;
+        cfg.unit_base = e0.unit_base;
+        launch_long_thread(cfg, e0.b, e0.survivors, e0.counters + LIST_A, 1, s_cap, max_slices, sb.scratch.p + long_off,
+                           e0.survivors + e0.n_units, e0.counters + LIST_BAILS, ctx->d_total_surv.p, ctx->sm_count, st);
+        a.list = LIST_BAILS; a.total_survivors = nullptr;
         ctx->stats.kernel_launches += 3;
     }
-    launch_exact(cfg, b, a, ctx->plan, st);
-    if (ev) CK(cudaEventRecord(ev[3], st));
+    launch_exact(ctx->dcfg, t, a, ctx->plan, st);
+    if (ev) CK(cudaEventRecord(ev[2], st));
     CK(cudaGetLastError());
-    ctx->stats.kernel_launches += 3;
-    return TREW_OK;
+    ctx->stats.kernel_launches += 2;
+    return TREW_OK;
+}
+
+int launch_scan(trew_ctx* ctx, const DevBatch& b, uint32_t n_units, uint32_t max_read_len, ScanBufs& sb, cudaStream_t st) {
+    StageTable t{};
+    t.n = 1;
+    int rc = screen_batch(ctx, b, n_units, max_read_len, sb, st, nullptr, &t.e[0]);
+    return rc ? rc : run_stage(ctx, t, max_read_len, sb, st, nullptr);
 }
 
 int retire_slot(trew_ctx* ctx, SlotRes& s) {
@@ -254,6 +283,7 @@
 
 int export_entries(trew_ctx* ctx, bool need_sorted, const trew_entry** out, uint64_t* n_out);
 int check_device_error(trew_ctx* ctx);
+int flush_stage(trew_ctx* ctx);
 
 int grow_table_to(trew_ctx* ctx, size_t min_slots) {
     size_t new_slots = ctx->n_slots;
@@ -323,6 +353,7 @@
     for (int i = 0; i < n_ranges; i++) { total_bases += rg[i].bases; max_len = std::max(max_len, rg[i].max_len); }
     const uint32_t n = n_ranges ? rg[n_ranges - 1].r1 - rg[0].r0 : 0u;
     if (n == 0) return TREW_OK;
+    if (int rc0 = flush_stage(ctx)) return rc0;
     SlotRes& s = ctx->slots[ctx->next_slot];
     ctx->next_slot = (ctx->next_slot + 1) % ctx->slots.size();
     static const bool trace = getenv("TREW_SUBMIT_TRACE") != nullptr;
@@ -472,16 +503,20 @@
 }
 
 int collect_prof(trew_ctx* ctx) {
+    if (int rc = flush_stage(ctx)) return rc;
     for (trew_resident* r : ctx->pending_prof) {
         if (!r->ev_pending) continue;
-        CK(cudaEventSynchronize(r->ev[3]));
+        CK(cudaEventSynchronize(r->ev[r->stage_events ? 4 : 1]));
         float a = 0, b = 0, c = 0;
         CK(cudaEventElapsedTime(&a, r->ev[0], r->ev[1]));
-        CK(cudaEventElapsedTime(&b, r->ev[1], r->ev[2]));
-        CK(cudaEventElapsedTime(&c, r->ev[2], r->ev[3]));
+        if (r->stage_events) {
+            CK(cudaEventElapsedTime(&b, r->ev[2], r->ev[3]));
+            CK(cudaEventElapsedTime(&c, r->ev[3], r->ev[4]));
+        }
         ctx->screen_ms += a; ctx->decide_ms += b; ctx->exact_ms += c; ctx->n_prof_scans++;
         ctx->stats.device_ms += a + b + c;
         r->ev_pending = false;
+        r->stage_events = false;
     }
     ctx->pending_prof.clear();
     return TREW_OK;
@@ -498,6 +533,21 @@
     if (ctx->resident_streams != 2) return TREW_OK;
     CK(cudaEventRecord(ctx->ev_join, ctx->main_stream));
     CK(cudaStreamWaitEvent(ctx->aux_stream, ctx->ev_join, 0));
+    return TREW_OK;
+}
+
+int flush_stage(trew_ctx* ctx) {
+    if (ctx->pending.empty()) return TREW_OK;
+    if (int rc = join_aux(ctx)) return rc;
+    StageTable t{};
+    for (trew_resident* r : ctx->pending) t.e[t.n++] = r->entry;
+    trew_resident* first = ctx->pending.front();
+    trew_resident* last = ctx->pending.back();
+    ctx->pending.clear();
+    last->stage_events = true;
+    int rc = run_stage(ctx, t, ctx->stage_len, first->scan, ctx->main_stream, last->ev + 2);
+    if (rc) return rc;
+    CK(cudaEventRecord(ctx->ev_b, ctx->main_stream));
     return TREW_OK;
 }
 
@@ -722,6 +772,7 @@
     size_t bytes = batch_bytes(n, bases);
     if (bytes > ctx->staging_bytes || n > ctx->slots[0].survivors_cap)
         return fail(ctx, TREW_ERR_ARG, "packed batch (%zu bytes) larger than a staging buffer (%zu)", bytes, ctx->staging_bytes);
+    if ((rc = flush_stage(ctx)) != TREW_OK) return rc;
     SlotRes& s = ctx->slots[ctx->next_slot];
     ctx->next_slot = (ctx->next_slot + 1) % ctx->slots.size();
     rc = retire_slot(ctx, s);
@@ -762,27 +813,35 @@
     trew_resident* r = const_cast<trew_resident*>(rb);
     ctx->keys_seen = std::max<unsigned int>(ctx->keys_seen, (unsigned int)(ctx->n_slots / 16 + 1));
     if (r->ev_pending) { int rc0 = collect_prof(ctx); if (rc0) return rc0; }
-    if (!r->ev[0]) for (int i = 0; i < 4; i++) CK(cudaEventCreate(&r->ev[i]));
+    if (!r->ev[0]) for (auto& e : r->ev) CK(cudaEventCreate(&e));
+    const int key = stage_key_for(ctx, r->max_read_len, r->n_units);
+    if (!ctx->pending.empty() && (key != ctx->stage_key || ctx->pending.size() >= (size_t)kStageBatches)) {
+        int rc0 = flush_stage(ctx);
+        if (rc0) return rc0;
+    }
     cudaStream_t st = (ctx->resident_streams == 2 && (ctx->resident_seq++ & 1)) ? ctx->aux_stream : ctx->main_stream;
     CK(cudaEventRecord(ctx->ev_a, st));
-    int rc = launch_scan(ctx, r->batch, r->n_units, r->max_read_len, r->scan, st, r->ev);
+    int rc = screen_batch(ctx, r->batch, r->n_units, r->max_read_len, r->scan, st, r->ev, &r->entry);
     r->ev_pending = true; ctx->pending_prof.push_back(r);
     if (rc) return rc;
-    CK(cudaEventRecord(ctx->ev_b, st));
+    if (ctx->pending.empty()) { ctx->stage_key = key; ctx->stage_len = 0; }
+    ctx->pending.push_back(r);
+    ctx->stage_len = std::max(ctx->stage_len, r->max_read_len);
     ctx->stats.reads += r->n_reads; ctx->stats.bases += r->bases; ctx->stats.units += r->n_units;
-    return TREW_OK;
+    return ctx->cfg.mode == TREW_MODE_LONG ? flush_stage(ctx) : TREW_OK;
 }
 
 void trew_dev_free_resident(trew_ctx* ctx, trew_resident* r) {
     if (!r) return;
-    if (ctx) { cudaSetDevice(ctx->cfg.device); cudaStreamSynchronize(ctx->main_stream); cudaStreamSynchronize(ctx->aux_stream); collect_prof(ctx); }
-    for (int i = 0; i < 4; i++) if (r->ev[i]) cudaEventDestroy(r->ev[i]);
+    if (ctx) { cudaSetDevice(ctx->cfg.device); flush_stage(ctx); cudaStreamSynchronize(ctx->main_stream); cudaStreamSynchronize(ctx->aux_stream); collect_prof(ctx); }
+    for (auto& e : r->ev) if (e) cudaEventDestroy(e);
     delete r;
 }
 
 int trew_dev_sync(trew_ctx* ctx) {
     if (!ctx) return TREW_ERR_ARG;
     CK(cudaSetDevice(ctx->cfg.device));
+    { int rc = flush_stage(ctx); if (rc) return rc; }
     for (auto& s : ctx->slots) { int rc = retire_slot(ctx, s); if (rc) return rc; }
     { int rc = join_aux(ctx); if (rc) return rc; }
     CK(cudaStreamSynchronize(ctx->main_stream));
@@ -969,6 +1028,7 @@
 int trew_dev_merge_rows(trew_ctx* ctx, const trew_entry* d_rows, uint64_t n_rows) {
     if (!ctx || (n_rows && !d_rows) || n_rows > 0xffffffffULL) return TREW_ERR_ARG;
     CK(cudaSetDevice(ctx->cfg.device));
+    { int rc = flush_stage(ctx); if (rc) return rc; }
     ctx->export_valid = false;
     ctx->table_used = true;
     ctx->keys_seen = std::max<unsigned int>(ctx->keys_seen, (unsigned int)(ctx->n_slots / 16 + 1));
@@ -980,6 +1040,8 @@
 
 int trew_dev_set_report_filter(trew_ctx* ctx, uint32_t min_total) {
     if (!ctx) return TREW_ERR_ARG;
+    CK(cudaSetDevice(ctx->cfg.device));
+    { int rc = flush_stage(ctx); if (rc) return rc; }
     ctx->report_min = min_total;
     return TREW_OK;
 }
@@ -1042,6 +1104,7 @@
 int trew_dev_get_stats(trew_ctx* ctx, trew_stats* out) {
     if (!ctx || !out) return TREW_ERR_ARG;
     CK(cudaSetDevice(ctx->cfg.device));
+    { int rc = flush_stage(ctx); if (rc) return rc; }
     unsigned long long s = 0;
     CK(cudaMemcpy(&s, ctx->d_total_surv.p, sizeof(s), cudaMemcpyDeviceToHost));
     ctx->stats.survivors = s;
@@ -1051,6 +1114,8 @@
 
 int trew_dev_last_resident_ms(trew_ctx* ctx, float* ms) {
     if (!ctx || !ms) return TREW_ERR_ARG;
+    CK(cudaSetDevice(ctx->cfg.device));
+    { int rc = flush_stage(ctx); if (rc) return rc; }
     CK(cudaEventSynchronize(ctx->ev_b));
     CK(cudaEventElapsedTime(ms, ctx->ev_a, ctx->ev_b));
     return TREW_OK;
@@ -1066,6 +1131,7 @@
 int trew_dev_timer_stop(trew_ctx* ctx, float* ms) {
     if (!ctx || !ms) return TREW_ERR_ARG;
     CK(cudaSetDevice(ctx->cfg.device));
+    { int rc = flush_stage(ctx); if (rc) return rc; }
     { int rc = join_aux(ctx); if (rc) return rc; }
     CK(cudaEventRecord(ctx->ev_t1, ctx->main_stream));
     CK(cudaEventSynchronize(ctx->ev_t1));
diff --git a/trew_b200/csrc/scan_kernels.cu b/trew_b200/csrc/scan_kernels.cu
--- a/trew_b200/csrc/scan_kernels.cu
+++ b/trew_b200/csrc/scan_kernels.cu
@@ -522,6 +522,37 @@
         base = __shfl_sync(0xffffffffu, base, 0);
         if (flag) *(top - (base + __popc(m & ((1u << lane_id()) - 1u)))) = value;
     }
+}
+
+__device__ __forceinline__ void stage_append(bool flag, u32 value, u32* list, u32* count, bool down, int key) {
+    const u32 m = __ballot_sync(0xffffffffu, flag);
+    if (m == 0u) return;
+    const u32 grp = __match_any_sync(0xffffffffu, key) & m;
+    const int leader = grp ? __ffs(grp) - 1 : 0;
+    u32 base = 0;
+    if (flag && (int)lane_id() == leader) base = atomicAdd(count, (u32)__popc(grp));
+    base = __shfl_sync(0xffffffffu, base, leader);
+    if (flag) {
+        const u32 at = base + __popc(grp & ((1u << lane_id()) - 1u));
+        if (down) *(list - at) = value;
+        else list[at] = value;
+    }
+}
+
+__device__ __forceinline__ void stage_prefix(const StageTable& t, int which, u32* s_pre) {
+    if (threadIdx.x != 0) return;
+    u32 acc = 0;
+    for (int j = 0; j < t.n; j++) {
+        s_pre[j] = acc;
+        acc += which == 2 && !t.e[j].screened ? t.e[j].n_units : t.e[j].counters[which];
+    }
+    s_pre[t.n] = acc;
+}
+
+__device__ __forceinline__ int stage_batch(const u32* s_pre, int n, u32 i) {
+    int j = 0;
+    while (j + 1 < n && s_pre[j + 1] <= i) j++;
+    return j;
 }
 
 #ifndef TREW_SCREEN_BPS
@@ -691,20 +722,20 @@
 }
 
 template <int MAXNW>
-__global__ void __launch_bounds__(kDecideThreads, (MAXNW <= 5 ? 4 : 2)) trew_filter_kernel(DevCfg cfg, DevBatch b, const u32* __restrict__ units,
-                                                          const u32* __restrict__ n_units_ptr, u32 n_units_all,
-                                                          u32* __restrict__ survivors, u32* __restrict__ n_survivors,
-                                                          u32* __restrict__ surv_b_top, u32* __restrict__ n_surv_b, int thread_min_windows, int third_level,
-                                                          u32* __restrict__ work_counter) {
+__global__ void __launch_bounds__(kDecideThreads, (MAXNW <= 5 ? 4 : 2)) trew_filter_kernel(DevCfg cfg, const __grid_constant__ StageTable t,
+                                                          int two_lists, int thread_min_windows, int third_level) {
     __shared__ unsigned short thr[kThrTableSize];
     __shared__ u32 s_m4[18 * kDecideThreads];
+    __shared__ u32 s_pre[kStageBatches + 1];
     for (int i = threadIdx.x; i < kThrTableSize; i += blockDim.x) thr[i] = cfg.thr_low[i];
+    stage_prefix(t, 2, s_pre);
     __syncthreads();
-    const u32 n_units = units ? *n_units_ptr : n_units_all;
-    const bool pack_probes = n_units_all < (1u << kProbeShift);
+    const u32 n_units = s_pre[t.n];
+    u32* const work_counter = t.e[0].counters + 7;
     const u32 lane = lane_id();
     bool have = false, maybe = false, exhausted = false;
     u32 u = 0, live = 0, todo = 0;
+    int bi = 0;
     int t_hit = 1 << 20;
     Probe p[4];
     for (;;) {
@@ -717,14 +748,18 @@
             const u32 i = base + (u32)__popc(idle & ((1u << lane) - 1u));
             if (!have && i < n_units) {
                 u32 pm = 0xfu;
-                u = i;
-                if (units) { const u32 e = units[i]; u = e & ((1u << kProbeShift) - 1u); pm = e >> kProbeShift; }
-                const int np = unit_probes(cfg, b, u, p);
+                bi = stage_batch(s_pre, t.n, i);
+                const StageBatch& sb = t.e[bi];
+                u = i - s_pre[bi];
+                if (sb.screened) { const u32 e = sb.survivors[sb.n_units + u]; u = e & ((1u << kProbeShift) - 1u); pm = e >> kProbeShift; }
+                const int np = unit_probes(cfg, sb.b, u, p);
                 live = todo = pm & ((1u << np) - 1u);
                 maybe = false; t_hit = 1 << 20; have = true;
             }
         }
         if (__ballot_sync(0xffffffffu, have) == 0u) break;
+        const StageBatch& sb = t.e[bi];
+        const DevBatch& b = sb.b;
         if (have && todo != 0u) {
             const int j = __ffs(todo) - 1;
             todo &= todo - 1u;
@@ -735,9 +770,9 @@
         }
         const bool fin = have && (todo == 0u || maybe);
         const bool keep = fin && maybe;
-        const u32 entry = pack_probes ? u | (live << kProbeShift) : u;
-        if (surv_b_top == nullptr) {
-            list_append(keep, entry, survivors, n_survivors);
+        const u32 entry = sb.n_units < (1u << kProbeShift) ? u | (live << kProbeShift) : u;
+        if (!two_lists) {
+            stage_append(keep, entry, sb.survivors, sb.counters + LIST_A, false, bi);
         } else {
             bool to_b = false;
             if (keep) {
@@ -750,38 +785,46 @@
                 }
                 to_b = len > et::kMaxRead || t_hit < thread_min_windows;
             }
-            list_append(keep && !to_b, entry, survivors, n_survivors);
-            list_append_rev(keep && to_b, entry, surv_b_top, n_surv_b);
+            stage_append(keep && !to_b, entry, sb.survivors, sb.counters + LIST_A, false, bi);
+            stage_append(keep && to_b, entry, sb.survivors + sb.n_units - 1, sb.counters + LIST_B, true, bi);
         }
         if (fin) have = false;
     }
 }
 
-void launch_filter(const DevCfg& cfg, const DevBatch& b, unsigned int n_units, unsigned int max_read_len,
-                   unsigned int* deferred, unsigned int* n_deferred, unsigned int* survivors, unsigned int* n_survivors,
-                   const LaunchPlan& plan, cudaStream_t stream, cudaEvent_t after_screen, unsigned int* surv_b_top,
-                   unsigned int* n_surv_b, unsigned int* work_counter) {
-    if (n_units == 0) return;
-    unsigned int longest;
-    if (cfg.mode == 2) longest = 2u * (unsigned)cfg.slice_len;
-    else longest = (max_read_len < 4u * (unsigned)cfg.max_mer) ? max_read_len : (max_read_len + 1) / 2;
-    unsigned int need = (n_units + 255) / 256;
-    const bool screen = deferred != nullptr && !(cfg.mode == 2 && cfg.slice_len > kFastMaxWlLong) && n_units < (1u << kProbeShift);
-    if (screen) {
-        int blocks = plan.screen_blocks;
-        if ((unsigned)blocks > need) blocks = (int)need;
-        if (longest <= (unsigned)kFastMaxWl) trew_screen_kernel<false><<<blocks, 256, 0, stream>>>(cfg, b, n_units, deferred, n_deferred);
-        else trew_screen_kernel<true><<<blocks, 256, 0, stream>>>(cfg, b, n_units, deferred, n_deferred);
-    }
-    if (after_screen) cudaEventRecord(after_screen, stream);
+static unsigned int longest_window(const DevCfg& cfg, unsigned int max_read_len) {
+    if (cfg.mode == 2) return 2u * (unsigned)cfg.slice_len;
+    return (max_read_len < 4u * (unsigned)cfg.max_mer) ? max_read_len : (max_read_len + 1) / 2;
+}
+
+int decide_variant(const DevCfg& cfg, unsigned int max_read_len) {
+    const unsigned int longest = longest_window(cfg, max_read_len);
+    return longest + 1 <= 96 ? 3 : longest + 1 <= 160 ? 5 : 8;
+}
+
+bool launch_screen(const DevCfg& cfg, const DevBatch& b, unsigned int n_units, unsigned int max_read_len, unsigned int* deferred,
+                   unsigned int* n_deferred, const LaunchPlan& plan, cudaStream_t stream) {
+    if ((cfg.mode == 2 && cfg.slice_len > kFastMaxWlLong) || n_units >= (1u << kProbeShift)) return false;
+    if (n_units == 0) return true;
+    int blocks = plan.screen_blocks;
+    const unsigned int need = (n_units + 255) / 256;
+    if ((unsigned)blocks > need) blocks = (int)need;
+    if (longest_window(cfg, max_read_len) <= (unsigned)kFastMaxWl) trew_screen_kernel<false><<<blocks, 256, 0, stream>>>(cfg, b, n_units, deferred, n_deferred);
+    else trew_screen_kernel<true><<<blocks, 256, 0, stream>>>(cfg, b, n_units, deferred, n_deferred);
+    return true;
+}
+
+void launch_decide(const DevCfg& cfg, const StageTable& t, unsigned int longest_read, unsigned long long units, bool two_lists,
+                   const LaunchPlan& plan, cudaStream_t stream) {
+    if (units == 0) return;
     static const int tmw = [] { const char* e = getenv("TREW_THREAD_MIN_WINDOWS"); return e && *e ? atoi(e) : kThreadMinWindows; }();
     static const int m4_on = [] { const char* e = getenv("TREW_MOD4_BELOW"); return e && *e ? atoi(e) : kMod4BelowWindows; }();
-    const unsigned int* list = screen ? deferred : nullptr;
     int blocks = plan.decide_blocks;
-    if ((unsigned)blocks > need) blocks = (int)need;
-    if (longest + 1 <= 96) trew_filter_kernel<3><<<blocks, 256, 0, stream>>>(cfg, b, list, n_deferred, n_units, survivors, n_survivors, surv_b_top, n_surv_b, tmw, m4_on, work_counter);
-    else if (longest + 1 <= 160) trew_filter_kernel<5><<<blocks, 256, 0, stream>>>(cfg, b, list, n_deferred, n_units, survivors, n_survivors, surv_b_top, n_surv_b, tmw, m4_on, work_counter);
-    else trew_filter_kernel<8><<<blocks, 256, 0, stream>>>(cfg, b, list, n_deferred, n_units, survivors, n_survivors, surv_b_top, n_surv_b, tmw, m4_on, work_counter);
+    if ((unsigned long long)blocks > (units + 255) / 256) blocks = (int)((units + 255) / 256);
+    const int nw = decide_variant(cfg, longest_read), tl = two_lists ? 1 : 0;
+    if (nw == 3) trew_filter_kernel<3><<<blocks, 256, 0, stream>>>(cfg, t, tl, tmw, m4_on);
+    else if (nw == 5) trew_filter_kernel<5><<<blocks, 256, 0, stream>>>(cfg, t, tl, tmw, m4_on);
+    else trew_filter_kernel<8><<<blocks, 256, 0, stream>>>(cfg, t, tl, tmw, m4_on);
 }
 
 
@@ -1673,18 +1716,19 @@
 };
 
 template <int MODE, class K, bool REC>
-__global__ void __launch_bounds__(TREW_THREAD_BLOCK, (thread_kernel_bps<MODE, K>())) trew_exact_thread_kernel(DevCfg cfg, DevBatch b, const u32* __restrict__ survivors,
-                                                                              const u32* __restrict__ n_survivors, int packed_probes,
-                                                                              u32* __restrict__ hard, u32* __restrict__ n_hard,
-                                                                              unsigned long long* total_survivors, u32* work_counter) {
+__global__ void __launch_bounds__(TREW_THREAD_BLOCK, (thread_kernel_bps<MODE, K>())) trew_exact_thread_kernel(DevCfg cfg, const __grid_constant__ StageTable t,
+                                                                              unsigned long long* total_survivors) {
     u32* work = reinterpret_cast<u32*>(g_smem);
     u64* s_key = reinterpret_cast<u64*>(work + et::Lay<K>::WORDS * TREW_THREAD_BLOCK);
     u32* s_meta = reinterpret_cast<u32*>(s_key + kStageSlots);
     u32* s_cnt = s_meta + kStageSlots;
+    __shared__ u32 s_pre[kStageBatches + 1];
     for (int i = threadIdx.x; i < kStageSlots; i += blockDim.x) { s_meta[i] = 0u; s_cnt[i] = 0u; }
+    stage_prefix(t, LIST_A, s_pre);
     __syncthreads();
     const et::Mem m{work + threadIdx.x, TREW_THREAD_BLOCK};
-    const u32 n = *n_survivors;
+    const u32 n = s_pre[t.n];
+    u32* const work_counter = t.e[0].counters + 6;
     if (blockIdx.x == 0 && threadIdx.x == 0 && total_survivors) atomicAdd(total_survivors, (unsigned long long)n);
     StageEmit emit{s_meta, s_cnt, s_key, cfg.slots, cfg.slot_mask, cfg.error_flag};
     for (;;) {
@@ -1695,10 +1739,12 @@
         const u32 i = base + lane_id();
         bool bail = false;
         u32 entry = 0;
+        const int bi = i < n ? stage_batch(s_pre, t.n, i) : 0;
+        const StageBatch& sb = t.e[bi];
         if (i < n) {
-            entry = survivors[i];
-            u32 u = entry, pm = 3u;
-            if (packed_probes) { pm = entry >> kProbeShift; u &= (1u << kProbeShift) - 1u; }
+            const DevBatch& b = sb.b;
+            entry = sb.survivors[i - s_pre[bi]];
+            const u32 u = entry & ((1u << kProbeShift) - 1u), pm = entry >> kProbeShift;
             auto route = [&](auto& em) {
                 if (MODE == 0) {
                     const u32 b0 = __ldg(b.bit_off + u);
@@ -1713,13 +1759,13 @@
                 return et::route_pair_thread<K>(m, n1, n2, cfg.min_mer, cfg.max_mer, cfg.thr_low, cfg.thr_high, load, em);
             };
             if constexpr (REC) {
-                RecStageEmit rem{emit, cfg.recs, cfg.unit_base + u};
+                RecStageEmit rem{emit, cfg.recs, sb.unit_base + u};
                 bail = !route(rem);
             } else {
                 bail = !route(emit);
             }
         }
-        list_append(bail, entry, hard, n_hard);
+        stage_append(bail, entry, sb.survivors + sb.n_units, sb.counters + LIST_BAILS, false, bi);
     }
     __syncthreads();
     for (int i = threadIdx.x; i < kStageSlots; i += blockDim.x) {
@@ -1869,14 +1915,13 @@
     return cfg.mode == 1 && max_read_len >= 4u * (unsigned)cfg.max_mer;
 }
 
-void launch_exact_thread(const DevCfg& cfg, const DevBatch& b, const unsigned int* survivors, const unsigned int* n_survivors,
-                         int packed_probes, unsigned int* hard, unsigned int* n_hard, unsigned long long* total_survivors, int sm_count,
-                         int blocks_per_sm, unsigned int* work_counter, cudaStream_t stream) {
+void launch_exact_thread(const DevCfg& cfg, const StageTable& t, unsigned long long* total_survivors, int sm_count, int blocks_per_sm,
+                         cudaStream_t stream) {
     const bool wide = cfg.max_mer > 32;
 #define TREW_LAUNCH_THREAD(MODE, K, REC)                                                                                          \
     trew_exact_thread_kernel<MODE, K, REC><<<sm_count * (blocks_per_sm > 0 ? blocks_per_sm : thread_kernel_bps<MODE, K>()),       \
                                              TREW_THREAD_BLOCK, thread_kernel_smem<K>(), stream>>>(                               \
-        cfg, b, survivors, n_survivors, packed_probes, hard, n_hard, total_survivors, work_counter)
+        cfg, t, total_survivors)
 #define TREW_LAUNCH_THREAD_MODE(MODE)                                                                                             \
     if (cfg.recs) { if (wide) TREW_LAUNCH_THREAD(MODE, et::u128, true); else TREW_LAUNCH_THREAD(MODE, et::u64, true); }            \
     else          { if (wide) TREW_LAUNCH_THREAD(MODE, et::u128, false); else TREW_LAUNCH_THREAD(MODE, et::u64, false); }
@@ -1887,7 +1932,7 @@
 }
 
 template <int MODE, bool REC>
-__global__ void __launch_bounds__(kExactWarps * 32, TREW_EXACT_BPS) trew_exact_kernel(DevCfg cfg, DevBatch b, ExactArgs a) {
+__global__ void __launch_bounds__(kExactWarps * 32, TREW_EXACT_BPS) trew_exact_kernel(DevCfg cfg, const __grid_constant__ StageTable t, ExactArgs a) {
     const int wid = threadIdx.x >> 5;
     const u32 lane = lane_id();
     WS ws;
@@ -1896,11 +1941,12 @@
     TableRef tr{cfg.slots, cfg.slot_mask, cfg.error_flag};
     ws.hdr()[lane] = lane == HD_CUR_LEN || lane == HD_EV_LEN || lane == HD_EV_K ? 0xffffffffu : 0u;
     if constexpr (REC) {
-        if (lane == HD_UNIT_BASE) { ws.hdr()[lane] = (u32)cfg.unit_base; ws.hdr()[lane + 1] = (u32)(cfg.unit_base >> 32); }
         if (lane == HD_RECS) { ws.hdr()[lane] = (u32)(u64)cfg.recs; ws.hdr()[lane + 1] = (u32)((u64)cfg.recs >> 32); }
     }
-    __syncwarp();
-    const u32 n = *a.n_survivors;
+    __shared__ u32 s_pre[kStageBatches + 1];
+    stage_prefix(t, a.list, s_pre);
+    __syncthreads();
+    const u32 n = s_pre[t.n];
     if (blockIdx.x == 0 && threadIdx.x == 0 && a.total_survivors) atomicAdd(a.total_survivors, (u64)n);
     unsigned char* scratch = a.slice_scratch + (size_t)(blockIdx.x * kExactWarps + wid) * a.slice_scratch_stride;
     for (;;) {
@@ -1908,9 +1954,17 @@
         if (lane == 0) idx = atomicAdd(a.work_counter, 1u);
         idx = __shfl_sync(0xffffffffu, idx, 0);
         if (idx >= n) break;
-        u32 u = a.reverse ? *(a.survivors - idx) : a.survivors[idx], pm = 0xfu;
-        if (a.packed_probes) { pm = u >> kProbeShift; u &= (1u << kProbeShift) - 1u; }
-        if constexpr (REC) ws.hdr()[HD_UNIT] = u;
+        const int bi = stage_batch(s_pre, t.n, idx);
+        const StageBatch& sb = t.e[bi];
+        const DevBatch& b = sb.b;
+        const u32 j = idx - s_pre[bi];
+        u32 u = a.list == LIST_A ? sb.survivors[j] : a.list == LIST_B ? sb.survivors[sb.n_units - 1 - j] : sb.survivors[sb.n_units + j];
+        u32 pm = 0xfu;
+        if (sb.n_units < (1u << kProbeShift)) { pm = u >> kProbeShift; u &= (1u << kProbeShift) - 1u; }
+        if constexpr (REC) {
+            ws.hdr()[HD_UNIT] = u;
+            ws.hdr()[HD_UNIT_BASE] = (u32)sb.unit_base; ws.hdr()[HD_UNIT_BASE + 1] = (u32)(sb.unit_base >> 32);
+        }
         if constexpr (MODE == 0) route_short<REC>(cfg, tr, ws, b, u, pm);
         else if constexpr (MODE == 1) route_pair<REC>(cfg, tr, ws, b, u);
         else route_long<REC>(cfg, tr, ws, b, u, scratch);
@@ -1947,18 +2001,18 @@
 
 LaunchPlan default_launch_plan(int sm_count) { return LaunchPlan{sm_count * 128, sm_count * 4, sm_count * kExactBlocksPerSM}; }
 
-void launch_exact(const DevCfg& cfg, const DevBatch& b, const ExactArgs& a, const LaunchPlan& plan, cudaStream_t stream) {
+void launch_exact(const DevCfg& cfg, const StageTable& t, const ExactArgs& a, const LaunchPlan& plan, cudaStream_t stream) {
     size_t smem = exact_smem_bytes(a.run_cap, true);
     dim3 grid(plan.exact_blocks), block(kExactWarps * 32);
     if (cfg.recs) {
-        if (cfg.mode == 0) trew_exact_kernel<0, true><<<grid, block, smem, stream>>>(cfg, b, a);
-        else if (cfg.mode == 1) trew_exact_kernel<1, true><<<grid, block, smem, stream>>>(cfg, b, a);
-        else trew_exact_kernel<2, true><<<grid, block, smem, stream>>>(cfg, b, a);
+        if (cfg.mode == 0) trew_exact_kernel<0, true><<<grid, block, smem, stream>>>(cfg, t, a);
+        else if (cfg.mode == 1) trew_exact_kernel<1, true><<<grid, block, smem, stream>>>(cfg, t, a);
+        else trew_exact_kernel<2, true><<<grid, block, smem, stream>>>(cfg, t, a);
     } else {
-        if (cfg.mode == 0) trew_exact_kernel<0, false><<<grid, block, smem, stream>>>(cfg, b, a);
-        else if (cfg.mode == 1) trew_exact_kernel<1, false><<<grid, block, smem, stream>>>(cfg, b, a);
-        else trew_exact_kernel<2, false><<<grid, block, smem, stream>>>(cfg, b, a);
-    }
-}
-
-}
+        if (cfg.mode == 0) trew_exact_kernel<0, false><<<grid, block, smem, stream>>>(cfg, t, a);
+        else if (cfg.mode == 1) trew_exact_kernel<1, false><<<grid, block, smem, stream>>>(cfg, t, a);
+        else trew_exact_kernel<2, false><<<grid, block, smem, stream>>>(cfg, t, a);
+    }
+}
+
+}
diff --git a/trew_b200/csrc/scan_kernels.cuh b/trew_b200/csrc/scan_kernels.cuh
--- a/trew_b200/csrc/scan_kernels.cuh
+++ b/trew_b200/csrc/scan_kernels.cuh
@@ -43,29 +43,42 @@
     const unsigned int* val;
 };
 
+constexpr int kStageBatches = 16;
+struct StageBatch {
+    DevBatch b;
+    unsigned int* survivors;
+    unsigned int* counters;
+    unsigned long long unit_base;
+    unsigned int n_units;
+    int screened;
+};
+struct StageTable {
+    int n;
+    StageBatch e[kStageBatches];
+};
+enum StageList { LIST_A = 0, LIST_B = 4, LIST_BAILS = 3 };
+
 struct ExactArgs {
-    const unsigned int* survivors;
-    const unsigned int* n_survivors;
+    int list;
     unsigned int* work_counter;
     unsigned char* slice_scratch;
     unsigned int slice_scratch_stride;
     int run_cap;
     unsigned long long* total_survivors;
-    int packed_probes;
-    int reverse;
     unsigned int exp_flags;
 };
 
 struct LaunchPlan { int screen_blocks, decide_blocks, exact_blocks; };
 LaunchPlan default_launch_plan(int sm_count);
 
-void launch_filter(const DevCfg& cfg, const DevBatch& b, unsigned int n_units, unsigned int max_read_len,
-                   unsigned int* deferred, unsigned int* n_deferred, unsigned int* survivors, unsigned int* n_survivors,
-                   const LaunchPlan& plan, cudaStream_t stream, cudaEvent_t after_screen,
-                   unsigned int* surv_b_top, unsigned int* n_surv_b, unsigned int* work_counter);
+bool launch_screen(const DevCfg& cfg, const DevBatch& b, unsigned int n_units, unsigned int max_read_len, unsigned int* deferred,
+                   unsigned int* n_deferred, const LaunchPlan& plan, cudaStream_t stream);
+void launch_decide(const DevCfg& cfg, const StageTable& t, unsigned int longest_read, unsigned long long units, bool two_lists,
+                   const LaunchPlan& plan, cudaStream_t stream);
+int decide_variant(const DevCfg& cfg, unsigned int max_read_len);
 size_t exact_smem_bytes(int run_cap, bool wide);
 cudaError_t prepare_exact(int run_cap_max);
-void launch_exact(const DevCfg& cfg, const DevBatch& b, const ExactArgs& a, const LaunchPlan& plan, cudaStream_t stream);
+void launch_exact(const DevCfg& cfg, const StageTable& t, const ExactArgs& a, const LaunchPlan& plan, cudaStream_t stream);
 int exact_warps_total(int sm_count);
 bool long_thread_path_applies(const DevCfg& cfg);
 size_t long_thread_scratch_bytes(unsigned int s_cap, unsigned int max_slices);
@@ -73,9 +86,8 @@
                         int packed_probes, unsigned int s_cap, unsigned int max_slices, unsigned char* scratch, unsigned int* hard,
                         unsigned int* n_hard, unsigned long long* total_survivors, int sm_count, cudaStream_t stream);
 bool thread_path_applies(const DevCfg& cfg, unsigned int max_read_len);
-void launch_exact_thread(const DevCfg& cfg, const DevBatch& b, const unsigned int* survivors, const unsigned int* n_survivors,
-                         int packed_probes, unsigned int* hard, unsigned int* n_hard, unsigned long long* total_survivors, int sm_count,
-                         int blocks_per_sm, unsigned int* work_counter, cudaStream_t stream);
+void launch_exact_thread(const DevCfg& cfg, const StageTable& t, unsigned long long* total_survivors, int sm_count, int blocks_per_sm,
+                         cudaStream_t stream);
 void launch_compact(const Slot* slots, unsigned int n_slots, trew_entry* out, unsigned int* d_n, cudaStream_t stream, unsigned int cap);
 cudaError_t sort_entries_radix(const trew_entry* d_entries, trew_entry* d_out, unsigned int n, bool wide, void* d_temp,
                                size_t* temp_bytes, cudaStream_t stream);
```

Result: faster. 1068 (median of 6 runs) (+3.1%).
